# amathislab/myochallenge

Measured on AMD Instinct MI355X. Metric: env-steps/sec (Baoding, 4096 envs), higher is better.
Workload: dtype f64

## Files before the change

include/myobatch.h:

```cpp
#ifndef MYOBATCH_H
#define MYOBATCH_H

#include <stddef.h>
#include <stdint.h>

#ifdef __cplusplus
extern "C" {
#endif

#define MYO_OK 0
#define MYO_E_ARG -1
#define MYO_E_UNSUPPORTED -2
#define MYO_E_DEVICE -3
#define MYO_E_STATE -4

typedef struct myo_model myo_model;
typedef struct myo_batch myo_batch;

enum { MYO_F64 = 0, MYO_MIXED = 1, MYO_F32 = 1 };
enum { MYO_TASK_NONE = 0, MYO_TASK_BAODING_P1 = 1, MYO_TASK_BAODING_P2 = 2, MYO_TASK_REORIENT = 3, MYO_TASK_POSE = 4 };
enum { MYO_POSE_RESET_INIT = 0, MYO_POSE_RESET_RANDOM = 1, MYO_POSE_RESET_SDS = 2 };
enum { MYO_POSE_TARGET_GENERATE = 0, MYO_POSE_TARGET_FIXED = 1 };
enum { MYO_WHICH_HOLD = 0, MYO_WHICH_CW = 1, MYO_WHICH_CCW = 2 };
enum { MYO_CHOICE_FIXED = 0, MYO_CHOICE_CW = 1, MYO_CHOICE_CCW = 2, MYO_CHOICE_RANDOM = 3 };

#define MYO_N_RWD 8
#define MYO_ROT_CHOICE_MAX 4
#define MYO_OBJG_MAX 20
#define MYO_POSE_NQ_MAX 38

typedef struct myo_task_cfg {
  int32_t kind;
  int32_t frame_skip;
  int32_t max_episode_steps;
  int32_t n_hand;
  int32_t obj1_sid, obj2_sid, target1_sid, target2_sid;
  int32_t obj1_bid, obj2_bid, obj1_gid, obj2_gid;
  int32_t task_choice;
  int32_t enable_rsi, balls_overlap, limit_init_angle_on, beta_init_angle_on, beta_ball_size_on,
      beta_ball_mass_on;
  double drop_th, proximity_th;
  double center_pos[2];
  double weights[7];
  double goal_time_period[2], goal_xrange[2], goal_yrange[2];
  double rsi_probability, overlap_probability;
  double noise_palm, noise_fingers, noise_balls;
  double limit_init_angle, beta_init_angle[2], beta_ball_size[2], beta_ball_mass[2];
  double obj_size_range[2], obj_mass_range[2], obj_friction_change[3];
  double init_qpos0;
  double ro_weights[9];
  double ro_goal_pos[2], ro_goal_rot[2];
  int32_t ro_n_rot_choice[3], ro_pad_;
  double ro_rot_choice[3][MYO_ROT_CHOICE_MAX][2];
  double ro_obj_size_change, ro_pos_th, ro_rot_th;
  double ro_goal_init_pos[3], ro_goal_obj_offset[3];
  double ro_rsi_distance_pos, ro_rsi_distance_rot;
  double pose_weights[7];
  double pose_thd, pose_far_th, pose_sds_distance, pose_target_distance;
  int32_t pose_reset_type, pose_target_type;
  double pose_init_qpos[MYO_POSE_NQ_MAX];
  double pose_target_value[MYO_POSE_NQ_MAX];
  double pose_target_range[MYO_POSE_NQ_MAX][2];
  double pose_reset_range[MYO_POSE_NQ_MAX][2];
} myo_task_cfg;

int myo_model_from_blob(const void* blob, size_t nbytes, myo_model** out);
int myo_model_load_mjb(const char* path, int integrator, int unsupported_contacts, myo_model** out);
void myo_model_destroy(myo_model* m);
int myo_model_size(const myo_model* m, const char* name);

int myo_batch_create(const myo_model* m, const myo_task_cfg* cfg, int n_envs, int device,
                     uint64_t seed, int dtype, myo_batch** out);
void myo_batch_destroy(myo_batch* b);
int myo_batch_num_envs(const myo_batch* b);
int myo_batch_obs_dim(const myo_batch* b);
int myo_batch_lds_bytes(const myo_batch* b);

int myo_batch_reset(myo_batch* b, const uint8_t* mask, float* obs, void* stream);

int myo_batch_step(myo_batch* b, const float* act, float* obs, float* rew, uint8_t* done,
                   uint8_t* trunc, float* term_obs, float* comps, float* ep_info, void* stream);

int myo_batch_set_step_generation(myo_batch* b, unsigned int gen);

int myo_batch_health(myo_batch* b, int out[4]);

int myo_debug_wave_slots(int device, int n_workgroups, int lds_bytes, int32_t out[4]);

int myo_batch_step_inner(myo_batch* b, const uint8_t* mask, const float* act, float* obs, uint8_t* done, void* stream);

int myo_batch_step_inner_idx(myo_batch* b, const int* idx, int n_idx, const float* act, float* obs, uint8_t* done, void* stream);

int myo_batch_copy_envs(myo_batch* dst, const int* dst_idx, const myo_batch* src, const int* src_idx, int k, void* stream);

int myo_batch_physics_step(myo_batch* b, const double* ctrl, int nsub, void* stream);

int myo_batch_get_state(myo_batch* b, double* qpos, double* qvel, double* act, double* time,
                        void* stream);
int myo_batch_set_state(myo_batch* b, const double* qpos, const double* qvel, const double* act,
                        const double* time, void* stream);
int myo_batch_set_bad_state_buffer(myo_batch* b, uint8_t* bad_state);

int myo_batch_warmstart(myo_batch* b, double* get_qacc_warmstart, const double* set_qacc_warmstart, void* stream);

int myo_batch_set_task(myo_batch* b, const int32_t* task_i, const double* task_d,
                       const double* ball_d, void* stream);
int myo_batch_get_task(myo_batch* b, int32_t* task_i, double* task_d, double* ball_d, void* stream);

int myo_batch_set_object_group(myo_batch* b, int gid0, int gidn);
int myo_batch_object_friction(myo_batch* b, const double* set_fric, double* get_fric, void* stream);

int myo_batch_bind_constants(myo_batch* b, void* stream);

int myo_batch_tune_wrap_order(myo_batch* b, void* stream);

int myo_batch_forward_dump(myo_batch* b, const double* ctrl, double* out, void* stream);
int myo_batch_dump_size(const myo_batch* b);
int myo_batch_dump_offset(const myo_batch* b, const char* name);

typedef struct myo_render_camera {
  double lookat[3];
  double distance, azimuth, elevation;
  double fovy;
} myo_render_camera;
#define MYO_RENDER_RGB 1
#define MYO_RENDER_DEPTH 2
#define MYO_RENDER_SEG 4
#define MYO_RENDER_SITES 8
#define MYO_RENDER_ITEM_N 24
#define MYO_RENDER_MAX_PIXELS (1 << 24)

int myo_model_default_camera(const myo_model* m, myo_render_camera* out);

int myo_batch_geom_poses(myo_batch* b, const int32_t* env_idx, int k, double* out, void* stream);

int myo_batch_render(myo_batch* b, const int32_t* env_idx, int k, const myo_render_camera* cams, int ncams, int width, int height,
                     int flags, uint8_t* rgb, float* depth, int32_t* segid, void* stream);

double myo_batch_kernel_ms(myo_batch* b);
int myo_batch_enable_timing(myo_batch* b, int on);

int myo_ppo_loss_grad(const float* mean, const float* values, const float* actions, const float* old_logp,
                      const float* adv, const float* returns, const float* log_std, const float* adv_stats,
                      int B, int A, float clip, float vf_coef, float* dmean, float* dvalue, float* acc,
                      uint16_t* dmean_bf16, uint16_t* dvalue_bf16, float* work, int in_bf16, float ent_coef,
                      float* g_log_std, float* g_bias_pi, float* g_bias_vf, void* stream);

int myo_ppo_gather(const float* obs, const float* act, const float* oldlp, const float* adv, const float* ret,
                   const int64_t* idx, int bs, int obs_dim, int act_dim, uint16_t* obs_bf16, int copies,
                   float* act_mb, float* oldlp_mb, float* adv_mb, float* ret_mb, float* adv_stats , float* work,
                   void* stream);

int myo_bias_relu_bf16(uint16_t* h, const uint16_t* bias, int groups, int rows, int cols, void* stream);

int myo_splitk_reduce(const void* part, int part_is_bf16, float* out, int groups, int splits, int n, void* stream);
int myo_splitk_reduce2(const void* part_a, int a_is_bf16, float* out_a, int groups_a, int splits_a, int n_a,
                       const void* part_b, int b_is_bf16, float* out_b, int groups_b, int splits_b, int n_b, void* stream);

int myo_relu_bwd_colsum_bf16(uint16_t* dy, const uint16_t* act, int rows, int cols, float* partial, void* stream);

int myo_rollout_policy_input(const float* obs, int N, int O, float* obs_buf, uint16_t* x_bf16, int copies,
                             const int32_t* t_idx, void* stream);
int myo_rollout_sample(const uint16_t* mean_bf16, const uint16_t* value_bf16, const float* log_std, int N, int A,
                       uint64_t seed, uint64_t* draw_counter, const int32_t* t_idx, float* act_buf, float* val_buf,
                       float* logp_buf, float* clipped, int deterministic, void* stream);
int myo_vecnorm_step(const float* obs, const float* rew, const uint8_t* done, const uint8_t* trunc, const float* term_obs,
                     int N, int O, double* obs_mean, double* obs_var, double* obs_count, double* ret_stats,
                     double* returns, double gamma, double eps, double clip_obs, double clip_rew, int training,
                     int norm_obs, int norm_reward, float* nobs, float* starts, const int32_t* t_idx, float* rew_buf,
                     float* start_buf, float* term_buf, float* trunc_buf, double* work, void* stream);
int myo_rollout_sample_sde(const float* mean, const float* latent, const float* exploration_mat, const float* log_std, int N, int L,
                           int A, float* actions, float* clipped, float* logp, int deterministic, void* stream);

int myo_vecnorm_batch_moments(const float* obs, const float* rew, int N, int O, double* returns, double gamma, int training,
                              double* work, double* batch, void* stream);
int myo_vecnorm_finish(const float* obs, const float* rew, const uint8_t* done, const uint8_t* trunc, const float* term_obs,
                       int N, int O, double* obs_mean, double* obs_var, double* obs_count, double* ret_stats, double* returns,
                       double eps, double clip_obs, double clip_rew, int training, int norm_obs, int norm_reward, float* nobs,
                       float* starts, const int32_t* t_idx, float* rew_buf, float* start_buf, float* term_buf, float* trunc_buf,
                       const double* batch, void* stream);
int myo_rollout_advance(int32_t* t_idx, int T, uint64_t* draw_counter, void* stream);

int myo_lstm_cell_fwd(const void* gx, const void* gh, const void* c_prev, const float* keep_next, int R, int N, int H,
                      int is_bf16, void* out_h, void* hm_next, void* cm_next, void* c_new, void* ws, void* stream);
int myo_lstm_cell_bwd(const void* dout, const void* dhm_next, const void* dcm_next, const float* keep_next,
                      const void* c_prev, const void* c_new, const void* ws, int R, int N, int H, int is_bf16,
                      void* dgates, void* dc_prev, void* stream);

int myo_lstm_step_supported(int H);
int myo_lstm_step_fwd(const void* gx, long long gx_sg, long long gx_sr, const void* h_prev, const void* c_prev, const void* w_hh,
                      const float* keep_next, int G, int N, int H, void* out_h, long long out_sg, void* hm_next, void* cm_next,
                      void* c_new, void* ws, const float* c_prev32, float* cm_next32, void* stream);
int myo_lstm_step_bwd(const void* dout, long long dout_sg, const void* dgates_next, const void* dcm_next, const void* w_hh_t,
                      const float* keep_next, const void* c_prev, const void* c_new, const void* ws, int G, int N, int H,
                      void* dgates, void* dc_prev, void* stream);

int myo_lstm_seq_supported(int H);
int myo_lstm_seq_fwd(const void* gx, long long gx_st, long long gx_sg, long long gx_sr, void* hm, void* cm, const void* w_frag,
                     const float* keep, int G, int N, int H, int T, int row_split, void* out_h, long long out_sg, long long out_st,
                     void* c_new, void* ws, const float* c0_32, void* stream);
int myo_lstm_seq_bwd(const void* dout, long long dout_sg, long long dout_st, const void* wt_frag, const float* keep, const void* cm,
                     const void* c_new, const void* ws, int G, int N, int H, int T, int row_split, void* dgates, void* stream);

int myo_gae(const float* rew, const float* val, const float* starts, const float* last_val,
            const float* last_done, int T, int N, float gamma, float lam, float* adv, float* ret,
            void* stream);

typedef struct myo_ppo_mlp_desc {
  const float *obs, *act, *oldlp, *adv, *ret;
  const int64_t* idx;
  int32_t B, O, A, hidden;
  const float* params;
  float* grads;
  int64_t G;
  int64_t off_W1[2], off_b1[2], off_W2[2], off_b2[2], off_Wh[2], off_bh[2], off_log_std;
  float clip, vf_coef, ent_coef;
  int32_t compute_adv_stats;
  float* adv_stats;
  float* acc;
  void* workspace;
  int64_t workspace_bytes;
  float* sqnorm_part;
  int32_t* adam_step;
} myo_ppo_mlp_desc;
int myo_ppo_mlp_sqnorm_parts(int act_dim);
long long myo_ppo_mlp_workspace_bytes(int B, int obs_dim, int act_dim, int hidden, long long G);
int myo_ppo_mlp_step(const myo_ppo_mlp_desc* d, void* stream);

typedef struct myo_ppo_mlp_rollout_desc {
  const float* obs;
  int32_t N, O, A, hidden;
  const float* params;
  int64_t off_W1[2], off_b1[2], off_W2[2], off_b2[2], off_Wh[2], off_bh[2], off_log_std;
  uint64_t seed;
  uint64_t* draw_counter;
  const int32_t* t_idx;
  float *obs_buf, *act_buf, *val_buf, *logp_buf, *clipped;
  int32_t deterministic;
  void* workspace;
  int64_t workspace_bytes;
} myo_ppo_mlp_rollout_desc;
long long myo_ppo_mlp_rollout_workspace_bytes(int obs_dim, int act_dim, int hidden);
int myo_ppo_mlp_rollout_refresh(const myo_ppo_mlp_rollout_desc* d, void* stream);
int myo_ppo_mlp_rollout(const myo_ppo_mlp_rollout_desc* d, void* stream);

int myo_adam_clip_step(float* p, const float* g, float* m, float* v, int n, float lr, float b1, float b2,
                       float eps, float max_norm, float grad_scale, int* step, float* scratch, uint16_t* p_bf16,
                       void* stream);
int myo_adam_apply(float* p, const float* g, float* m, float* v, int n, float lr, float b1, float b2,
                   float eps, float max_norm, float grad_scale, const int* step, const float* scratch, int nparts,
                   uint16_t* p_bf16, void* stream);

const char* myo_last_error(void);
const char* myo_version(void);

#ifdef __cplusplus
}
#endif
#endif
```

myochallenge_amd/csrc/myo_ppo_mlp.h:

```cpp
#pragma once
#ifndef MYO_EMU

typedef __attribute__((ext_vector_type(8))) __bf16 myo_bf16x8;
typedef __attribute__((ext_vector_type(4))) float myo_f32x4;

#define MLP_H 256
#define MLP_OPMAX 128
#define MLP_APM 48
#define MLP_AKP 64
#define MLP_XS (MLP_OPMAX + 8)
#define MLP_HS (MLP_H + 8)
#define MLP_DS (MLP_AKP + 8)
#define MLP_SOS 49
#define MLP_SPLITK 16

struct MlpArgs {
  const float *obs, *act, *oldlp, *adv, *ret;
  const long long* idx;
  const float *log_std, *adv_stats;
  const unsigned short *W1p, *W2, *W2T, *Whp, *WhT;
  const float* bias;
  unsigned short *XT, *H1T, *H2T, *dH1T, *dH2T, *dOT;
  float* part;
  int B, O, A, OP, NB;
  float clip, vf_coef;
};

__device__ __forceinline__ unsigned short mlp_f2bf(float x) {
  unsigned u = __float_as_uint(x);
  u += 0x7fffu + ((u >> 16) & 1u);
  return (unsigned short)(u >> 16);
}
__device__ __forceinline__ float mlp_bf2f(unsigned short h) { return __uint_as_float((unsigned)h << 16); }

struct MlpPrepArgs {
  const float* p;
  long long off_W1[2], off_b1[2], off_W2[2], off_b2[2], off_Wh[2], off_bh[2];
  int O, OP, Ah[2];
  unsigned short *W1p, *W2, *W2T, *Whp, *WhT;
  float* bias;
  const float* adv_part;
  float* adv_stats;
  int adv_nb, B;
};

#define MLP_ADV_BLOCKS 64
__global__ void __launch_bounds__(256) k_mlp_prep(MlpPrepArgs P) {
  if (P.adv_nb > 0 && blockIdx.x == gridDim.x - 1) {
    __shared__ float sp[3 * MLP_ADV_BLOCKS];
    const int t = threadIdx.x;
    if (t < 3 * P.adv_nb) sp[t] = P.adv_part[t];
    __syncthreads();
    if (t == 0) {
      float cn = 0.f, cm = 0.f, c2 = 0.f;
      for (int b = 0; b < P.adv_nb; ++b) {
        const float bn = sp[3 * b], bm = sp[3 * b + 1], b2 = sp[3 * b + 2];
        if (bn > 0.f) {
          const float tot = cn + bn, dl = bm - cm;
          cm += dl * (bn / tot);
          c2 += b2 + dl * dl * (cn * bn / tot);
          cn = tot;
        }
      }
      P.adv_stats[0] = cm; P.adv_stats[1] = sqrtf(c2 / (P.B > 1 ? P.B - 1 : 1));
    }
  }
  constexpr int H = MLP_H;
  const long long tid = (long long)blockIdx.x * blockDim.x + threadIdx.x, nth = (long long)gridDim.x * blockDim.x;
  for (int net = 0; net < 2; ++net) {
    const float* W1 = P.p + P.off_W1[net]; const float* W2 = P.p + P.off_W2[net]; const float* Wh = P.p + P.off_Wh[net];
    for (long long e = tid; e < (long long)H * P.OP; e += nth) {
      const int o = (int)(e / P.OP), i = (int)(e % P.OP);
      P.W1p[(size_t)net * H * P.OP + e] = i < P.O ? mlp_f2bf(W1[(size_t)o * P.O + i]) : (unsigned short)0;
    }
    for (long long e = tid; e < (long long)H * H; e += nth) {
      const int o = (int)(e / H), i = (int)(e % H);
      const unsigned short v = mlp_f2bf(W2[e]);
      P.W2[(size_t)net * H * H + e] = v;
      P.W2T[(size_t)net * H * H + (size_t)i * H + o] = v;
    }
    for (long long e = tid; e < (long long)MLP_APM * H; e += nth) {
      const int a = (int)(e / H), h = (int)(e % H);
      P.Whp[(size_t)net * MLP_APM * H + e] = a < P.Ah[net] ? mlp_f2bf(Wh[(size_t)a * H + h]) : (unsigned short)0;
    }
    for (long long e = tid; e < (long long)H * MLP_AKP; e += nth) {
      const int h = (int)(e / MLP_AKP), a = (int)(e % MLP_AKP);
      P.WhT[(size_t)net * H * MLP_AKP + e] = a < P.Ah[net] ? mlp_f2bf(Wh[(size_t)a * H + h]) : (unsigned short)0;
    }
    for (long long e = tid; e < H; e += nth) {
      P.bias[net * H + e] = P.p[P.off_b1[net] + e];
      P.bias[2 * H + net * H + e] = P.p[P.off_b2[net] + e];
    }
    for (long long e = tid; e < MLP_APM; e += nth) P.bias[4 * H + net * MLP_APM + e] = e < P.Ah[net] ? P.p[P.off_bh[net] + e] : 0.f;
  }
}

__global__ void __launch_bounds__(256) k_adv_moments(const float* __restrict__ adv, const long long* __restrict__ idx, int B,
                                                     float* __restrict__ part) {
  __shared__ float red[4];
  __shared__ float s_mean;
  const int t = threadIdx.x, nb = gridDim.x;
  const int chunk = (B + nb - 1) / nb, lo = blockIdx.x * chunk, hi = min(B, lo + chunk), n = max(hi - lo, 0);
  constexpr int PER = 4;
  float v[PER];
  float s = 0.f;
#pragma unroll
  for (int k = 0; k < PER; ++k) { const int i = lo + t + 256 * k; v[k] = i < hi ? adv[idx[i]] : 0.f; s += v[k]; }
  for (int i = lo + t + 256 * PER; i < hi; i += 256) s += adv[idx[i]];
  for (int off = 32; off >= 1; off >>= 1) s += __shfl_xor(s, off, 64);
  if ((t & 63) == 0) red[t >> 6] = s;
  __syncthreads();
  if (t == 0) s_mean = n ? ((red[0] + red[1]) + (red[2] + red[3])) / n : 0.f;
  __syncthreads();
  const float mean = s_mean;
  float m2 = 0.f;
#pragma unroll
  for (int k = 0; k < PER; ++k) { const float d = v[k] - mean; m2 += (lo + t + 256 * k) < hi ? d * d : 0.f; }
  for (int i = lo + t + 256 * PER; i < hi; i += 256) { const float d = adv[idx[i]] - mean; m2 += d * d; }
  for (int off = 32; off >= 1; off >>= 1) m2 += __shfl_xor(m2, off, 64);
  __syncthreads();
  if ((t & 63) == 0) red[t >> 6] = m2;
  __syncthreads();
  if (t == 0) { part[3 * blockIdx.x] = (float)n; part[3 * blockIdx.x + 1] = mean; part[3 * blockIdx.x + 2] = (red[0] + red[1]) + (red[2] + red[3]); }
}

template <int KSTEPS>
__device__ __forceinline__ void mlp_load_w(myo_bf16x8 (&bw)[8][4], const unsigned short* Wg, int w_stride, int n0, int lm, int lq) {
#pragma unroll
  for (int ks = 0; ks < KSTEPS; ++ks)
#pragma unroll
    for (int nt = 0; nt < 4; ++nt) bw[ks][nt] = *reinterpret_cast<const myo_bf16x8*>(Wg + (size_t)(n0 + 16 * nt + lm) * w_stride + 32 * ks + 8 * lq);
  __builtin_amdgcn_sched_barrier(0);
}
template <int KSTEPS, int MT>
__device__ __forceinline__ void mlp_mma_slab(myo_f32x4 (&acc)[MT][4], const unsigned short* As, int as_stride, const myo_bf16x8 (&bw)[8][4],
                                             int lm, int lq) {
#pragma unroll
  for (int mt = 0; mt < MT; ++mt)
#pragma unroll
    for (int nt = 0; nt < 4; ++nt) acc[mt][nt] = myo_f32x4{0.f, 0.f, 0.f, 0.f};
#pragma unroll
  for (int ks = 0; ks < KSTEPS; ++ks) {
#pragma unroll
    for (int m2 = 0; m2 < MT; m2 += 2) {
      myo_bf16x8 a[2];
#pragma unroll
      for (int mt = 0; mt < 2; ++mt) a[mt] = *reinterpret_cast<const myo_bf16x8*>(As + (16 * (m2 + mt) + lm) * as_stride + 32 * ks + 8 * lq);
#pragma unroll
      for (int mt = 0; mt < 2; ++mt)
#pragma unroll
        for (int nt = 0; nt < 4; ++nt) acc[m2 + mt][nt] = __builtin_amdgcn_mfma_f32_16x16x32_bf16(a[mt], bw[ks][nt], acc[m2 + mt][nt], 0, 0, 0);
    }
  }
  __builtin_amdgcn_sched_barrier(0);
}

#ifdef MLP_PROF
__device__ unsigned long long g_mlp_prof[16];
#define MLP_STAMP(k) { __syncthreads(); if (threadIdx.x == 0 && blockIdx.x == 3 && blockIdx.y == 0) g_mlp_prof[k] = wall_clock64(); }
extern "C" int myo_debug_mlp_prof(unsigned long long* out) { return (int)hipMemcpyFromSymbol(out, HIP_SYMBOL(g_mlp_prof), sizeof g_mlp_prof); }
#else
#define MLP_STAMP(k)
#endif

#ifndef MLP_BM
#define MLP_BM 32
#endif
#define MLP_FWDBWD_LDS (512 + MLP_BM * MLP_XS * 2 + MLP_BM * MLP_HS * 2 + MLP_BM * MLP_SOS * 4 + MLP_BM * MLP_DS * 2 + 128 * 4 + 192 * 4)

template <int MT>
__device__ __forceinline__ unsigned long long mlp_store_act(const myo_f32x4 (&acc)[MT][4], const float (&bb)[4], unsigned short* Hs, unsigned short* HT,
                                                            size_t B, int r0, int n0, int lm, int lq) {
  static_assert(MT * 16 <= 64, "one mask bit per accumulator element");
  unsigned long long mask = 0;
#pragma unroll
  for (int mt = 0; mt < MT; ++mt)
#pragma unroll
    for (int nt = 0; nt < 4; ++nt) {
      const int n = n0 + 16 * nt + lm, m = 16 * mt + 4 * lq;
      unsigned short h[4];
#pragma unroll
      for (int r = 0; r < 4; ++r) {
        h[r] = mlp_f2bf(fmaxf(acc[mt][nt][r] + bb[nt], 0.f)); Hs[(m + r) * MLP_HS + n] = h[r];
        mask |= (unsigned long long)(h[r] != 0) << (16 * mt + 4 * nt + r);
      }
      *reinterpret_cast<uint2*>(HT + (size_t)n * B + r0 + m) = make_uint2((unsigned)h[0] | ((unsigned)h[1] << 16), (unsigned)h[2] | ((unsigned)h[3] << 16));
    }
  return mask;
}
template <int MT, bool TO_LDS>
__device__ __forceinline__ void mlp_store_grad(const myo_f32x4 (&acc)[MT][4], unsigned long long mask, unsigned short* Hs, unsigned short* HT, size_t B,
                                               int r0, int n0, int lm, int lq) {
#pragma unroll
  for (int mt = 0; mt < MT; ++mt)
#pragma unroll
    for (int nt = 0; nt < 4; ++nt) {
      const int n = n0 + 16 * nt + lm, m = 16 * mt + 4 * lq;
      unsigned short h[4];
#pragma unroll
      for (int r = 0; r < 4; ++r) {
        const unsigned short on = (unsigned short)(-(int)((mask >> (16 * mt + 4 * nt + r)) & 1ull));
        h[r] = mlp_f2bf(acc[mt][nt][r]) & on;
        if (TO_LDS) Hs[(m + r) * MLP_HS + n] = h[r];
      }
      *reinterpret_cast<uint2*>(HT + (size_t)n * B + r0 + m) = make_uint2((unsigned)h[0] | ((unsigned)h[1] << 16), (unsigned)h[2] | ((unsigned)h[3] << 16));
    }
}

__global__ void __launch_bounds__(256, 2) k_mlp_fwdbwd(MlpArgs P) {
  constexpr int H = MLP_H, XS = MLP_XS, HS = MLP_HS, DS = MLP_DS, SOS = MLP_SOS, BM = MLP_BM, MT = BM / 16, RW = BM / 4;
  extern __shared__ __align__(16) unsigned char mlp_smem[];
  long long* s_idx = reinterpret_cast<long long*>(mlp_smem);
  unsigned short* Xs = reinterpret_cast<unsigned short*>(mlp_smem + 512);
  float* So = reinterpret_cast<float*>(mlp_smem + 512);
  unsigned short* Hs = Xs + BM * XS;
  float* Sa = reinterpret_cast<float*>(Hs + BM * HS);
  unsigned short* dOs = reinterpret_cast<unsigned short*>(Sa + BM * SOS);
  float* s_ls = reinterpret_cast<float*>(dOs + BM * DS);
  float* s_row = s_ls + 128;
  static_assert(BM * MLP_SOS * 4 <= BM * MLP_XS * 2, "the head output tile fits where X was");
  static_assert(BM == 32 || BM == 64, "wave / tile mapping below");
  const int t = threadIdx.x, w = t >> 6, lane = t & 63, lm = lane & 15, lq = lane >> 4;
  const int net = blockIdx.y, blk = blockIdx.x, r0 = blk * BM, B = P.B, O = P.O, A = P.A, OP = P.OP;
  const int n0 = 64 * w;
  MLP_STAMP(0)
  if (t < BM) s_idx[t] = P.idx[r0 + t];
  if (t < A) { const float ls = P.log_std[t]; s_ls[t] = ls; s_ls[64 + t] = __expf(-ls); }
  const float* b1 = P.bias + net * H; const float* b2 = P.bias + 2 * H + net * H; const float* bh = P.bias + 4 * H + net * MLP_APM;
  float bb1[4], bb2[4];
#pragma unroll
  for (int nt = 0; nt < 4; ++nt) { bb1[nt] = b1[n0 + 16 * nt + lm]; bb2[nt] = b2[n0 + 16 * nt + lm]; }
  myo_bf16x8 bw[8][4];
  {
    const unsigned short* W1 = P.W1p + (size_t)net * H * OP;
    if (OP == 96) mlp_load_w<3>(bw, W1, OP, n0, lm, lq);
    else if (OP == 128) mlp_load_w<4>(bw, W1, OP, n0, lm, lq);
    else if (OP == 64) mlp_load_w<2>(bw, W1, OP, n0, lm, lq);
    else mlp_load_w<1>(bw, W1, OP, n0, lm, lq);
  }
  __syncthreads();
  if (t < BM) {
    const size_t src = (size_t)s_idx[t];
    s_row[t] = P.adv[src]; s_row[64 + t] = P.oldlp[src]; s_row[128 + t] = P.ret[src];
  }
  {
    float v[RW][2], av[RW];
#pragma unroll
    for (int k = 0; k < RW; ++k) {
      const size_t row = (size_t)s_idx[RW * w + k];
      v[k][0] = lane < O ? P.obs[row * O + lane] : 0.f;
      v[k][1] = lane + 64 < O ? P.obs[row * O + lane + 64] : 0.f;
      av[k] = (net == 0 && lane < A) ? P.act[row * A + lane] : 0.f;
    }
#pragma unroll
    for (int k = 0; k < RW; ++k) {
      Xs[(RW * w + k) * XS + lane] = mlp_f2bf(v[k][0]);
      if (lane + 64 < OP) Xs[(RW * w + k) * XS + lane + 64] = mlp_f2bf(v[k][1]);
      if (lane < A) Sa[(RW * w + k) * SOS + lane] = av[k];
    }
    if (net == 0) {
#pragma unroll
      for (int h = 0; h < 2; ++h) {
        const int c = lane + 64 * h;
        if (c < OP) {
          unsigned u[RW / 2];
#pragma unroll
          for (int k = 0; k < RW / 2; ++k) u[k] = (unsigned)mlp_f2bf(v[2 * k][h]) | ((unsigned)mlp_f2bf(v[2 * k + 1][h]) << 16);
          uint4* dst = reinterpret_cast<uint4*>(P.XT + (size_t)c * B + r0 + RW * w);
#pragma unroll
          for (int q = 0; q < RW / 8; ++q) dst[q] = make_uint4(u[4 * q], u[4 * q + 1], u[4 * q + 2], u[4 * q + 3]);
        }
      }
    }
  }
  __syncthreads();
  MLP_STAMP(1)
  myo_f32x4 acc[MT][4];
  if (OP == 96) mlp_mma_slab<3, MT>(acc, Xs, XS, bw, lm, lq);
  else if (OP == 128) mlp_mma_slab<4, MT>(acc, Xs, XS, bw, lm, lq);
  else if (OP == 64) mlp_mma_slab<2, MT>(acc, Xs, XS, bw, lm, lq);
  else mlp_mma_slab<1, MT>(acc, Xs, XS, bw, lm, lq);
  mlp_load_w<H / 32>(bw, P.W2 + (size_t)net * H * H, H, n0, lm, lq);
  const unsigned long long mask1 = mlp_store_act<MT>(acc, bb1, Hs, P.H1T + (size_t)net * H * B, B, r0, n0, lm, lq);
  __syncthreads();
  MLP_STAMP(2)
  mlp_mma_slab<H / 32, MT>(acc, Hs, HS, bw, lm, lq);
  const unsigned short* Wh = P.Whp + (size_t)net * MLP_APM * H;
  myo_bf16x8 bh2[H / 32];
  if (w < 3) {
#pragma unroll
    for (int ks = 0; ks < H / 32; ++ks) bh2[ks] = *reinterpret_cast<const myo_bf16x8*>(Wh + (size_t)(16 * w + lm) * H + 32 * ks + 8 * lq);
  }
  __builtin_amdgcn_sched_barrier(0);
  __syncthreads();
  const unsigned long long mask2 = mlp_store_act<MT>(acc, bb2, Hs, P.H2T + (size_t)net * H * B, B, r0, n0, lm, lq);
  __syncthreads();
  MLP_STAMP(3)
  if (w < 3) {
    const float bv = bh[16 * w + lm];
#pragma unroll
    for (int mt = 0; mt < MT; ++mt) {
      myo_f32x4 ah = myo_f32x4{0.f, 0.f, 0.f, 0.f};
#pragma unroll
      for (int ks = 0; ks < H / 32; ++ks) {
        const myo_bf16x8 a = *reinterpret_cast<const myo_bf16x8*>(Hs + (16 * mt + lm) * HS + 32 * ks + 8 * lq);
        ah = __builtin_amdgcn_mfma_f32_16x16x32_bf16(a, bh2[ks], ah, 0, 0, 0);
      }
#pragma unroll
      for (int r = 0; r < 4; ++r) So[(16 * mt + 4 * lq + r) * SOS + 16 * w + lm] = ah[r] + bv;
    }
  }
  mlp_load_w<MLP_AKP / 32>(bw, P.WhT + (size_t)net * H * MLP_AKP, MLP_AKP, n0, lm, lq);
  __syncthreads();
  MLP_STAMP(4)
  const int NB = P.NB;
  if (w == 0) {
    const int r = lane < BM ? lane : 0;
    const bool on = lane < BM;
    if (net == 0) {
      float logp = 0.f;
      for (int a = 0; a < A; ++a) {
        const float z = (Sa[r * SOS + a] - So[r * SOS + a]) * s_ls[64 + a];
        logp += -0.5f * z * z - s_ls[a] - 0.9189385332046727f;
      }
      const float an = (s_row[r] - P.adv_stats[0]) / (P.adv_stats[1] + 1e-8f);
      const float ratio = __expf(logp - s_row[64 + r]);
      const float s1 = an * ratio;
      const float rc = fminf(fmaxf(ratio, 1.f - P.clip), 1.f + P.clip);
      const float s2 = an * rc;
      float pl_i = on ? -fminf(s1, s2) / B : 0.f;
      const bool inside = (ratio > 1.f - P.clip) && (ratio < 1.f + P.clip);
      const float dlogp = -(an * ratio) * ((s1 <= s2) ? 1.f : (inside ? 1.f : 0.f)) / B;
      if (on) {
        for (int a = 0; a < A; ++a) {
          const float inv = s_ls[64 + a];
          const float z = (Sa[r * SOS + a] - So[r * SOS + a]) * inv;
          const float dm = dlogp * z * inv;
          So[r * SOS + a] = dm;
          Sa[r * SOS + a] = dlogp * (z * z - 1.f);
          dOs[r * DS + a] = mlp_f2bf(dm);
        }
        for (int a = A; a < MLP_AKP; ++a) dOs[r * DS + a] = 0;
      }
      for (int off = 32; off >= 1; off >>= 1) pl_i += __shfl_xor(pl_i, off, 64);
      if (lane == 0) P.part[(size_t)A * NB + blk] = pl_i;
    } else {
      const float dv = So[r * SOS] - s_row[128 + r];
      float vl_i = on ? dv * dv / B : 0.f, dv_i = on ? P.vf_coef * 2.f / B * dv : 0.f;
      if (on) {
        dOs[r * DS] = mlp_f2bf(dv_i);
        for (int a = 1; a < MLP_AKP; ++a) dOs[r * DS + a] = 0;
      }
      for (int off = 32; off >= 1; off >>= 1) { vl_i += __shfl_xor(vl_i, off, 64); dv_i += __shfl_xor(dv_i, off, 64); }
      if (lane == 0) { P.part[(size_t)(A + 1) * NB + blk] = vl_i; P.part[(size_t)(2 * A + 2) * NB + blk] = dv_i; }
    }
  }
  __syncthreads();
  MLP_STAMP(5)
  if (net == 0 && t < A) {
    float my_ls = 0.f, my_db = 0.f;
    for (int r = 0; r < BM; ++r) { my_ls += Sa[r * SOS + t]; my_db += So[r * SOS + t]; }
    P.part[(size_t)t * NB + blk] = my_ls; P.part[(size_t)(A + 2 + t) * NB + blk] = my_db;
  }
  {
    const int Ah = net == 0 ? A : 1;
    for (int e = t; e < Ah * (BM / 8); e += 256) {
      const int c = e / (BM / 8), ch = e % (BM / 8);
      unsigned v[4];
#pragma unroll
      for (int k = 0; k < 4; ++k) v[k] = (unsigned)dOs[(8 * ch + 2 * k) * DS + c] | ((unsigned)dOs[(8 * ch + 2 * k + 1) * DS + c] << 16);
      *reinterpret_cast<uint4*>(P.dOT + ((size_t)net * 128 + c) * B + r0 + 8 * ch) = make_uint4(v[0], v[1], v[2], v[3]);
    }
  }
  MLP_STAMP(6)
  mlp_mma_slab<MLP_AKP / 32, MT>(acc, dOs, DS, bw, lm, lq);
  mlp_load_w<H / 32>(bw, P.W2T + (size_t)net * H * H, H, n0, lm, lq);
  mlp_store_grad<MT, true>(acc, mask2, Hs, P.dH2T + (size_t)net * H * B, B, r0, n0, lm, lq);
  __syncthreads();
  MLP_STAMP(7)
  mlp_mma_slab<H / 32, MT>(acc, Hs, HS, bw, lm, lq);
  mlp_store_grad<MT, false>(acc, mask1, Hs, P.dH1T + (size_t)net * H * B, B, r0, n0, lm, lq);
  MLP_STAMP(8)
}

struct MlpPolicyArgs {
  const float* obs;
  const float* log_std;
  const unsigned short *W1p, *W2, *Whp;
  const float* bias;
  float* obs_buf;
  float *act_buf, *val_buf, *logp_buf, *clipped;
  const int* t_idx;
  unsigned long long* draw_counter;
  unsigned long long seed;
  int N, O, A, OP, deterministic;
};
#define MLP_POLICY_LDS (MLP_BM * MLP_XS * 2 + MLP_BM * MLP_HS * 2 + 128 * 4)

template <int MT>
__device__ __forceinline__ void mlp_store_act_lds(const myo_f32x4 (&acc)[MT][4], const float (&bb)[4], unsigned short* Hs, int n0, int lm, int lq) {
#pragma unroll
  for (int mt = 0; mt < MT; ++mt)
#pragma unroll
    for (int nt = 0; nt < 4; ++nt) {
// ... 250 lines not shown
```

myochallenge_amd/csrc/myobatch.hip:

```cpp
#include <hip/hip_runtime.h>
#include <utility>
#include <vector>
#define MYO_BACKEND_NAME "gfx950"
#define MYO_BACKEND_DENSE_NEWTON 0
#define MYO_BACKEND_BATCH_FIELDS hipEvent_t ev0, ev1; std::vector<std::pair<hipEvent_t, hipEvent_t>> pending;
#include "myo_host.h"

typedef hipStream_t be_stream;
static int be_malloc(void** p, size_t n) { return (int)hipMalloc(p, n ? n : 1); }
static void be_free(void* p) { (void)hipFree(p); }
static int be_h2d(void* d, const void* h, size_t n) { return (int)hipMemcpy(d, h, n, hipMemcpyHostToDevice); }
static int be_set_device(int dev) { return (int)hipSetDevice(dev); }
static const char* be_errstr(int e) { return hipGetErrorString((hipError_t)e); }

#define MYO_MAX_DEVICES 64
struct BoundDev { const myo_batch* b = nullptr; hipStream_t last = nullptr; bool have_last = false; hipEvent_t ev = nullptr; };
static BoundDev g_bound[MYO_MAX_DEVICES];
static std::mutex g_bound_mu;
struct SlotWs { double* p = nullptr; int* map = nullptr; int users = 0; char* big = nullptr; int big_users = 0; };
static SlotWs g_slot_ws[MYO_MAX_DEVICES];
static bool slot_workspace_acquire(int device, double** ws, int** map) {
  if (device < 0 || device >= MYO_MAX_DEVICES) return false;
  std::lock_guard<std::mutex> lk(g_bound_mu);
  SlotWs& w = g_slot_ws[device];
// ... 1258 lines not shown
      const double m = part[((size_t)b * (O + 1) + c) * 2];
      s1 += n_b * m;
      s2 += part[((size_t)b * (O + 1) + c) * 2 + 1] + n_b * m * m;
    }
    batch[1 + c] = s1; batch[2 + O + c] = s2;
  }
  if (t == 0) batch[0] = (double)N;
}
__global__ void __launch_bounds__(128) k_vecnorm_merge_batch(const double* __restrict__ batch, int O, double* __restrict__ obs_mean,
                                                             double* __restrict__ obs_var, double* __restrict__ obs_count,
                                                             double* __restrict__ ret_stats, int upd_obs, int upd_ret) {
  const int t = threadIdx.x;
  const double oc = *obs_count, rc = ret_stats[2], n = batch[0];
  __syncthreads();
  for (int c = t; c <= O; c += 128) {
    if ((c < O && !upd_obs) || (c == O && !upd_ret)) continue;
    const double bmean = batch[1 + c] / n;
    double bvar = batch[2 + O + c] / n - bmean * bmean;
    bvar = bvar < 0 ? 0 : bvar;
    double* mean = c < O ? obs_mean + c : ret_stats;
    double* var = c < O ? obs_var + c : ret_stats + 1;
    const double cnt = c < O ? oc : rc;
    const double delta = bmean - *mean, tot = cnt + n;
    const double new_mean = *mean + delta * n / tot;
    const double M2 = *var * cnt + bvar * n + delta * delta * cnt * n / tot;
    *mean = new_mean; *var = M2 / tot;
  }
  if (t == 0) { if (upd_obs) *obs_count = oc + n; if (upd_ret) ret_stats[2] = rc + n; }
}
__global__ void __launch_bounds__(256) k_vecnorm_apply(const float* __restrict__ obs, const float* __restrict__ rew,
                                                       const unsigned char* __restrict__ done, const unsigned char* __restrict__ trunc,
                                                       const float* __restrict__ term, int N, int O, const double* __restrict__ obs_mean,
                                                       const double* __restrict__ obs_var, const double* __restrict__ ret_stats,
                                                       double* __restrict__ returns, double eps, double clip_obs, double clip_rew,
                                                       int norm_obs, int norm_rew, float* __restrict__ nobs, float* __restrict__ starts,
                                                       const int* __restrict__ t_idx, float* __restrict__ rew_buf,
                                                       float* __restrict__ start_buf, float* __restrict__ term_buf,
                                                       float* __restrict__ trunc_buf) {
  const size_t i = (size_t)blockIdx.x * blockDim.x + threadIdx.x;
  const size_t n = (size_t)N * O, tt = (size_t)(*t_idx);
  if (i < n) {
    const int c = (int)(i % O);
    double o = obs[i], q = term[i];
    if (norm_obs) {
      const double sd = sqrt(obs_var[c] + eps), mu = obs_mean[c];
      o = fmin(fmax((o - mu) / sd, -clip_obs), clip_obs);
      q = fmin(fmax((q - mu) / sd, -clip_obs), clip_obs);
    }
    nobs[i] = (float)o;
    if (term_buf) term_buf[tt * n + i] = (float)q;
  }
  if (i < (size_t)N) {
    double r = rew[i];
    if (norm_rew) r = fmin(fmax(r / sqrt(ret_stats[1] + eps), -clip_rew), clip_rew);
    rew_buf[tt * N + i] = (float)r;
    start_buf[tt * N + i] = starts[i];
    const unsigned char dn = done[i];
    starts[i] = dn ? 1.f : 0.f;
    if (trunc_buf) trunc_buf[tt * N + i] = trunc[i] ? 1.f : 0.f;
    if (dn) returns[i] = 0.0;
  }
}
__global__ void __launch_bounds__(64) k_sample_sde(const float* __restrict__ mean, const float* __restrict__ latent,
                                                   const float* __restrict__ W, const float* __restrict__ log_std, int N, int L, int A,
                                                   float* __restrict__ actions, float* __restrict__ clipped, float* __restrict__ logp,
                                                   int deterministic) {
  const int n = blockIdx.x, t = threadIdx.x;
  float lp_part = 0.f;
  for (int j = t; j < A; j += 64) {
    const float* w = W + (size_t)n * L * A + j;
    const float* lat = latent + (size_t)n * L;
    float noise = 0.f, var = 0.f;
    for (int l = 0; l < L; ++l) {
      const float x = lat[l], sd = __expf(log_std[(size_t)l * A + j]);
      noise = fmaf(x, w[(size_t)l * A], noise);
      var = fmaf(x * x, sd * sd, var);
    }
    const float mu = mean[(size_t)n * A + j], sg = sqrtf(var + 1e-6f);
    const float a = deterministic ? mu : mu + noise;
    actions[(size_t)n * A + j] = a;
    clipped[(size_t)n * A + j] = fminf(fmaxf(a, -1.f), 1.f);
    const float z = (a - mu) / sg;
    lp_part += -0.5f * z * z - logf(sg) - 0.9189385332046727f;
  }
  for (int off = 32; off >= 1; off >>= 1) lp_part += __shfl_xor(lp_part, off, 64);
  if (t == 0) logp[n] = lp_part;
}
__global__ void k_rollout_advance(int* t_idx, int T, unsigned long long* draw_counter) {
  *t_idx = (*t_idx + 1) % T;
  draw_counter[0] = draw_counter[1];
}
extern "C" int myo_rollout_policy_input(const float* obs, int N, int O, float* obs_buf, uint16_t* x_bf16, int copies,
                                        const int32_t* t_idx, void* stream) {
  if (!obs || !x_bf16 || !t_idx || N <= 0 || O <= 0 || copies <= 0) return fail(MYO_E_ARG, "myo_rollout_policy_input: bad arguments");
  const size_t n = (size_t)N * O;
  hipLaunchKernelGGL(k_obs_prepare, dim3((unsigned)((n + 255) / 256)), dim3(256), 0, (hipStream_t)stream, obs, n, obs_buf, x_bf16, copies, t_idx);
  LAUNCH_CHECK(0)
  return MYO_OK;
}
extern "C" int myo_rollout_sample(const uint16_t* mean_bf16, const uint16_t* value_bf16, const float* log_std, int N, int A,
                                  uint64_t seed, uint64_t* draw_counter, const int32_t* t_idx, float* act_buf, float* val_buf,
                                  float* logp_buf, float* clipped, int deterministic, void* stream) {
  if (!mean_bf16 || !value_bf16 || !log_std || !draw_counter || !t_idx || !act_buf || !val_buf || !logp_buf || !clipped || N <= 0 || A <= 0)
    return fail(MYO_E_ARG, "myo_rollout_sample: bad arguments");
  hipLaunchKernelGGL(k_sample_actions, dim3((N + MYO_SAMPLE_ROWS - 1) / MYO_SAMPLE_ROWS), dim3(16 * MYO_SAMPLE_ROWS), 0, (hipStream_t)stream, mean_bf16, value_bf16, log_std, N, A,
                     (unsigned long long)seed, (unsigned long long*)draw_counter, t_idx, act_buf, val_buf, logp_buf, clipped, deterministic);
  LAUNCH_CHECK(0)
  return MYO_OK;
}
extern "C" int myo_vecnorm_step(const float* obs, const float* rew, const uint8_t* done, const uint8_t* trunc, const float* term_obs,
                                int N, int O, double* obs_mean, double* obs_var, double* obs_count, double* ret_stats,
                                double* returns, double gamma, double eps, double clip_obs, double clip_rew, int training,
                                int norm_obs, int norm_reward, float* nobs, float* starts, const int32_t* t_idx, float* rew_buf,
                                float* start_buf, float* term_buf, float* trunc_buf, double* work, void* stream) {
  if (!obs || !rew || !done || !trunc || !term_obs || !obs_mean || !obs_var || !obs_count || !ret_stats || !returns || !nobs ||
      !starts || !t_idx || !rew_buf || !start_buf || !work || N <= 0 || O <= 0)
    return fail(MYO_E_ARG, "myo_vecnorm_step: bad arguments");
  hipStream_t st = (hipStream_t)stream;
  const int nb = (N + MYO_VN_ROWS - 1) / MYO_VN_ROWS;
  hipLaunchKernelGGL(k_vecnorm_moments, dim3(nb), dim3(128), 0, st, obs, rew, N, O, returns, gamma, training, work);
  if (training)
    hipLaunchKernelGGL(k_vecnorm_merge, dim3(1), dim3(128), 0, st, work, nb, N, O, obs_mean, obs_var, obs_count, ret_stats,
                       (int)(training && norm_obs), (int)(training != 0));
  const size_t n = (size_t)N * O;
  hipLaunchKernelGGL(k_vecnorm_apply, dim3((unsigned)((n + 255) / 256)), dim3(256), 0, st, obs, rew, done, trunc, term_obs, N, O,
                     obs_mean, obs_var, ret_stats, returns, eps, clip_obs, clip_rew, norm_obs, norm_reward, nobs, starts, t_idx,
                     rew_buf, start_buf, term_buf, trunc_buf);
  LAUNCH_CHECK(0)
  return MYO_OK;
}
extern "C" int myo_rollout_sample_sde(const float* mean, const float* latent, const float* exploration_mat, const float* log_std,
                                      int N, int L, int A, float* actions, float* clipped, float* logp, int deterministic, void* stream) {
  if (!mean || !latent || !exploration_mat || !log_std || !actions || !clipped || !logp || N <= 0 || L <= 0 || A <= 0)
    return fail(MYO_E_ARG, "myo_rollout_sample_sde: bad arguments");
  hipLaunchKernelGGL(k_sample_sde, dim3(N), dim3(64), 0, (hipStream_t)stream, mean, latent, exploration_mat, log_std, N, L, A, actions,
                     clipped, logp, deterministic);
  LAUNCH_CHECK(0)
  return MYO_OK;
}
extern "C" int myo_vecnorm_batch_moments(const float* obs, const float* rew, int N, int O, double* returns, double gamma, int training,
                                         double* work, double* batch, void* stream) {
  if (!obs || !rew || !returns || !work || !batch || N <= 0 || O <= 0) return fail(MYO_E_ARG, "myo_vecnorm_batch_moments: bad arguments");
  hipStream_t st = (hipStream_t)stream;
  const int nb = (N + MYO_VN_ROWS - 1) / MYO_VN_ROWS;
  hipLaunchKernelGGL(k_vecnorm_moments, dim3(nb), dim3(128), 0, st, obs, rew, N, O, returns, gamma, training, work);
  hipLaunchKernelGGL(k_vecnorm_batch, dim3(1), dim3(128), 0, st, work, nb, N, O, batch);
  LAUNCH_CHECK(0)
  return MYO_OK;
}
extern "C" int myo_vecnorm_finish(const float* obs, const float* rew, const uint8_t* done, const uint8_t* trunc, const float* term_obs,
                                  int N, int O, double* obs_mean, double* obs_var, double* obs_count, double* ret_stats,
                                  double* returns, double eps, double clip_obs, double clip_rew, int training, int norm_obs,
                                  int norm_reward, float* nobs, float* starts, const int32_t* t_idx, float* rew_buf, float* start_buf,
                                  float* term_buf, float* trunc_buf, const double* batch, void* stream) {
  if (!obs || !rew || !done || !trunc || !term_obs || !obs_mean || !obs_var || !obs_count || !ret_stats || !returns || !nobs ||
      !starts || !t_idx || !rew_buf || !start_buf || !batch || N <= 0 || O <= 0)
    return fail(MYO_E_ARG, "myo_vecnorm_finish: bad arguments");
  hipStream_t st = (hipStream_t)stream;
  if (training)
    hipLaunchKernelGGL(k_vecnorm_merge_batch, dim3(1), dim3(128), 0, st, batch, O, obs_mean, obs_var, obs_count, ret_stats,
                       (int)(training && norm_obs), (int)(training != 0));
  const size_t n = (size_t)N * O;
  hipLaunchKernelGGL(k_vecnorm_apply, dim3((unsigned)((n + 255) / 256)), dim3(256), 0, st, obs, rew, done, trunc, term_obs, N, O,
                     obs_mean, obs_var, ret_stats, returns, eps, clip_obs, clip_rew, norm_obs, norm_reward, nobs, starts, t_idx,
                     rew_buf, start_buf, term_buf, trunc_buf);
  LAUNCH_CHECK(0)
  return MYO_OK;
}
extern "C" int myo_rollout_advance(int32_t* t_idx, int T, uint64_t* draw_counter, void* stream) {
  if (!t_idx || !draw_counter || T <= 0) return fail(MYO_E_ARG, "myo_rollout_advance: bad arguments");
  hipLaunchKernelGGL(k_rollout_advance, dim3(1), dim3(1), 0, (hipStream_t)stream, t_idx, T, (unsigned long long*)draw_counter);
  LAUNCH_CHECK(0)
  return MYO_OK;
}

template <typename E> __device__ __forceinline__ float myo_ld(const E* p, size_t i);
template <> __device__ __forceinline__ float myo_ld<float>(const float* p, size_t i) { return p[i]; }
template <> __device__ __forceinline__ float myo_ld<unsigned short>(const unsigned short* p, size_t i) { return __uint_as_float((unsigned)p[i] << 16); }
template <typename E> __device__ __forceinline__ void myo_st(E* p, size_t i, float v);
template <> __device__ __forceinline__ void myo_st<float>(float* p, size_t i, float v) { p[i] = v; }
template <> __device__ __forceinline__ void myo_st<unsigned short>(unsigned short* p, size_t i, float v) { p[i] = myo_f2bf(v); }
__device__ __forceinline__ float myo_sigmoid(float x) { return 1.f / (1.f + __expf(-x)); }
template <typename E>
__global__ void __launch_bounds__(256) k_lstm_cell_fwd(const E* __restrict__ gx, const E* __restrict__ gh, const E* __restrict__ c_prev,
                                                       const float* __restrict__ keep_next, int R, int N, int H, E* __restrict__ out_h,
                                                       E* __restrict__ hm_next, E* __restrict__ cm_next, E* __restrict__ c_new,
                                                       E* __restrict__ ws) {
  const size_t idx = (size_t)blockIdx.x * blockDim.x + threadIdx.x;
  if (idx >= (size_t)R * H) return;
  const int r = (int)(idx / H), j = (int)(idx % H);
  const size_t g0 = (size_t)r * 4 * H + j;
  const float i = myo_sigmoid(myo_ld(gx, g0) + myo_ld(gh, g0));
  const float f = myo_sigmoid(myo_ld(gx, g0 + H) + myo_ld(gh, g0 + H));
  const float g = tanhf(myo_ld(gx, g0 + 2 * H) + myo_ld(gh, g0 + 2 * H));
  const float o = myo_sigmoid(myo_ld(gx, g0 + 3 * H) + myo_ld(gh, g0 + 3 * H));
  const float c = f * myo_ld(c_prev, idx) + i * g;
  const float h = o * tanhf(c);
  const float k = keep_next ? keep_next[r % N] : 1.f;
  myo_st(out_h, idx, h);
  myo_st(c_new, idx, c);
  myo_st(hm_next, idx, h * k);
  myo_st(cm_next, idx, c * k);
  myo_st(ws, g0, i); myo_st(ws, g0 + H, f); myo_st(ws, g0 + 2 * H, g); myo_st(ws, g0 + 3 * H, o);
}
template <typename E>
__global__ void __launch_bounds__(256) k_lstm_cell_bwd(const E* __restrict__ dout, const E* __restrict__ dhm_next, const E* __restrict__ dcm_next,
                                                       const float* __restrict__ keep_next, const E* __restrict__ c_prev,
                                                       const E* __restrict__ c_new, const E* __restrict__ ws, int R, int N, int H,
                                                       E* __restrict__ dgates, E* __restrict__ dc_prev) {
  const size_t idx = (size_t)blockIdx.x * blockDim.x + threadIdx.x;
  if (idx >= (size_t)R * H) return;
  const int r = (int)(idx / H), j = (int)(idx % H);
  const size_t g0 = (size_t)r * 4 * H + j;
  const float k = keep_next ? keep_next[r % N] : 1.f;
  const float dh = (dout ? myo_ld(dout, idx) : 0.f) + (dhm_next ? k * myo_ld(dhm_next, idx) : 0.f);
  const float dc_in = dcm_next ? k * myo_ld(dcm_next, idx) : 0.f;
  const float i = myo_ld(ws, g0), f = myo_ld(ws, g0 + H), g = myo_ld(ws, g0 + 2 * H), o = myo_ld(ws, g0 + 3 * H);
  const float tc = tanhf(myo_ld(c_new, idx));
  const float dct = dc_in + dh * o * (1.f - tc * tc);
  myo_st(dgates, g0, dct * g * i * (1.f - i));
  myo_st(dgates, g0 + H, dct * myo_ld(c_prev, idx) * f * (1.f - f));
  myo_st(dgates, g0 + 2 * H, dct * i * (1.f - g * g));
  myo_st(dgates, g0 + 3 * H, dh * tc * o * (1.f - o));
  myo_st(dc_prev, idx, dct * f);
}
extern "C" int myo_lstm_cell_fwd(const void* gx, const void* gh, const void* c_prev, const float* keep_next, int R, int N, int H,
                                 int is_bf16, void* out_h, void* hm_next, void* cm_next, void* c_new, void* ws, void* stream) {
  if (!gx || !gh || !c_prev || !out_h || !hm_next || !cm_next || !c_new || !ws || R <= 0 || N <= 0 || H <= 0 || R % N)
    return fail(MYO_E_ARG, "myo_lstm_cell_fwd: bad arguments");
  const unsigned nb = (unsigned)(((size_t)R * H + 255) / 256);
  if (is_bf16)
    hipLaunchKernelGGL(k_lstm_cell_fwd<unsigned short>, dim3(nb), dim3(256), 0, (hipStream_t)stream, (const unsigned short*)gx,
                       (const unsigned short*)gh, (const unsigned short*)c_prev, keep_next, R, N, H, (unsigned short*)out_h,
                       (unsigned short*)hm_next, (unsigned short*)cm_next, (unsigned short*)c_new, (unsigned short*)ws);
  else
    hipLaunchKernelGGL(k_lstm_cell_fwd<float>, dim3(nb), dim3(256), 0, (hipStream_t)stream, (const float*)gx, (const float*)gh,
                       (const float*)c_prev, keep_next, R, N, H, (float*)out_h, (float*)hm_next, (float*)cm_next, (float*)c_new,
                       (float*)ws);
  LAUNCH_CHECK(0)
  return MYO_OK;
}
extern "C" int myo_lstm_cell_bwd(const void* dout, const void* dhm_next, const void* dcm_next, const float* keep_next,
                                 const void* c_prev, const void* c_new, const void* ws, int R, int N, int H, int is_bf16,
                                 void* dgates, void* dc_prev, void* stream) {
  if (!c_prev || !c_new || !ws || !dgates || !dc_prev || R <= 0 || N <= 0 || H <= 0 || R % N)
    return fail(MYO_E_ARG, "myo_lstm_cell_bwd: bad arguments");
  const unsigned nb = (unsigned)(((size_t)R * H + 255) / 256);
  if (is_bf16)
    hipLaunchKernelGGL(k_lstm_cell_bwd<unsigned short>, dim3(nb), dim3(256), 0, (hipStream_t)stream, (const unsigned short*)dout,
                       (const unsigned short*)dhm_next, (const unsigned short*)dcm_next, keep_next, (const unsigned short*)c_prev,
                       (const unsigned short*)c_new, (const unsigned short*)ws, R, N, H, (unsigned short*)dgates,
                       (unsigned short*)dc_prev);
  else
    hipLaunchKernelGGL(k_lstm_cell_bwd<float>, dim3(nb), dim3(256), 0, (hipStream_t)stream, (const float*)dout, (const float*)dhm_next,
                       (const float*)dcm_next, keep_next, (const float*)c_prev, (const float*)c_new, (const float*)ws, R, N, H,
                       (float*)dgates, (float*)dc_prev);
  LAUNCH_CHECK(0)
  return MYO_OK;
}

__global__ void k_gae(const float* __restrict__ rew, const float* __restrict__ val, const float* __restrict__ starts,
                      const float* __restrict__ last_val, const float* __restrict__ last_done, int T, int N, float gamma,
                      float lam, float* __restrict__ adv, float* __restrict__ ret) {
  const int e = blockIdx.x * blockDim.x + threadIdx.x;
  if (e >= N) return;
  float last = 0.f, nextv = last_val[e], nonterm = 1.f - last_done[e];
  for (int t = T - 1; t >= 0; --t) {
    const size_t i = (size_t)t * N + e;
    const float v = val[i];
    const float delta = rew[i] + gamma * nextv * nonterm - v;
    last = delta + gamma * lam * nonterm * last;
    adv[i] = last;
    ret[i] = last + v;
    nextv = v;
    nonterm = 1.f - starts[i];
  }
}
extern "C" int myo_gae(const float* rew, const float* val, const float* starts, const float* last_val, const float* last_done,
                       int T, int N, float gamma, float lam, float* adv, float* ret, void* stream) {
  if (!rew || !val || !starts || !last_val || !last_done || !adv || !ret || T <= 0 || N <= 0) return fail(MYO_E_ARG, "myo_gae: bad arguments");
  hipLaunchKernelGGL(k_gae, dim3((N + 255) / 256), dim3(256), 0, (hipStream_t)stream, rew, val, starts, last_val, last_done, T, N,
                     gamma, lam, adv, ret);
  LAUNCH_CHECK(0)
  return MYO_OK;
}

#define MYO_SQN_BLOCKS 64
__global__ void __launch_bounds__(256) k_grad_sqnorm(const float* __restrict__ g, int n, float gs, float* __restrict__ part,
                                                     int* __restrict__ step) {
  float acc = 0.f;
  for (int i = blockIdx.x * 256 + threadIdx.x; i < n; i += MYO_SQN_BLOCKS * 256) { const float x = g[i] * gs; acc += x * x; }
  for (int off = 32; off >= 1; off >>= 1) acc += __shfl_xor(acc, off, 64);
  __shared__ float red[4];
  if ((threadIdx.x & 63) == 0) red[threadIdx.x >> 6] = acc;
  __syncthreads();
  if (threadIdx.x == 0) {
    part[blockIdx.x] = (red[0] + red[1]) + (red[2] + red[3]);
    if (blockIdx.x == 0) { const int done = step[1]; step[0] = done; step[1] = done + 1; }
  }
}
__global__ void __launch_bounds__(256) k_adam(float* __restrict__ p, const float* __restrict__ g, float* __restrict__ m,
                                              float* __restrict__ v, int n, float lr, float b1, float b2, float eps,
                                              float max_norm, float gs, const int* __restrict__ step,
                                              const float* __restrict__ part, unsigned short* __restrict__ p_bf16, int nparts) {
  __shared__ float sq_red[256];
  {
    float a = 0.f;
    for (int k = threadIdx.x; k < nparts; k += 256) a += part[k];
    sq_red[threadIdx.x] = a;
    __syncthreads();
    for (int w = 128; w >= 1; w >>= 1) { if ((int)threadIdx.x < w) sq_red[threadIdx.x] += sq_red[threadIdx.x + w]; __syncthreads(); }
  }
  const float sq = sq_red[0];
  const int t = step[1];
  const float norm = sqrtf(sq);
  const float clip = (max_norm > 0.f) ? fminf(1.f, max_norm / (norm + 1e-6f)) : 1.f;
  const float bc1 = 1.f - powf(b1, (float)t), bc2 = 1.f - powf(b2, (float)t);
  const float step_size = lr / bc1, inv_sqrt_bc2 = rsqrtf(bc2);
  for (int i = blockIdx.x * blockDim.x + threadIdx.x; i < n; i += gridDim.x * blockDim.x) {
    const float gi = g[i] * gs * clip;
    const float mi = b1 * m[i] + (1.f - b1) * gi;
    const float vi = b2 * v[i] + (1.f - b2) * gi * gi;
    m[i] = mi; v[i] = vi;
    const float pn = p[i] - step_size * mi / (sqrtf(vi) * inv_sqrt_bc2 + eps);
    p[i] = pn;
    if (p_bf16) p_bf16[i] = myo_f2bf(pn);
  }
}
extern "C" int myo_adam_clip_step(float* p, const float* g, float* m, float* v, int n, float lr, float b1, float b2,
                                  float eps, float max_norm, float grad_scale, int* step, float* scratch, uint16_t* p_bf16,
                                  void* stream) {
  if (!p || !g || !m || !v || !step || !scratch || n <= 0) return fail(MYO_E_ARG, "myo_adam_clip_step: bad arguments");
  hipStream_t st = (hipStream_t)stream;
  const int blocks = (n + 255) / 256 < 1024 ? (n + 255) / 256 : 1024;
  hipLaunchKernelGGL(k_grad_sqnorm, dim3(MYO_SQN_BLOCKS), dim3(256), 0, st, g, n, grad_scale, scratch, step);
  hipLaunchKernelGGL(k_adam, dim3(blocks), dim3(256), 0, st, p, g, m, v, n, lr, b1, b2, eps, max_norm, grad_scale, step, scratch,
                     (unsigned short*)p_bf16, MYO_SQN_BLOCKS);
  LAUNCH_CHECK(0)
  return MYO_OK;
}
extern "C" int myo_adam_apply(float* p, const float* g, float* m, float* v, int n, float lr, float b1, float b2,
                              float eps, float max_norm, float grad_scale, const int* step, const float* scratch, int nparts,
                              uint16_t* p_bf16, void* stream) {
  if (!p || !g || !m || !v || !step || !scratch || n <= 0 || nparts <= 0) return fail(MYO_E_ARG, "myo_adam_apply: bad arguments");
  const int blocks = (n + 255) / 256 < 1024 ? (n + 255) / 256 : 1024;
  hipLaunchKernelGGL(k_adam, dim3(blocks), dim3(256), 0, (hipStream_t)stream, p, g, m, v, n, lr, b1, b2, eps, max_norm, grad_scale, step, scratch,
                     (unsigned short*)p_bf16, nparts);
  LAUNCH_CHECK(0)
  return MYO_OK;
}

#include "myo_ppo_mlp.h"
struct MlpWs { unsigned short *W1p, *W2, *W2T, *Whp, *WhT; float* bias; unsigned short *XT, *H1T, *H2T, *dH1T, *dH2T, *dOT; float *part, *slab, *advpart; size_t bytes; };
static MlpWs mlp_carve(unsigned char* base, int B, int OP, int A, long long G) {
  MlpWs w;
  size_t o = 0;
  auto take = [&](size_t n) { unsigned char* p = base ? base + o : nullptr; o += (n + 255) / 256 * 256; return p; };
  const size_t H = MLP_H;
  w.W1p = (unsigned short*)take(2 * H * OP * 2); w.W2 = (unsigned short*)take(2 * H * H * 2); w.W2T = (unsigned short*)take(2 * H * H * 2);
  w.Whp = (unsigned short*)take(2 * MLP_APM * H * 2); w.WhT = (unsigned short*)take(2 * H * MLP_AKP * 2);
  w.bias = (float*)take((4 * H + 2 * MLP_APM) * 4);
  w.XT = (unsigned short*)take((size_t)128 * B * 2);
  w.H1T = (unsigned short*)take(2 * H * (size_t)B * 2); w.H2T = (unsigned short*)take(2 * H * (size_t)B * 2);
  w.dH1T = (unsigned short*)take(2 * H * (size_t)B * 2); w.dH2T = (unsigned short*)take(2 * H * (size_t)B * 2);
  w.dOT = (unsigned short*)take((size_t)256 * B * 2);
  w.part = (float*)take((size_t)(2 * A + 3) * (B / MLP_BM) * 4);
  w.slab = (float*)take((size_t)MLP_SPLITK * G * 4);
  w.advpart = (float*)take(3 * MLP_ADV_BLOCKS * 4);
  w.bytes = o;
  return w;
}
static int mlp_shape_ok(int B, int O, int A, int hidden) {
  return hidden == MLP_H && O >= 1 && O <= MLP_OPMAX && A >= 1 && A <= MLP_APM && B >= 64 * MLP_SPLITK && B % (64 * MLP_SPLITK) == 0;
}
extern "C" long long myo_ppo_mlp_workspace_bytes(int B, int obs_dim, int act_dim, int hidden, long long G) {
  if (!mlp_shape_ok(B, obs_dim, act_dim, hidden) || G <= 0) return -1;
  return (long long)mlp_carve(nullptr, B, (obs_dim + 31) / 32 * 32, act_dim, G).bytes;
}
extern "C" int myo_ppo_mlp_sqnorm_parts(int act_dim) {
  return MLP_RF_BLOCKS + 2 * act_dim + 3;
}
extern "C" int myo_ppo_mlp_step(const myo_ppo_mlp_desc* d, void* stream) {
  if (!d || !d->obs || !d->act || !d->oldlp || !d->adv || !d->ret || !d->idx || !d->params || !d->grads || !d->adv_stats || !d->acc ||
      !d->workspace)
    return fail(MYO_E_ARG, "myo_ppo_mlp_step: null argument");
  const int B = d->B, O = d->O, A = d->A, OP = (O + 31) / 32 * 32;
  if (!mlp_shape_ok(B, O, A, d->hidden)) return fail(MYO_E_UNSUPPORTED, "myo_ppo_mlp_step: needs hidden = %d, obs <= %d, act <= %d, batch a multiple of %d", MLP_H, MLP_OPMAX, MLP_APM, 64 * MLP_SPLITK);
  const MlpWs w = mlp_carve((unsigned char*)d->workspace, B, OP, A, d->G);
  if ((long long)w.bytes > d->workspace_bytes) return fail(MYO_E_ARG, "myo_ppo_mlp_step: workspace too small (%zu bytes needed)", w.bytes);
  hipStream_t st = (hipStream_t)stream;
  static bool lds_set = false;
  if (!lds_set) {
    if (hipFuncSetAttribute((const void*)k_mlp_fwdbwd, hipFuncAttributeMaxDynamicSharedMemorySize, MLP_FWDBWD_LDS) != hipSuccess)
      return fail(MYO_E_DEVICE, "myo_ppo_mlp_step: cannot reserve %d bytes of LDS", (int)MLP_FWDBWD_LDS);
    lds_set = true;
  }
  if (d->compute_adv_stats) hipLaunchKernelGGL(k_adv_moments, dim3(MLP_ADV_BLOCKS), dim3(256), 0, st, d->adv, (const long long*)d->idx, B, w.advpart);
  MlpPrepArgs pp;
  pp.p = d->params; pp.O = O; pp.OP = OP; pp.Ah[0] = A; pp.Ah[1] = 1;
  for (int k = 0; k < 2; ++k) {
    pp.off_W1[k] = d->off_W1[k]; pp.off_b1[k] = d->off_b1[k]; pp.off_W2[k] = d->off_W2[k]; pp.off_b2[k] = d->off_b2[k];
    pp.off_Wh[k] = d->off_Wh[k]; pp.off_bh[k] = d->off_bh[k];
  }
  pp.adv_part = w.advpart; pp.adv_stats = d->adv_stats; pp.adv_nb = d->compute_adv_stats ? MLP_ADV_BLOCKS : 0; pp.B = B;
  pp.W1p = w.W1p; pp.W2 = w.W2; pp.W2T = w.W2T; pp.Whp = w.Whp; pp.WhT = w.WhT; pp.bias = w.bias;
  hipLaunchKernelGGL(k_mlp_prep, dim3(256), dim3(256), 0, st, pp);
  MlpArgs a;
  a.obs = d->obs; a.act = d->act; a.oldlp = d->oldlp; a.adv = d->adv; a.ret = d->ret; a.idx = (const long long*)d->idx;
  a.log_std = d->params + d->off_log_std; a.adv_stats = d->adv_stats;
  a.W1p = w.W1p; a.W2 = w.W2; a.W2T = w.W2T; a.Whp = w.Whp; a.WhT = w.WhT; a.bias = w.bias;
  a.XT = w.XT; a.H1T = w.H1T; a.H2T = w.H2T; a.dH1T = w.dH1T; a.dH2T = w.dH2T; a.dOT = w.dOT; a.part = w.part;
  a.B = B; a.O = O; a.A = A; a.OP = OP; a.NB = B / MLP_BM; a.clip = d->clip; a.vf_coef = d->vf_coef;
  hipLaunchKernelGGL(k_mlp_fwdbwd, dim3(B / MLP_BM, 2), dim3(256), MLP_FWDBWD_LDS, st, a);
  MlpWgradArgs g;
  g.njobs = 0; g.B = B; g.rows_per_split = B / MLP_SPLITK; g.G = d->G; g.slab = w.slab;
  const size_t HB = (size_t)MLP_H * B;
  for (int net = 0; net < 2; ++net) {
    for (int m0 = 0; m0 < MLP_H; m0 += 128) {
      for (int n0 = 0; n0 < MLP_H; n0 += 128)
        g.job[g.njobs++] = MlpWgradJob{w.dH2T + net * HB, w.H1T + net * HB, MLP_H, MLP_H, MLP_H, m0, n0, d->off_W2[net], n0 == 0 ? d->off_b2[net] : -1};
      g.job[g.njobs++] = MlpWgradJob{w.dH1T + net * HB, w.XT, MLP_H, O, O, m0, 0, d->off_W1[net], d->off_b1[net]};
    }
    for (int n0 = 0; n0 < MLP_H; n0 += 128)
      g.job[g.njobs++] = MlpWgradJob{w.dOT + (size_t)net * 128 * B, w.H2T + net * HB, net == 0 ? A : 1, MLP_H, MLP_H, 0, n0, d->off_Wh[net], -1};
  }
  hipLaunchKernelGGL(k_mlp_wgrad, dim3(g.njobs * MLP_SPLITK), dim3(256), 0, st, g);
  if (d->sqnorm_part && d->adam_step) {
    MlpRfArgs rf;
    rf.slab = w.slab; rf.g = d->grads; rf.G = d->G; rf.splits = MLP_SPLITK; rf.part = w.part; rf.acc = d->acc; rf.NB = B / MLP_BM; rf.A = A;
    rf.ent_coef = d->ent_coef; rf.off_log_std = d->off_log_std; rf.off_bh0 = d->off_bh[0]; rf.off_bh1 = d->off_bh[1];
    rf.sq_part = d->sqnorm_part; rf.adam_step = d->adam_step;
    hipLaunchKernelGGL(k_mlp_reduce_finish, dim3(MLP_RF_BLOCKS + 2 * A + 3), dim3(256), 0, st, rf);
  } else {
    hipLaunchKernelGGL(k_mlp_reduce, dim3((unsigned)((d->G + 255) / 256)), dim3(256), 0, st, (const float*)w.slab, d->grads, d->G, MLP_SPLITK);
    hipLaunchKernelGGL(k_colmajor_finish, dim3(2 * A + 3), dim3(64), 0, st, (const float*)w.part, d->acc, B / MLP_BM, A, d->ent_coef,
                       d->grads + d->off_log_std, d->grads + d->off_bh[0], d->grads + d->off_bh[1]);
  }
  LAUNCH_CHECK(0)
  return MYO_OK;
}

struct MlpImg { unsigned short *W1p, *W2, *W2T, *Whp, *WhT; float* bias; size_t bytes; };
static MlpImg mlp_carve_images(unsigned char* base, int OP) {
  MlpImg w;
  size_t o = 0;
  auto take = [&](size_t n) { unsigned char* p = base ? base + o : nullptr; o += (n + 255) / 256 * 256; return p; };
  const size_t H = MLP_H;
  w.W1p = (unsigned short*)take(2 * H * OP * 2); w.W2 = (unsigned short*)take(2 * H * H * 2); w.W2T = (unsigned short*)take(2 * H * H * 2);
  w.Whp = (unsigned short*)take(2 * MLP_APM * H * 2); w.WhT = (unsigned short*)take(2 * H * MLP_AKP * 2);
  w.bias = (float*)take((4 * H + 2 * MLP_APM) * 4);
  w.bytes = o;
  return w;
}
static int mlp_rollout_ok(const myo_ppo_mlp_rollout_desc* d) {
  return d->hidden == MLP_H && d->O >= 1 && d->O <= MLP_OPMAX && d->A >= 1 && d->A <= MLP_APM && d->N >= MLP_BM && d->N % MLP_BM == 0;
}
extern "C" long long myo_ppo_mlp_rollout_workspace_bytes(int obs_dim, int act_dim, int hidden) {
  if (hidden != MLP_H || obs_dim < 1 || obs_dim > MLP_OPMAX || act_dim < 1 || act_dim > MLP_APM) return -1;
  return (long long)mlp_carve_images(nullptr, (obs_dim + 31) / 32 * 32).bytes;
}
extern "C" int myo_ppo_mlp_rollout_refresh(const myo_ppo_mlp_rollout_desc* d, void* stream) {
  if (!d || !d->params || !d->workspace) return fail(MYO_E_ARG, "myo_ppo_mlp_rollout_refresh: null argument");
  if (!mlp_rollout_ok(d)) return fail(MYO_E_UNSUPPORTED, "myo_ppo_mlp_rollout: needs hidden = %d, obs <= %d, act <= %d, envs a multiple of %d", MLP_H, MLP_OPMAX, MLP_APM, MLP_BM);
  const int OP = (d->O + 31) / 32 * 32;
  const MlpImg w = mlp_carve_images((unsigned char*)d->workspace, OP);
  if ((long long)w.bytes > d->workspace_bytes) return fail(MYO_E_ARG, "myo_ppo_mlp_rollout_refresh: workspace too small (%zu bytes needed)", w.bytes);
  MlpPrepArgs pp;
  pp.p = d->params; pp.O = d->O; pp.OP = OP; pp.Ah[0] = d->A; pp.Ah[1] = 1;
  for (int k = 0; k < 2; ++k) {
    pp.off_W1[k] = d->off_W1[k]; pp.off_b1[k] = d->off_b1[k]; pp.off_W2[k] = d->off_W2[k]; pp.off_b2[k] = d->off_b2[k];
    pp.off_Wh[k] = d->off_Wh[k]; pp.off_bh[k] = d->off_bh[k];
  }
  pp.adv_part = nullptr; pp.adv_stats = nullptr; pp.adv_nb = 0; pp.B = 0;
  pp.W1p = w.W1p; pp.W2 = w.W2; pp.W2T = w.W2T; pp.Whp = w.Whp; pp.WhT = w.WhT; pp.bias = w.bias;
  hipLaunchKernelGGL(k_mlp_prep, dim3(256), dim3(256), 0, (hipStream_t)stream, pp);
  LAUNCH_CHECK(0)
  return MYO_OK;
}
extern "C" int myo_ppo_mlp_rollout(const myo_ppo_mlp_rollout_desc* d, void* stream) {
  if (!d || !d->obs || !d->params || !d->draw_counter || !d->t_idx || !d->act_buf || !d->val_buf || !d->logp_buf || !d->clipped || !d->workspace)
    return fail(MYO_E_ARG, "myo_ppo_mlp_rollout: null argument");
  if (!mlp_rollout_ok(d)) return fail(MYO_E_UNSUPPORTED, "myo_ppo_mlp_rollout: needs hidden = %d, obs <= %d, act <= %d, envs a multiple of %d", MLP_H, MLP_OPMAX, MLP_APM, MLP_BM);
  const int OP = (d->O + 31) / 32 * 32;
  const MlpImg w = mlp_carve_images((unsigned char*)d->workspace, OP);
  if ((long long)w.bytes > d->workspace_bytes) return fail(MYO_E_ARG, "myo_ppo_mlp_rollout: workspace too small (%zu bytes needed)", w.bytes);
  MlpPolicyArgs a;
  a.obs = d->obs; a.log_std = d->params + d->off_log_std; a.W1p = w.W1p; a.W2 = w.W2; a.Whp = w.Whp; a.bias = w.bias;
  a.obs_buf = d->obs_buf; a.act_buf = d->act_buf; a.val_buf = d->val_buf; a.logp_buf = d->logp_buf; a.clipped = d->clipped;
  a.t_idx = d->t_idx; a.draw_counter = (unsigned long long*)d->draw_counter; a.seed = d->seed;
  a.N = d->N; a.O = d->O; a.A = d->A; a.OP = OP; a.deterministic = d->deterministic;
  hipLaunchKernelGGL(k_mlp_policy, dim3(d->N / MLP_BM, 2), dim3(256), MLP_POLICY_LDS, (hipStream_t)stream, a);
  LAUNCH_CHECK(0)
  return MYO_OK;
}

#include "myo_lstm_step.h"
extern "C" int myo_lstm_step_supported(int H) { return (H == 32 || H == 64 || H == 128 || H == 256) ? 1 : 0; }
extern "C" int myo_lstm_step_fwd(const void* gx, long long gx_sg, long long gx_sr, const void* h_prev, const void* c_prev, const void* w_hh,
                                 const float* keep_next, int G, int N, int H, void* out_h, long long out_sg, void* hm_next, void* cm_next,
                                 void* c_new, void* ws, const float* c_prev32, float* cm_next32, void* stream) {
  if (!gx || !h_prev || (!c_prev && !c_prev32) || !w_hh || !out_h || !hm_next || (!cm_next && !cm_next32) || G <= 0 || N <= 0 || H <= 0 || (gx_sg & 3) || (gx_sr & 3) || (out_sg & 3))
    return fail(MYO_E_ARG, "myo_lstm_step_fwd: bad arguments");
  if (!myo_lstm_step_supported(H)) return fail(MYO_E_UNSUPPORTED, "myo_lstm_step_fwd: hidden size %d (32, 64, 128 or 256)", H);
  typedef const unsigned short* cu;
  typedef unsigned short* mu;
#define MYO_LSTM_FWD(HH)                                                                                                              \
  lstm_step_fwd_launch<HH>((cu)gx, gx_sg, gx_sr, (cu)h_prev, (cu)c_prev, (cu)w_hh, keep_next, G, N, (mu)out_h, out_sg, (mu)hm_next,   \
                           (mu)cm_next, (mu)c_new, (mu)ws, c_prev32, cm_next32, (hipStream_t)stream)
  switch (H) {
    case 32: MYO_LSTM_FWD(32); break;
    case 64: MYO_LSTM_FWD(64); break;
    case 128: MYO_LSTM_FWD(128); break;
    default: MYO_LSTM_FWD(256); break;
  }
#undef MYO_LSTM_FWD
  LAUNCH_CHECK(0)
  return MYO_OK;
}
extern "C" int myo_lstm_step_bwd(const void* dout, long long dout_sg, const void* dgates_next, const void* dcm_next, const void* w_hh_t,
                                 const float* keep_next, const void* c_prev, const void* c_new, const void* ws, int G, int N, int H,
                                 void* dgates, void* dc_prev, void* stream) {
  if (!c_prev || !c_new || !ws || !dgates || !dc_prev || (dgates_next && !w_hh_t) || G <= 0 || N <= 0 || H <= 0 || (dout_sg & 3))
    return fail(MYO_E_ARG, "myo_lstm_step_bwd: bad arguments");
  if (!myo_lstm_step_supported(H)) return fail(MYO_E_UNSUPPORTED, "myo_lstm_step_bwd: hidden size %d (32, 64, 128 or 256)", H);
  typedef const unsigned short* cu;
  typedef unsigned short* mu;
#define MYO_LSTM_BWD(HH)                                                                                                               \
  lstm_step_bwd_launch<HH>((cu)dout, dout_sg, (cu)dgates_next, (cu)dcm_next, (cu)w_hh_t, keep_next, (cu)c_prev, (cu)c_new, (cu)ws, G, N, \
                           (mu)dgates, (mu)dc_prev, (hipStream_t)stream)
  switch (H) {
    case 32: MYO_LSTM_BWD(32); break;
    case 64: MYO_LSTM_BWD(64); break;
    case 128: MYO_LSTM_BWD(128); break;
    default: MYO_LSTM_BWD(256); break;
  }
#undef MYO_LSTM_BWD
  LAUNCH_CHECK(0)
  return MYO_OK;
}

#include "myo_lstm_seq.h"
extern "C" int myo_lstm_seq_supported(int H) { return (H == 128 || H == 256) ? 1 : 0; }
static int lstm_seq_rs_ok(int H, int rs) { return rs == 1 || rs == 2 || (rs == 4 && H == 256); }
extern "C" int myo_lstm_seq_fwd(const void* gx, long long gx_st, long long gx_sg, long long gx_sr, void* hm, void* cm, const void* w_frag,
                                const float* keep, int G, int N, int H, int T, int row_split, void* out_h, long long out_sg, long long out_st,
                                void* c_new, void* ws, const float* c0_32, void* stream) {
  if (!gx || !hm || !cm || !w_frag || !keep || !out_h || !c_new || !ws || G <= 0 || N <= 0 || H <= 0 || T <= 0 || (gx_st & 7) || (gx_sg & 7) ||
      (gx_sr & 7) || (out_sg & 7) || (out_st & 7) || (N & 15))
    return fail(MYO_E_ARG, "myo_lstm_seq_fwd: bad arguments (N must be a multiple of 16, strides of 8)");
  if (!myo_lstm_seq_supported(H) || !lstm_seq_rs_ok(H, row_split))
    return fail(MYO_E_UNSUPPORTED, "myo_lstm_seq_fwd: hidden size %d (128 or 256) with row split %d (1, 2; 4 at 256)", H, row_split);
  typedef const unsigned short* cu;
  typedef unsigned short* mu;
#define MYO_SEQ_FWD(HH, RR) lstm_seq_fwd_launch<HH, RR>((cu)gx, gx_st, gx_sg, gx_sr, (mu)hm, (mu)cm, (cu)w_frag, keep, G, N, T, (mu)out_h, out_sg, out_st, \
                                                        (mu)c_new, (mu)ws, c0_32, (hipStream_t)stream)
  const int rc = H == 128 ? (row_split == 1 ? MYO_SEQ_FWD(128, 1) : MYO_SEQ_FWD(128, 2))
                          : (row_split == 1 ? MYO_SEQ_FWD(256, 1) : row_split == 2 ? MYO_SEQ_FWD(256, 2) : MYO_SEQ_FWD(256, 4));
#undef MYO_SEQ_FWD
  return rc ? fail(MYO_E_DEVICE, "myo_lstm_seq_fwd: launch failed") : MYO_OK;
}
extern "C" int myo_lstm_seq_bwd(const void* dout, long long dout_sg, long long dout_st, const void* wt_frag, const float* keep, const void* cm,
                                const void* c_new, const void* ws, int G, int N, int H, int T, int row_split, void* dgates, void* stream) {
  if (!dout || !wt_frag || !keep || !cm || !c_new || !ws || !dgates || G <= 0 || N <= 0 || H <= 0 || T <= 0 || (dout_sg & 7) || (dout_st & 7) || (N & 15))
    return fail(MYO_E_ARG, "myo_lstm_seq_bwd: bad arguments (N must be a multiple of 16, strides of 8)");
  if (!myo_lstm_seq_supported(H) || !lstm_seq_rs_ok(H, row_split))
    return fail(MYO_E_UNSUPPORTED, "myo_lstm_seq_bwd: hidden size %d (128 or 256) with row split %d (1, 2; 4 at 256)", H, row_split);
  typedef const unsigned short* cu;
#define MYO_SEQ_BWD(HH, RR) lstm_seq_bwd_launch<HH, RR>((cu)dout, dout_sg, dout_st, (cu)wt_frag, keep, (cu)cm, (cu)c_new, (cu)ws, G, N, T, \
                                                        (unsigned short*)dgates, (hipStream_t)stream)
  const int rc = H == 128 ? (row_split == 1 ? MYO_SEQ_BWD(128, 1) : MYO_SEQ_BWD(128, 2))
                          : (row_split == 1 ? MYO_SEQ_BWD(256, 1) : row_split == 2 ? MYO_SEQ_BWD(256, 2) : MYO_SEQ_BWD(256, 4));
#undef MYO_SEQ_BWD
  return rc ? fail(MYO_E_DEVICE, "myo_lstm_seq_bwd: launch failed") : MYO_OK;
}
```

myochallenge_amd/native.py:

```python
from __future__ import annotations

import ctypes as C
import os
from typing import Optional

import numpy as np

_HERE = os.path.dirname(os.path.abspath(__file__))
LIB_PATH = os.path.join(_HERE, "libmyobatch.so")

MYO_F64, MYO_MIXED = 0, 1
MYO_F32 = MYO_MIXED
TASK_NONE, TASK_BAODING_P1, TASK_BAODING_P2, TASK_REORIENT, TASK_POSE = 0, 1, 2, 3, 4
POSE_RESET_INIT, POSE_RESET_RANDOM, POSE_RESET_SDS = 0, 1, 2
POSE_TARGET_GENERATE, POSE_TARGET_FIXED = 0, 1
CHOICE_FIXED, CHOICE_CW, CHOICE_CCW, CHOICE_RANDOM = 0, 1, 2, 3
N_RWD = 8
RWD_KEYS = ("pos_dist_1", "pos_dist_2", "act_reg", "alive", "sparse", "solved", "done", "dense")


ROT_CHOICE_MAX, OBJG_MAX, POSE_NQ_MAX = 4, 20, 38


class TaskCfg(C.Structure):
    _fields_ = [
        ("kind", C.c_int32), ("frame_skip", C.c_int32), ("max_episode_steps", C.c_int32),
        ("n_hand", C.c_int32),
        ("obj1_sid", C.c_int32), ("obj2_sid", C.c_int32), ("target1_sid", C.c_int32),
        ("target2_sid", C.c_int32), ("obj1_bid", C.c_int32), ("obj2_bid", C.c_int32),
        ("obj1_gid", C.c_int32), ("obj2_gid", C.c_int32),
        ("task_choice", C.c_int32), ("enable_rsi", C.c_int32), ("balls_overlap", C.c_int32),
        ("limit_init_angle_on", C.c_int32), ("beta_init_angle_on", C.c_int32),
        ("beta_ball_size_on", C.c_int32), ("beta_ball_mass_on", C.c_int32),
        ("drop_th", C.c_double), ("proximity_th", C.c_double), ("center_pos", C.c_double * 2),
        ("weights", C.c_double * 7),
        ("goal_time_period", C.c_double * 2), ("goal_xrange", C.c_double * 2),
        ("goal_yrange", C.c_double * 2),
        ("rsi_probability", C.c_double), ("overlap_probability", C.c_double),
        ("noise_palm", C.c_double), ("noise_fingers", C.c_double), ("noise_balls", C.c_double),
        ("limit_init_angle", C.c_double), ("beta_init_angle", C.c_double * 2),
        ("beta_ball_size", C.c_double * 2), ("beta_ball_mass", C.c_double * 2),
        ("obj_size_range", C.c_double * 2), ("obj_mass_range", C.c_double * 2),
        ("obj_friction_change", C.c_double * 3), ("init_qpos0", C.c_double),
        ("ro_weights", C.c_double * 9), ("ro_goal_pos", C.c_double * 2), ("ro_goal_rot", C.c_double * 2),
        ("ro_n_rot_choice", C.c_int32 * 3), ("ro_pad_", C.c_int32),
        ("ro_rot_choice", C.c_double * 2 * ROT_CHOICE_MAX * 3),
        ("ro_obj_size_change", C.c_double), ("ro_pos_th", C.c_double), ("ro_rot_th", C.c_double),
        ("ro_goal_init_pos", C.c_double * 3), ("ro_goal_obj_offset", C.c_double * 3),
        ("ro_rsi_distance_pos", C.c_double), ("ro_rsi_distance_rot", C.c_double),
        ("pose_weights", C.c_double * 7),
        ("pose_thd", C.c_double), ("pose_far_th", C.c_double), ("pose_sds_distance", C.c_double),
        ("pose_target_distance", C.c_double),
        ("pose_reset_type", C.c_int32), ("pose_target_type", C.c_int32),
        ("pose_init_qpos", C.c_double * POSE_NQ_MAX), ("pose_target_value", C.c_double * POSE_NQ_MAX),
        ("pose_target_range", C.c_double * 2 * POSE_NQ_MAX), ("pose_reset_range", C.c_double * 2 * POSE_NQ_MAX),
    ]


class PpoMlpDesc(C.Structure):
    _fields_ = [
        ("obs", C.c_void_p), ("act", C.c_void_p), ("oldlp", C.c_void_p), ("adv", C.c_void_p), ("ret", C.c_void_p), ("idx", C.c_void_p),
        ("B", C.c_int32), ("O", C.c_int32), ("A", C.c_int32), ("hidden", C.c_int32),
        ("params", C.c_void_p), ("grads", C.c_void_p), ("G", C.c_int64),
        ("off_W1", C.c_int64 * 2), ("off_b1", C.c_int64 * 2), ("off_W2", C.c_int64 * 2), ("off_b2", C.c_int64 * 2),
        ("off_Wh", C.c_int64 * 2), ("off_bh", C.c_int64 * 2), ("off_log_std", C.c_int64),
        ("clip", C.c_float), ("vf_coef", C.c_float), ("ent_coef", C.c_float), ("compute_adv_stats", C.c_int32),
        ("adv_stats", C.c_void_p), ("acc", C.c_void_p), ("workspace", C.c_void_p), ("workspace_bytes", C.c_int64),
        ("sqnorm_part", C.c_void_p), ("adam_step", C.c_void_p),
    ]


class PpoMlpRolloutDesc(C.Structure):
    _fields_ = [
        ("obs", C.c_void_p), ("N", C.c_int32), ("O", C.c_int32), ("A", C.c_int32), ("hidden", C.c_int32), ("params", C.c_void_p),
        ("off_W1", C.c_int64 * 2), ("off_b1", C.c_int64 * 2), ("off_W2", C.c_int64 * 2), ("off_b2", C.c_int64 * 2),
        ("off_Wh", C.c_int64 * 2), ("off_bh", C.c_int64 * 2), ("off_log_std", C.c_int64),
        ("seed", C.c_uint64), ("draw_counter", C.c_void_p), ("t_idx", C.c_void_p),
        ("obs_buf", C.c_void_p), ("act_buf", C.c_void_p), ("val_buf", C.c_void_p), ("logp_buf", C.c_void_p), ("clipped", C.c_void_p),
        ("deterministic", C.c_int32), ("workspace", C.c_void_p), ("workspace_bytes", C.c_int64),
    ]


class RenderCamera(C.Structure):
    _fields_ = [("lookat", C.c_double * 3), ("distance", C.c_double), ("azimuth", C.c_double), ("elevation", C.c_double),
                ("fovy", C.c_double)]


RENDER_RGB, RENDER_DEPTH, RENDER_SEG, RENDER_SITES = 1, 2, 4, 8
RENDER_ITEM_N = 24


class MyoError(RuntimeError):
    pass


class NativeLib:
    def __init__(self, path: str):
        if not os.path.exists(path):
            raise MyoError(
                f"{path} not found: build the HIP extension first (python -c 'import __graft_entry__ as g; "
                "g.build()').  libmyobatch has no CPU fallback.")
        L = C.CDLL(path)
        self.path = path
        self.L = L
        vp, i32, u64, dbl = C.c_void_p, C.c_int, C.c_uint64, C.c_double
        L.myo_last_error.restype = C.c_char_p
        L.myo_version.restype = C.c_char_p
        L.myo_model_from_blob.argtypes = [vp, C.c_size_t, C.POINTER(vp)]
        L.myo_model_load_mjb.argtypes = [C.c_char_p, i32, i32, C.POINTER(vp)]
        L.myo_model_destroy.argtypes = [vp]
        L.myo_model_size.argtypes = [vp, C.c_char_p]
        L.myo_batch_create.argtypes = [vp, C.POINTER(TaskCfg), i32, i32, u64, i32, C.POINTER(vp)]
        L.myo_batch_destroy.argtypes = [vp]
        L.myo_batch_num_envs.argtypes = [vp]
        L.myo_batch_set_step_generation.argtypes = [vp, C.c_uint32]
        L.myo_batch_health.argtypes = [vp, C.POINTER(i32)]
        L.myo_debug_wave_slots.argtypes = [C.c_int, C.c_int, C.c_int, C.POINTER(i32)]
        L.myo_batch_obs_dim.argtypes = [vp]
        L.myo_batch_lds_bytes.argtypes = [vp]
        L.myo_batch_reset.argtypes = [vp, vp, vp, vp]
        L.myo_batch_step.argtypes = [vp] * 10
        L.myo_batch_step_inner.argtypes = [vp] * 6
        L.myo_batch_step_inner_idx.argtypes = [vp, vp, i32, vp, vp, vp, vp]
        L.myo_batch_copy_envs.argtypes = [vp, vp, vp, vp, i32, vp]
        L.myo_batch_physics_step.argtypes = [vp, vp, i32, vp]
        L.myo_batch_get_state.argtypes = [vp] * 6
        L.myo_batch_set_state.argtypes = [vp] * 6
        L.myo_batch_set_task.argtypes = [vp] * 5
        L.myo_batch_warmstart.argtypes = [vp] * 4
        L.myo_batch_set_bad_state_buffer.argtypes = [vp, vp]
        L.myo_batch_get_task.argtypes = [vp] * 5
        L.myo_batch_bind_constants.argtypes = [vp, vp]
        L.myo_batch_tune_wrap_order.argtypes = [vp, vp]
        L.myo_batch_set_object_group.argtypes = [vp, i32, i32]
        L.myo_batch_object_friction.argtypes = [vp, vp, vp, vp]
        L.myo_batch_forward_dump.argtypes = [vp, vp, vp, vp]
        L.myo_batch_dump_size.argtypes = [vp]
        L.myo_batch_dump_offset.argtypes = [vp, C.c_char_p]
        L.myo_batch_kernel_ms.argtypes = [vp]
        L.myo_batch_kernel_ms.restype = dbl
        L.myo_batch_enable_timing.argtypes = [vp, i32]
        L.myo_model_default_camera.argtypes = [vp, C.POINTER(RenderCamera)]
        L.myo_batch_geom_poses.argtypes = [vp, vp, i32, vp, vp]
        L.myo_batch_render.argtypes = [vp, vp, i32, C.POINTER(RenderCamera), i32, i32, i32, i32, vp, vp, vp, vp]
        if b"MYO_EMU" in L.myo_version():
            return
        L.myo_ppo_loss_grad.argtypes = [vp] * 8 + [i32, i32, C.c_float, C.c_float, vp, vp, vp, vp, vp, vp, i32, C.c_float, vp, vp, vp, vp]
        L.myo_ppo_gather.argtypes = [vp] * 6 + [i32, i32, i32, vp, i32] + [vp] * 7
        L.myo_bias_relu_bf16.argtypes = [vp, vp, i32, i32, i32, vp]
        L.myo_splitk_reduce.argtypes = [vp, i32, vp, i32, i32, i32, vp]
        L.myo_splitk_reduce2.argtypes = [vp, i32, vp, i32, i32, i32, vp, i32, vp, i32, i32, i32, vp]
        L.myo_relu_bwd_colsum_bf16.argtypes = [vp, vp, i32, i32, vp, vp]
        L.myo_rollout_policy_input.argtypes = [vp, i32, i32, vp, vp, i32, vp, vp]
        L.myo_rollout_sample.argtypes = [vp, vp, vp, i32, i32, u64, vp, vp, vp, vp, vp, vp, i32, vp]
        L.myo_vecnorm_step.argtypes = [vp] * 5 + [i32, i32] + [vp] * 5 + [dbl] * 4 + [i32] * 3 + [vp] * 9
        L.myo_rollout_advance.argtypes = [vp, i32, vp, vp]
        L.myo_rollout_sample_sde.argtypes = [vp] * 4 + [i32] * 3 + [vp] * 3 + [i32, vp]
        L.myo_vecnorm_batch_moments.argtypes = [vp, vp, i32, i32, vp, dbl, i32, vp, vp, vp]
        L.myo_vecnorm_finish.argtypes = [vp] * 5 + [i32, i32] + [vp] * 5 + [dbl] * 3 + [i32] * 3 + [vp] * 9
        L.myo_gae.argtypes = [vp] * 5 + [i32, i32, C.c_float, C.c_float, vp, vp, vp]
        L.myo_lstm_cell_fwd.argtypes = [vp] * 4 + [i32] * 4 + [vp] * 6
        L.myo_lstm_cell_bwd.argtypes = [vp] * 7 + [i32] * 4 + [vp] * 3
        L.myo_lstm_step_supported.argtypes = [i32]
        L.myo_lstm_step_fwd.argtypes = [vp, C.c_longlong, C.c_longlong] + [vp] * 4 + [i32] * 3 + [vp, C.c_longlong] + [vp] * 7
        L.myo_lstm_step_bwd.argtypes = [vp, C.c_longlong] + [vp] * 7 + [i32] * 3 + [vp] * 3
        L.myo_lstm_seq_supported.argtypes = [i32]
        L.myo_lstm_seq_fwd.argtypes = [vp] + [C.c_longlong] * 3 + [vp] * 4 + [i32] * 5 + [vp, C.c_longlong, C.c_longlong] + [vp] * 4
        L.myo_lstm_seq_bwd.argtypes = [vp, C.c_longlong, C.c_longlong] + [vp] * 5 + [i32] * 5 + [vp] * 2
        L.myo_adam_clip_step.argtypes = [vp] * 4 + [i32] + [C.c_float] * 6 + [vp, vp, vp, vp]
        L.myo_adam_apply.argtypes = [vp] * 4 + [i32] + [C.c_float] * 6 + [vp, vp, i32, vp, vp]
        L.myo_ppo_mlp_workspace_bytes.restype = C.c_longlong
        L.myo_ppo_mlp_workspace_bytes.argtypes = [i32, i32, i32, i32, C.c_longlong]
        L.myo_ppo_mlp_step.argtypes = [C.POINTER(PpoMlpDesc), vp]
        L.myo_ppo_mlp_sqnorm_parts.argtypes = [i32]
        L.myo_ppo_mlp_rollout_workspace_bytes.restype = C.c_longlong
        L.myo_ppo_mlp_rollout_workspace_bytes.argtypes = [i32, i32, i32]
        L.myo_ppo_mlp_rollout_refresh.argtypes = [C.POINTER(PpoMlpRolloutDesc), vp]
        L.myo_ppo_mlp_rollout.argtypes = [C.POINTER(PpoMlpRolloutDesc), vp]

    def check(self, rc: int):
        if rc != 0:
            raise MyoError(f"libmyobatch error {rc}: {self.L.myo_last_error().decode()}")

    @property
    def version(self) -> str:
        return self.L.myo_version().decode()

    @property
    def build_id(self) -> str:
        v = self.version
        return v.rsplit(" build ", 1)[1] if " build " in v else "unknown"

    @property
    def is_emulation(self) -> bool:
        return "MYO_EMU" in self.version


_LIB: Optional[NativeLib] = None


def load(path: Optional[str] = None) -> NativeLib:
    global _LIB
    if path is not None:
        return NativeLib(path)
    if _LIB is None:
        _LIB = NativeLib(LIB_PATH)
    return _LIB


EXPORTED_SYMBOLS = [
    "myo_model_from_blob", "myo_model_load_mjb", "myo_model_destroy", "myo_model_size", "myo_batch_create",
    "myo_batch_destroy", "myo_batch_set_step_generation", "myo_batch_health", "myo_debug_wave_slots", "myo_batch_num_envs", "myo_batch_obs_dim", "myo_batch_lds_bytes",
    "myo_batch_reset", "myo_batch_step", "myo_batch_step_inner", "myo_batch_step_inner_idx", "myo_batch_copy_envs", "myo_batch_physics_step", "myo_batch_get_state",
    "myo_batch_set_state", "myo_batch_warmstart", "myo_batch_set_bad_state_buffer", "myo_batch_set_task", "myo_batch_get_task", "myo_batch_set_object_group", "myo_batch_object_friction", "myo_batch_bind_constants", "myo_batch_tune_wrap_order", "myo_batch_forward_dump",
    "myo_batch_dump_size", "myo_batch_dump_offset", "myo_batch_kernel_ms",
    "myo_batch_enable_timing", "myo_ppo_loss_grad", "myo_ppo_gather", "myo_bias_relu_bf16", "myo_rollout_policy_input", "myo_rollout_sample",
    "myo_vecnorm_step", "myo_rollout_sample_sde", "myo_vecnorm_batch_moments", "myo_vecnorm_finish", "myo_rollout_advance", "myo_gae", "myo_lstm_cell_fwd", "myo_lstm_cell_bwd", "myo_lstm_step_supported", "myo_lstm_step_fwd", "myo_lstm_step_bwd", "myo_lstm_seq_supported", "myo_lstm_seq_fwd", "myo_lstm_seq_bwd", "myo_splitk_reduce", "myo_splitk_reduce2", "myo_relu_bwd_colsum_bf16", "myo_adam_clip_step", "myo_ppo_mlp_workspace_bytes", "myo_ppo_mlp_step", "myo_ppo_mlp_sqnorm_parts", "myo_adam_apply", "myo_ppo_mlp_rollout_workspace_bytes", "myo_ppo_mlp_rollout_refresh", "myo_ppo_mlp_rollout", "myo_last_error", "myo_version",
    "myo_model_default_camera", "myo_batch_geom_poses", "myo_batch_render",
]

ENV_PATH_SYMBOLS = [
    "myo_batch_bind_constants", "myo_batch_copy_envs", "myo_batch_create", "myo_batch_destroy", "myo_batch_dump_offset", "myo_batch_dump_size",
    "myo_batch_enable_timing", "myo_batch_forward_dump", "myo_batch_get_state", "myo_batch_get_task", "myo_batch_health", "myo_batch_kernel_ms",
    "myo_batch_lds_bytes", "myo_batch_num_envs", "myo_batch_object_friction", "myo_batch_obs_dim", "myo_batch_physics_step", "myo_batch_reset",
    "myo_batch_set_bad_state_buffer", "myo_batch_set_object_group", "myo_batch_set_state", "myo_batch_set_step_generation", "myo_batch_set_task",
    "myo_batch_step", "myo_batch_step_inner", "myo_batch_step_inner_idx", "myo_batch_tune_wrap_order", "myo_batch_warmstart", "myo_debug_wave_slots",
    "myo_last_error", "myo_model_destroy", "myo_model_from_blob", "myo_model_load_mjb", "myo_model_size", "myo_version",
    "myo_model_default_camera", "myo_batch_geom_poses", "myo_batch_render",
]


class Model:

    def __init__(self, compiled, lib: Optional[NativeLib] = None):
        self.lib = lib or load()
        self.compiled = compiled
        blob = compiled.to_blob()
        self._buf = C.create_string_buffer(blob, len(blob))
        h = C.c_void_p()
        self.lib.check(self.lib.L.myo_model_from_blob(self._buf, len(blob), C.byref(h)))
        self.h = h

    @classmethod
    def from_mjb(cls, path: str, lib: Optional[NativeLib] = None, integrator: Optional[int] = None, unsupported_contacts: str = "error",
                 allow_other_solver: bool = False):
        self = cls.__new__(cls)
        self.lib, self.compiled, self._buf = lib or load(), None, None
        h = C.c_void_p()
        self.lib.check(self.lib.L.myo_model_load_mjb(os.fsencode(path), -1 if integrator is None else int(integrator),
                                                     {"error": 0, "drop": 1}[unsupported_contacts] | (2 if allow_other_solver else 0), C.byref(h)))
        self.h = h
        return self

    def size(self, name: str) -> int:
        return self.lib.L.myo_model_size(self.h, name.encode())

    def default_camera(self) -> dict:
        c = RenderCamera()
        self.lib.check(self.lib.L.myo_model_default_camera(self.h, C.byref(c)))
        return {"lookat": tuple(c.lookat), "distance": c.distance, "azimuth": c.azimuth, "elevation": c.elevation, "fovy": c.fovy}

    def __del__(self):
        if getattr(self, "h", None):
            self.lib.L.myo_model_destroy(self.h)
            self.h = None


def _ptr(x):
    if x is None:
        return None
    if isinstance(x, int):
        return x
    if isinstance(x, np.ndarray):
        assert x.flags["C_CONTIGUOUS"]
        return x.ctypes.data
    return x.data_ptr()


class Batch:

    def __init__(self, model: Model, cfg: Optional[TaskCfg], n_envs: int, device: int = 0, seed: int = 0,
                 dtype: int = MYO_F32):
        self.lib, self.model = model.lib, model
        h = C.c_void_p()
        self.lib.check(self.lib.L.myo_batch_create(model.h, C.byref(cfg) if cfg is not None else None,
                                                   n_envs, device, seed, dtype, C.byref(h)))
        self.h = h
        self.n = n_envs
        self.dtype = dtype
        self.obs_dim = self.lib.L.myo_batch_obs_dim(h)

    def reset(self, mask=None, obs=None, stream=None):
        self.lib.check(self.lib.L.myo_batch_reset(self.h, _ptr(mask), _ptr(obs), stream))

    def step(self, act, obs, rew, done, trunc=None, term_obs=None, comps=None, ep_info=None, stream=None):
        self.lib.check(self.lib.L.myo_batch_step(self.h, _ptr(act), _ptr(obs), _ptr(rew), _ptr(done), _ptr(trunc),
                                                 _ptr(term_obs), _ptr(comps), _ptr(ep_info), stream))

    def step_inner(self, mask, act, obs, done=None, stream=None):
        self.lib.check(self.lib.L.myo_batch_step_inner(self.h, _ptr(mask), _ptr(act), _ptr(obs), _ptr(done), stream))

    def step_inner_idx(self, idx, act, obs, done=None, stream=None):
        self.lib.check(self.lib.L.myo_batch_step_inner_idx(self.h, _ptr(idx), int(idx.shape[0]), _ptr(act), _ptr(obs), _ptr(done), stream))

    def copy_envs_from(self, src: "Batch", dst_idx, src_idx, stream=None):
        self.lib.check(self.lib.L.myo_batch_copy_envs(self.h, _ptr(dst_idx), src.h, _ptr(src_idx), int(dst_idx.shape[0]), stream))

    def physics_step(self, ctrl, nsub, stream=None):
        self.lib.check(self.lib.L.myo_batch_physics_step(self.h, _ptr(ctrl), nsub, stream))

    def get_state(self, qpos=None, qvel=None, act=None, time=None, stream=None):
        self.lib.check(self.lib.L.myo_batch_get_state(self.h, _ptr(qpos), _ptr(qvel), _ptr(act), _ptr(time), stream))

    def set_state(self, qpos=None, qvel=None, act=None, time=None, stream=None):
        self.lib.check(self.lib.L.myo_batch_set_state(self.h, _ptr(qpos), _ptr(qvel), _ptr(act), _ptr(time), stream))

    def health(self) -> dict:
        out = (C.c_int32 * 4)()
        self.lib.check(self.lib.L.myo_batch_health(self.h, out))
        return {"protocol_errors": int(out[0]), "contact_overflows": int(out[1]), "limit_row_overflows": int(out[2]), "contact_slots_wanted": int(out[3])}

    def set_bad_state_buffer(self, buf):
        self._bad_buf = buf
        self.lib.check(self.lib.L.myo_batch_set_bad_state_buffer(self.h, _ptr(buf)))

    def warmstart(self, get=None, set=None, stream=None):
        self.lib.check(self.lib.L.myo_batch_warmstart(self.h, _ptr(get), _ptr(set), stream))

    def set_task(self, task_i=None, task_d=None, ball_d=None, stream=None):
        self.lib.check(self.lib.L.myo_batch_set_task(self.h, _ptr(task_i), _ptr(task_d), _ptr(ball_d), stream))

    def set_object_group(self, gid0: int, gidn: int):
        self.lib.check(self.lib.L.myo_batch_set_object_group(self.h, gid0, gidn))

    def object_friction(self, set_fric=None, get_fric=None, stream=None):
        self.lib.check(self.lib.L.myo_batch_object_friction(self.h, _ptr(set_fric), _ptr(get_fric), stream))

    def bind_constants(self, stream=None):
        self.lib.check(self.lib.L.myo_batch_bind_constants(self.h, stream))

    def tune_wrap_order(self, stream=None):
        self.lib.check(self.lib.L.myo_batch_tune_wrap_order(self.h, stream))

    def get_task(self, task_i=None, task_d=None, ball_d=None, stream=None):
        self.lib.check(self.lib.L.myo_batch_get_task(self.h, _ptr(task_i), _ptr(task_d), _ptr(ball_d), stream))

    def forward_dump(self, ctrl, out, stream=None):
        self.lib.check(self.lib.L.myo_batch_forward_dump(self.h, _ptr(ctrl), _ptr(out), stream))

    def geom_poses(self, env_idx, out, stream=None):
        self.lib.check(self.lib.L.myo_batch_geom_poses(self.h, _ptr(env_idx), int(env_idx.shape[0]), _ptr(out), stream))

    def render(self, env_idx, cams, width, height, flags, rgb=None, depth=None, segid=None, stream=None):
        arr = (RenderCamera * len(cams))()
        for c, d in zip(arr, cams):
            c.lookat[:] = [float(x) for x in d["lookat"]]
            c.distance, c.azimuth, c.elevation, c.fovy = (float(d[k]) for k in ("distance", "azimuth", "elevation", "fovy"))
        self.lib.check(self.lib.L.myo_batch_render(self.h, _ptr(env_idx), int(env_idx.shape[0]), arr, len(cams), int(width), int(height),
                                                   int(flags), _ptr(rgb), _ptr(depth), _ptr(segid), stream))

    @property
    def dump_size(self) -> int:
        return self.lib.L.myo_batch_dump_size(self.h)

    def dump_offset(self, name: str) -> int:
        return self.lib.L.myo_batch_dump_offset(self.h, name.encode())

    @property
    def lds_bytes(self) -> int:
        return self.lib.L.myo_batch_lds_bytes(self.h)

    def enable_timing(self, on=True):
        self.lib.check(self.lib.L.myo_batch_enable_timing(self.h, int(on)))

    def kernel_ms(self) -> float:
        return self.lib.L.myo_batch_kernel_ms(self.h)

    def close(self):
        if getattr(self, "h", None):
            self.lib.L.myo_batch_destroy(self.h)
            self.h = None

    def __del__(self):
        self.close()
```

myochallenge_amd/rl/fused_mlp.py:

```python
from __future__ import annotations

import ctypes as C
import math
from typing import List, Tuple

import torch


def _layers(seq) -> List[torch.nn.Linear]:
    return [m for m in seq if isinstance(m, torch.nn.Linear)]


def _nets(policy):
    return {"pi": _layers(policy.mlp_extractor.policy_net) + [policy.action_net],
            "vf": _layers(policy.mlp_extractor.value_net) + [policy.value_net]}


def _splitk_wgrad(dy: torch.Tensor, x: torch.Tensor, split: int) -> Tuple[torch.Tensor, torch.Tensor]:
    B = x.shape[0]
    if split > 1 and B % split == 0:
        gw = torch.bmm(dy.view(split, B // split, -1).transpose(1, 2), x.view(split, B // split, -1)).sum(0, dtype=torch.float32)
    else:
        gw = (dy.t() @ x).float()
    return gw, dy.sum(0, dtype=torch.float32)


@torch.no_grad()
def ppo_mlp_step_grads(policy, obs, actions, old_logp, adv, returns, clip_range, ent_coef, vf_coef,
                       normalize_advantage=True, bf16=True, split_k=32):
    assert not policy.recurrent
    cd = torch.bfloat16 if (bf16 and obs.is_cuda) else torch.float32
    B = obs.shape[0]
    x0 = obs.to(cd)
    nets = _nets(policy)
    acts, outs = {}, {}
    for name, layers in nets.items():
        h = x0
        saved = [h]
        for li, lin in enumerate(layers):
            h = torch.addmm(lin.bias.to(cd), h, lin.weight.to(cd).t())
            if li < len(layers) - 1:
                h = torch.relu_(h)
                saved.append(h)
        acts[name], outs[name] = saved, h.float()
    mean, values = outs["pi"], outs["vf"].squeeze(-1)
    log_std = policy.log_std.float()
    inv_std = torch.exp(-log_std)
    z = (actions - mean) * inv_std
    logp = (-0.5 * z * z - log_std - 0.5 * math.log(2 * math.pi)).sum(-1)
    if normalize_advantage and B > 1:
        adv = (adv - adv.mean()) / (adv.std() + 1e-8)
    ratio = torch.exp(logp - old_logp)
    s1 = adv * ratio
    s2 = adv * torch.clamp(ratio, 1 - clip_range, 1 + clip_range)
    pl = -torch.min(s1, s2).mean()
    vl = torch.mean((values - returns) ** 2)
    inside = (ratio > 1 - clip_range) & (ratio < 1 + clip_range)
    dlogp = -(adv * ratio) * torch.where(s1 <= s2, torch.ones_like(ratio), inside.to(ratio.dtype)) / B
    dmean = dlogp.unsqueeze(-1) * z * inv_std
    dlogstd = (dlogp.unsqueeze(-1) * (z * z - 1)).sum(0) - ent_coef
    dvalue = (vf_coef * 2.0 / B) * (values - returns)

    def put(p, g):
        if p.grad is None:
            p.grad = g.clone()
        else:
            p.grad.copy_(g)
    put(policy.log_std, dlogstd)
    for name, dout in (("pi", dmean), ("vf", dvalue.unsqueeze(-1))):
        layers, saved = nets[name], acts[name]
        dy = dout.to(cd)
        for li in reversed(range(len(layers))):
            lin = layers[li]
            gw, gb = _splitk_wgrad(dy, saved[li], split_k)
            put(lin.weight, gw)
            put(lin.bias, gb)
            if li > 0:
                dy = (dy @ lin.weight.to(cd)) * (saved[li] > 0).to(cd)
    return pl, vl


def _colsum(x):
    xf = x.float()
    ones = torch.ones((*xf.shape[:-2], 1, xf.shape[-2]), device=x.device)
    return torch.matmul(ones, xf).squeeze(-2)


def flatten_parameters(policy, pad: int = 64):
    if getattr(policy, "_flat", None) is not None:
        return policy._flat
    params = list(policy.parameters())
    pi, vf = _layers(policy.mlp_extractor.policy_net), _layers(policy.mlp_extractor.value_net)
    lead = []
    if len(pi) == len(vf) and all(a.weight.shape == b.weight.shape for a, b in zip(pi, vf)):
        for a, b in zip(pi, vf):
            lead += [a.weight, b.weight, a.bias, b.bias]
    la, lc = getattr(policy, "lstm_actor", None), getattr(policy, "lstm_critic", None)
    if policy.recurrent and lc is not None and la.hidden_size == lc.hidden_size:
        for key in ("weight_ih_l0", "weight_hh_l0", "bias_ih_l0", "bias_hh_l0"):
            lead += [getattr(la, key), getattr(lc, key)]
    ids = {id(p) for p in lead}
    params = lead + [p for p in params if id(p) not in ids]
    dev = params[0].device
    slots, n = [], 0
    for p in params:
        slots.append((n, p.numel()))
        n += (p.numel() + pad - 1) // pad * pad
    pflat, gflat = torch.zeros(n, device=dev), torch.zeros(n, device=dev)
    for p, (off, k) in zip(params, slots):
        pflat[off:off + k].copy_(p.data.reshape(-1))
        p.data = pflat[off:off + k].view(p.shape)
        p.grad = gflat[off:off + k].view(p.shape)
    policy._flat = {"p": pflat, "g": gflat, "slots": slots, "params": params}
    return policy._flat


class FlatAdam:

    def __init__(self, flat, lib, lr, max_norm, betas=(0.9, 0.999), eps=1e-5):
        self.flat, self.lib = flat, lib
        self.lr, self.max_norm, self.betas, self.eps = float(lr), float(max_norm), betas, float(eps)
        dev = flat["p"].device
        self.m, self.v = torch.zeros_like(flat["p"]), torch.zeros_like(flat["p"])
        self._step = torch.zeros(2, dtype=torch.int32, device=dev)
        self.sq = torch.zeros(512, device=dev)
        self.presummed = 0
        self.shadow = None

    @property
    def step_count(self):
        return self._step[1]

    def set_step_count(self, step: float) -> None:
        self._step.fill_(int(step))

    def step(self, grad_scale: float = 1.0):
        f = self.flat
        stream = torch.cuda.current_stream(f["p"].device).cuda_stream
        p = lambda t: C.c_void_p(t.data_ptr())
        if self.presummed > 0:
            self.lib.check(self.lib.L.myo_adam_apply(
                p(f["p"]), p(f["g"]), p(self.m), p(self.v), f["p"].numel(), self.lr, self.betas[0], self.betas[1],
                self.eps, self.max_norm, float(grad_scale), p(self._step), p(self.sq), int(self.presummed),
                p(self.shadow) if self.shadow is not None else None, C.c_void_p(stream)))
            return
        self.lib.check(self.lib.L.myo_adam_clip_step(
            p(f["p"]), p(f["g"]), p(self.m), p(self.v), f["p"].numel(), self.lr, self.betas[0], self.betas[1],
            self.eps, self.max_norm, float(grad_scale), p(self._step), p(self.sq),
            p(self.shadow) if self.shadow is not None else None, C.c_void_p(stream)))

    def snapshot(self):
        return [t.clone() for t in (self.flat["p"], self.m, self.v, self._step)]

    def restore(self, snap):
        for t, s in zip((self.flat["p"], self.m, self.v, self._step), snap):
            t.copy_(s)
        if self.shadow is not None:
            self.shadow.copy_(self.flat["p"])


class FusedPPOStep:

    def __init__(self, policy, lib, clip_range, ent_coef, vf_coef, split_k=64):
        self.policy, self.lib = policy, lib
        self.clip, self.ent, self.vf, self.split = float(clip_range), float(ent_coef), float(vf_coef), split_k
        self.adam_syncs_shadow = False
        self.nets = _nets(policy)
        dev = policy.log_std.device
        self.master, self.half = [], []
        self.wb = {}
        flat = getattr(policy, "_flat", None)
        if flat is not None:
            hflat = torch.empty_like(flat["p"], dtype=torch.bfloat16)
            self.master, self.half = [flat["p"]], [hflat]
            for p, (off, k) in zip(flat["params"], flat["slots"]):
                self.wb[id(p)] = hflat[off:off + k].view(p.shape)
        else:
            for name, layers in self.nets.items():
                for lin in layers:
                    for p in (lin.weight, lin.bias):
                        if p.grad is None:
                            p.grad = torch.zeros_like(p)
                        h = torch.empty_like(p, dtype=torch.bfloat16)
                        self.master.append(p.data)
                        self.half.append(h)
                        self.wb[id(p)] = h
        if policy.log_std.grad is None:
            policy.log_std.grad = torch.zeros_like(policy.log_std)
        A = policy.act_dim
        self.merged = None
        if flat is not None:
            self.merged = self._stacked_views(flat, hflat)
        self.acc = torch.zeros(2 * A + 4, device=dev)
        self.stats = torch.zeros(2, device=dev)
        self.external_adv_stats = False
        self.A = A
        self._work = {}
        self._mfma = {}
        self.use_mfma_step = True
        self.adam = None

    def _mfma_desc(self, B, obs_all, act_all, oldlp_all, adv_all, ret_all, idx):
        from .. import native
        flat = getattr(self.policy, "_flat", None)
        if not self.use_mfma_step or flat is None or self.merged is None or len(self.merged) != 2 or self.policy.recurrent:
            return None
        pi, vf = self.nets["pi"], self.nets["vf"]
        O = obs_all.shape[1]
        hid = pi[0].weight.shape[0]
        shapes_ok = all(tuple(l.weight.shape) == s for l, s in ((pi[0], (hid, O)), (vf[0], (hid, O)), (pi[1], (hid, hid)), (vf[1], (hid, hid)),
                                                               (pi[2], (self.A, hid)), (vf[2], (1, hid))))
        if not shapes_ok or self.policy.log_std.dim() != 1 or obs_all.dtype != torch.float32:
            return None
        G = flat["p"].numel()
        key = (B, O, self.A, hid, G)
        hit = self._mfma.get(key)
        if hit is not None:
            d = hit[0]
            if d is not None:
                d.obs, d.act, d.oldlp, d.adv, d.ret, d.idx = (t.data_ptr() for t in (obs_all, act_all, oldlp_all, adv_all, ret_all, idx))
            return d
        nbytes = self.lib.L.myo_ppo_mlp_workspace_bytes(B, O, self.A, hid, G)
        if nbytes <= 0:
            self._mfma[key] = (None, None)
            return None
        ws = torch.zeros(nbytes, dtype=torch.uint8, device=obs_all.device)
        slot = {id(p): sl[0] for p, sl in zip(flat["params"], flat["slots"])}
        d = native.PpoMlpDesc()
        d.obs, d.act, d.oldlp, d.adv, d.ret, d.idx = (t.data_ptr() for t in (obs_all, act_all, oldlp_all, adv_all, ret_all, idx))
        d.B, d.O, d.A, d.hidden = B, O, self.A, hid
        d.params, d.grads, d.G = flat["p"].data_ptr(), flat["g"].data_ptr(), G
        for k, (a, b) in enumerate(zip(pi, vf)):
            for net, lin in enumerate((a, b)):
                wname, bname = (("off_W1", "off_b1"), ("off_W2", "off_b2"), ("off_Wh", "off_bh"))[k]
                getattr(d, wname)[net] = slot[id(lin.weight)]
                getattr(d, bname)[net] = slot[id(lin.bias)]
        d.off_log_std = slot[id(self.policy.log_std)]
        d.clip, d.vf_coef, d.ent_coef = self.clip, self.vf, self.ent
        d.adv_stats, d.acc = self.stats.data_ptr(), self.acc.data_ptr()
        d.workspace, d.workspace_bytes = ws.data_ptr(), nbytes
        if self.adam is not None and self.lib.L.myo_ppo_mlp_sqnorm_parts(self.A) <= self.adam.sq.numel():
            d.sqnorm_part, d.adam_step = self.adam.sq.data_ptr(), self.adam._step.data_ptr()
        self._mfma[key] = (d, ws)
        return d

    def rollout_desc(self, obs, seed, draw, t_idx, obs_buf, act_buf, val_buf, logp_buf, clipped):
        from .. import native
        flat = getattr(self.policy, "_flat", None)
        if not self.use_mfma_step or flat is None or self.merged is None or len(self.merged) != 2 or self.policy.recurrent:
            return None
        pi, vf = self.nets["pi"], self.nets["vf"]
        N, O = obs.shape
        hid = pi[0].weight.shape[0]
        shapes_ok = all(tuple(l.weight.shape) == s for l, s in ((pi[0], (hid, O)), (vf[0], (hid, O)), (pi[1], (hid, hid)), (vf[1], (hid, hid)),
                                                               (pi[2], (self.A, hid)), (vf[2], (1, hid))))
        if not shapes_ok or self.policy.log_std.dim() != 1 or obs.dtype != torch.float32 or N % 32:
            return None
        nbytes = self.lib.L.myo_ppo_mlp_rollout_workspace_bytes(O, self.A, hid)
        if nbytes <= 0:
            return None
        ws = torch.zeros(nbytes, dtype=torch.uint8, device=obs.device)
        slot = {id(p): sl[0] for p, sl in zip(flat["params"], flat["slots"])}
        d = native.PpoMlpRolloutDesc()
        d.obs, d.N, d.O, d.A, d.hidden, d.params = obs.data_ptr(), N, O, self.A, hid, flat["p"].data_ptr()
        for k, (a, b) in enumerate(zip(pi, vf)):
            for net, lin in enumerate((a, b)):
                wname, bname = (("off_W1", "off_b1"), ("off_W2", "off_b2"), ("off_Wh", "off_bh"))[k]
                getattr(d, wname)[net] = slot[id(lin.weight)]
                getattr(d, bname)[net] = slot[id(lin.bias)]
        d.off_log_std = slot[id(self.policy.log_std)]
        d.seed, d.draw_counter, d.t_idx = seed, draw.data_ptr(), t_idx.data_ptr()
        d.obs_buf, d.act_buf, d.val_buf, d.logp_buf, d.clipped = (t.data_ptr() for t in (obs_buf, act_buf, val_buf, logp_buf, clipped))
        d.deterministic, d.workspace, d.workspace_bytes = 0, ws.data_ptr(), nbytes
        self._rollout = (d, ws)
        self.refresh_rollout_images()
        return d

    def refresh_rollout_images(self):
        r = getattr(self, "_rollout", None)
        if r is not None:
            stream = torch.cuda.current_stream(self.acc.device).cuda_stream
            self.lib.check(self.lib.L.myo_ppo_mlp_rollout_refresh(C.byref(r[0]), C.c_void_p(stream)))

    def rollout_policy(self, d):
        stream = torch.cuda.current_stream(self.acc.device).cuda_stream
        self.lib.check(self.lib.L.myo_ppo_mlp_rollout(C.byref(d), C.c_void_p(stream)))

    def _mfma_step(self, d):
        d.compute_adv_stats = 0 if self.external_adv_stats else 1
        stream = torch.cuda.current_stream(self.acc.device).cuda_stream
        self.lib.check(self.lib.L.myo_ppo_mlp_step(C.byref(d), C.c_void_p(stream)))
        if self.adam is not None:
            self.adam.presummed = self.lib.L.myo_ppo_mlp_sqnorm_parts(self.A) if d.sqnorm_part else 0
        return self.acc[self.A], self.acc[self.A + 1]

    def _workbuf(self, key, n):
        w = self._work.get((key, n))
        if w is None:
            w = self._work[(key, n)] = torch.zeros(n, device=self.acc.device)
        return w

    def _stacked_views(self, flat, hflat):
        pi, vf = self.nets["pi"][:-1], self.nets["vf"][:-1]
        if len(pi) != len(vf) or (not pi and not self.policy.recurrent):
            return None
        slot = {id(p): sl for p, sl in zip(flat["params"], flat["slots"])}
        out = []
        for a, b in zip(pi, vf):
            lay = {}
            for key, pa, pb in (("w", a.weight, b.weight), ("b", a.bias, b.bias)):
                (oa, k), (ob, kb) = slot[id(pa)], slot[id(pb)]
                if pa.shape != pb.shape or ob != oa + k:
                    return None
                shape = (2,) + tuple(pa.shape)
                lay[key + "h"] = hflat[oa:oa + 2 * k].view(shape)
                lay[key + "g"] = flat["g"][oa:oa + 2 * k].view(shape)
            out.append(lay)
        return out

    def _reduce(self, part, out, groups, splits):
        n = out.numel() // groups
        stream = torch.cuda.current_stream(out.device).cuda_stream
        self.lib.check(self.lib.L.myo_splitk_reduce(C.c_void_p(part.data_ptr()), int(part.dtype == torch.bfloat16),
                                                    C.c_void_p(out.data_ptr()), groups, splits, n, C.c_void_p(stream)))

    def _reduce2(self, part_a, out_a, groups_a, splits_a, part_b, out_b, groups_b, splits_b):
        stream = torch.cuda.current_stream(out_a.device).cuda_stream
        self.lib.check(self.lib.L.myo_splitk_reduce2(
            C.c_void_p(part_a.data_ptr()), int(part_a.dtype == torch.bfloat16), C.c_void_p(out_a.data_ptr()), groups_a, splits_a,
            out_a.numel() // groups_a, C.c_void_p(part_b.data_ptr()), int(part_b.dtype == torch.bfloat16),
            C.c_void_p(out_b.data_ptr()), groups_b, splits_b, out_b.numel() // groups_b, C.c_void_p(stream)))

    def _relu_bwd_partial(self, dh, act):
        G, B, H = dh.shape
        if not (B % 32 == 0 and H % 16 == 0 and 256 % (H // 2) == 0):
            return None
        partial = torch.empty((G * B // 32, H), device=dh.device)
        stream = torch.cuda.current_stream(dh.device).cuda_stream
        self.lib.check(self.lib.L.myo_relu_bwd_colsum_bf16(C.c_void_p(dh.data_ptr()), C.c_void_p(act.data_ptr()), G * B, H,
                                                           C.c_void_p(partial.data_ptr()), C.c_void_p(stream)))
        return partial

    def _relu_bwd_bias(self, dh, act, bias_grad):
        G, B, H = dh.shape
        if B % 32 == 0 and H % 16 == 0 and 256 % (H // 2) == 0:
            partial = torch.empty((G * B // 32, H), device=dh.device)
            stream = torch.cuda.current_stream(dh.device).cuda_stream
            self.lib.check(self.lib.L.myo_relu_bwd_colsum_bf16(C.c_void_p(dh.data_ptr()), C.c_void_p(act.data_ptr()), G * B, H,
                                                               C.c_void_p(partial.data_ptr()), C.c_void_p(stream)))
            self._reduce(partial, bias_grad, G, B // 32)
            return dh
        dh = torch.ops.aten.threshold_backward(dh, act, 0)
        bias_grad.copy_(_colsum(dh))
        return dh

    def _loss_kernel(self, mean, values, actions, old_logp, adv, returns, dmean_h=None, dvalue_h=None, direct=None):
        pol = self.policy
        B, A = mean.shape[0], self.A
        in_bf16 = int(mean.dtype == torch.bfloat16)
        assert values.dtype == mean.dtype
        d = direct or (None, None, None)
        dev = mean.device
        dmean, dvalue = torch.empty((B, A), device=dev), torch.empty(B, device=dev)
        work = self._workbuf("loss", ((B + 63) // 64) * (2 * A + 3))
        stream = torch.cuda.current_stream(dev).cuda_stream
        p = lambda t: C.c_void_p(t.data_ptr()) if t is not None else None
        self.lib.check(self.lib.L.myo_ppo_loss_grad(
            p(mean), p(values), p(actions), p(old_logp), p(adv), p(returns), p(pol.log_std.data), p(self.stats),
            B, A, self.clip, self.vf, p(dmean), p(dvalue), p(self.acc), p(dmean_h), p(dvalue_h), p(work), in_bf16, self.ent,
            p(d[0]), p(d[1]), p(d[2]), C.c_void_p(stream)))
        return dmean, dvalue

    def _sde_loss(self, mean_h, value_h, lat_h, actions, old_logp, adv, returns):
        pol, A, B = self.policy, self.A, mean_h.shape[0]
        pi_head, vf_head = self.nets["pi"][-1], self.nets["vf"][-1]
        lat2 = lat_h.float() ** 2
        e2 = torch.exp(2.0 * pol.log_std.data.float())
        var = lat2 @ e2 + pol.SDE_EPS
        diff = actions - mean_h.float()
        z2 = diff * diff
        logp = (-0.5 * z2 / var - 0.5 * torch.log(var)).sum(-1) - 0.5 * A * math.log(2 * math.pi)
        advn = (adv - self.stats[0]) / (self.stats[1] + 1e-8)
        ratio = torch.exp(logp - old_logp)
        s1, s2 = advn * ratio, advn * torch.clamp(ratio, 1 - self.clip, 1 + self.clip)
        inside = (ratio > 1 - self.clip) & (ratio < 1 + self.clip)
        dlogp = -(advn * ratio) * torch.where(s1 <= s2, torch.ones_like(ratio), inside.to(ratio.dtype)) / B
        dmean = dlogp.unsqueeze(-1) * diff / var
        dvar = dlogp.unsqueeze(-1) * (0.5 * z2 / (var * var) - 0.5 / var) - (self.ent / B) * 0.5 / var
        pol.log_std.grad.copy_(2.0 * e2 * (lat2.t() @ dvar))
        v = value_h.float().reshape(B)
        err = v - returns
        dvalue = (self.vf * 2.0 / B) * err
        sums = _colsum(torch.stack([torch.min(s1, s2), err * err], -1))
        self.acc[A].copy_(-sums[0] / B)
        self.acc[A + 1].copy_(sums[1] / B)
        pi_head.bias.grad.copy_(_colsum(dmean))
        vf_head.bias.grad.copy_(_colsum(dvalue.unsqueeze(-1)))
        return dmean.to(torch.bfloat16), dvalue.to(torch.bfloat16).unsqueeze(-1)

    @torch.no_grad()
    def run_indexed(self, obs_all, act_all, oldlp_all, adv_all, ret_all, idx):
        if self.merged is None:
            return self.run(obs_all[idx], act_all[idx], oldlp_all[idx], adv_all[idx], ret_all[idx])
        d = self._mfma_desc(idx.shape[0], obs_all, act_all, oldlp_all, adv_all, ret_all, idx)
        if d is not None:
            return self._mfma_step(d)
        if self.adam is not None:
            self.adam.presummed = 0
        B, O, A = idx.shape[0], obs_all.shape[1], self.A
        dev = obs_all.device
        x2 = torch.empty((2, B, O), device=dev, dtype=torch.bfloat16)
        act, oldlp = torch.empty((B, A), device=dev), torch.empty(B, device=dev)
        adv, ret = torch.empty(B, device=dev), torch.empty(B, device=dev)
        work = self._workbuf("gather", 2 * ((B + 15) // 16))
        stream = torch.cuda.current_stream(dev).cuda_stream
        p = lambda t: C.c_void_p(t.data_ptr())
        self.lib.check(self.lib.L.myo_ppo_gather(p(obs_all), p(act_all), p(oldlp_all), p(adv_all), p(ret_all), p(idx), B, O, A,
                                                 p(x2), 2, p(act), p(oldlp), p(adv), p(ret), None if self.external_adv_stats else p(self.stats), p(work),
                                                 C.c_void_p(stream)))
        return self._merged_core(x2, act, oldlp, adv, ret)

    @torch.no_grad()
    def _run_merged(self, obs, actions, old_logp, adv, returns):
        if self.use_mfma_step:
            B = obs.shape[0]
            ar = self._work.get(("arange", B))
            if ar is None:
                ar = self._work[("arange", B)] = torch.arange(B, device=obs.device)
            d = self._mfma_desc(B, obs.contiguous(), actions.contiguous(), old_logp.contiguous(), adv.contiguous(), returns.contiguous(), ar)
            if d is not None:
                return self._mfma_step(d)
        if self.adam is not None:
            self.adam.presummed = 0
        var, mu = torch.var_mean(adv)
        self.stats[0].copy_(mu)
        self.stats[1].copy_(var.sqrt())
        x2 = obs.to(torch.bfloat16).unsqueeze(0).expand(2, obs.shape[0], obs.shape[1]).contiguous()
        return self._merged_core(x2, actions, old_logp, adv, returns)

    def refresh_shadow(self):
        if len(self.half) == 1:
            self.half[0].copy_(self.master[0])
        else:
            torch._foreach_copy_(self.half, self.master)
        self.refresh_rollout_images()

    def trunk_heads(self, x2):
        B = x2.shape[1]
        stream = torch.cuda.current_stream(x2.device).cuda_stream
        h, saved = x2, [x2]
        for lay in self.merged:
            h = torch.bmm(h, lay["wh"].transpose(1, 2))
            self.lib.check(self.lib.L.myo_bias_relu_bf16(C.c_void_p(h.data_ptr()), C.c_void_p(lay["bh"].data_ptr()), 2, B,
                                                         h.shape[2], C.c_void_p(stream)))
            saved.append(h)
        pi_head, vf_head = self.nets["pi"][-1], self.nets["vf"][-1]
        mean_h = torch.addmm(self.wb[id(pi_head.bias)], h[0], self.wb[id(pi_head.weight)].t())
        value_h = torch.addmm(self.wb[id(vf_head.bias)], h[1], self.wb[id(vf_head.weight)].t())
        return saved, mean_h, value_h

    def _merged_core(self, x2, actions, old_logp, adv, returns, want_dx=False):
        pol, L = self.policy, self.merged
        B, A = x2.shape[1], self.A
        s = self.split if (B % self.split == 0) else 1
        dev = x2.device
        stream = torch.cuda.current_stream(dev).cuda_stream
        if not self.adam_syncs_shadow:
            self.refresh_shadow()
        saved, mean_h, value_h = self.trunk_heads(x2)
        h = saved[-1]
        pi_head, vf_head = self.nets["pi"][-1], self.nets["vf"][-1]
        wpi, wvf = self.wb[id(pi_head.weight)], self.wb[id(vf_head.weight)]
        acc = self.acc
        if getattr(pol, "use_sde", False):
            dmean_h, dvalue_h = self._sde_loss(mean_h, value_h, h[0], actions, old_logp, adv, returns)
        else:
            dmean_h = torch.empty((B, A), device=dev, dtype=torch.bfloat16)
            dvalue_h = torch.empty((B, 1), device=dev, dtype=torch.bfloat16)
            self._loss_kernel(mean_h, value_h, actions, old_logp, adv, returns, dmean_h, dvalue_h,
                              direct=(pol.log_std.grad, pi_head.bias.grad, vf_head.bias.grad))
        parts = [torch.bmm(dy.view(s, B // s, -1).transpose(1, 2), x.view(s, B // s, -1))
                 for dy, x in ((dmean_h, h[0]), (dvalue_h, h[1]))]
        if pi_head.weight.grad.numel() % 2 == 0 and vf_head.weight.grad.numel() % 2 == 0:
            self._reduce2(parts[0], pi_head.weight.grad, 1, s, parts[1], vf_head.weight.grad, 1, s)
        else:
            self._reduce(parts[0], pi_head.weight.grad, 1, s)
            self._reduce(parts[1], vf_head.weight.grad, 1, s)
        dh = torch.empty_like(h)
        torch.mm(dmean_h, wpi, out=dh[0])
        torch.mm(dvalue_h, wvf, out=dh[1])
        for li in reversed(range(len(L))):
            lay, x = L[li], saved[li]
            bias_part = self._relu_bwd_partial(dh, saved[li + 1])
            if bias_part is None:
                dh = self._relu_bwd_bias(dh, saved[li + 1], lay["bg"])
            H, I = lay["wh"].shape[1], lay["wh"].shape[2]
            part = torch.bmm(dh.view(2 * s, B // s, H).transpose(1, 2), x.reshape(2 * s, B // s, I))
            if bias_part is not None and (H * I) % 2 == 0:
                self._reduce2(part, lay["wg"], 2, s, bias_part, lay["bg"], 2, B // 32)
            else:
                if bias_part is not None:
                    self._reduce(bias_part, lay["bg"], 2, B // 32)
                self._reduce(part, lay["wg"], 2, s)
            if li > 0 or want_dx:
                dh = torch.bmm(dh, lay["wh"])
        if want_dx:
            return acc[A], acc[A + 1], dh
        return acc[A], acc[A + 1]

    @torch.no_grad()
    def run(self, obs, actions, old_logp, adv, returns):
        if self.merged is not None:
            return self._run_merged(obs, actions, old_logp, adv, returns)
        pol = self.policy
        if self.adam is not None:
            self.adam.presummed = 0
        B, A = obs.shape[0], self.A
        torch._foreach_copy_(self.half, self.master)
        x0 = obs.to(torch.bfloat16)
        acts, outs = {}, {}
        for name, layers in self.nets.items():
            h = x0
            saved = [h]
            for li, lin in enumerate(layers):
                h = torch.addmm(self.wb[id(lin.bias)], h, self.wb[id(lin.weight)].t())
                if li < len(layers) - 1:
                    h = torch.relu_(h)
                    saved.append(h)
            acts[name], outs[name] = saved, h.float()
        mean, values = outs["pi"].contiguous(), outs["vf"].reshape(B).contiguous()
        var, mu = torch.var_mean(adv)
        self.stats[0].copy_(mu)
        self.stats[1].copy_(var.sqrt())
        dmean, dvalue = self._loss_kernel(mean, values, actions, old_logp, adv, returns)
        torch.sub(self.acc[:A], self.ent, out=pol.log_std.grad)
        for name, dout in (("pi", dmean), ("vf", dvalue.unsqueeze(-1))):
            layers, saved = self.nets[name], acts[name]
            dy = dout.to(torch.bfloat16)
            for li in reversed(range(len(layers))):
                lin = layers[li]
                x = saved[li]
                s = self.split if (B % self.split == 0) else 1
                part = torch.bmm(dy.view(s, B // s, -1).transpose(1, 2), x.view(s, B // s, -1))
                torch.sum(part, 0, dtype=torch.float32, out=lin.weight.grad)
                lin.bias.grad.copy_(_colsum(dy))
                if li > 0:
                    dy = torch.ops.aten.threshold_backward(dy @ self.wb[id(lin.weight)], saved[li], 0)
        return self.acc[A], self.acc[A + 1]
```

myochallenge_amd/rl/ppo.py:

```python
from __future__ import annotations

import os
import time
from dataclasses import dataclass, field
from typing import Callable, Dict, Optional

import torch
import torch.distributed as dist

from .policy import ActorCriticPolicy


@dataclass
class PPOConfig:
    n_steps: int = 128
    batch_size: int = 4096
    n_epochs: int = 10
    learning_rate: float = 3e-4
    clip_range: float = 0.2
    ent_coef: float = 0.0
    vf_coef: float = 0.5
    gamma: float = 0.99
    gae_lambda: float = 0.95
    max_grad_norm: float = 0.5
    normalize_advantage: bool = True
    bf16: bool = True
    sync_adv_moments: bool = False
    use_graphs: bool = True
    graph_allreduce: bool = False


def compute_gae(rewards, values, episode_starts, last_values, last_dones, gamma, lam):
    T = rewards.shape[0]
    if rewards.is_cuda and rewards.dtype == torch.float32:
        import ctypes as C
        from .. import native
        lib = native.load()
        adv, ret = torch.empty_like(rewards), torch.empty_like(rewards)
        p = lambda t: C.c_void_p(t.contiguous().data_ptr())
        lv, ld = last_values.float().contiguous(), last_dones.float().contiguous()
        lib.check(lib.L.myo_gae(p(rewards), p(values), p(episode_starts), p(lv), p(ld), T, rewards.shape[1],
                                float(gamma), float(lam), p(adv), p(ret),
                                C.c_void_p(torch.cuda.current_stream(rewards.device).cuda_stream)))
        return adv, ret
    adv = torch.zeros_like(rewards)
    last = torch.zeros_like(last_values)
    for t in reversed(range(T)):
        if t == T - 1:
            nonterm, nextv = 1.0 - last_dones, last_values
        else:
            nonterm, nextv = 1.0 - episode_starts[t + 1], values[t + 1]
        delta = rewards[t] + gamma * nextv * nonterm - values[t]
        last = delta + gamma * lam * nonterm * last
        adv[t] = last
    return adv, adv + values


class PPO:
    def __init__(self, env, policy: ActorCriticPolicy, cfg: PPOConfig = PPOConfig(), seed: int = 0):
        self.env, self.policy, self.cfg = env, policy, cfg
        self.device = env.device
        self.policy.to(self.device)
        on_gpu = self.device.type == "cuda"
        if not policy.recurrent and (cfg.n_steps * env.num_envs) % min(cfg.batch_size, cfg.n_steps * env.num_envs):
            import warnings
            warnings.warn(f"rollout of {cfg.n_steps * env.num_envs} samples is not a multiple of batch_size={cfg.batch_size}: the last "
                          f"{(cfg.n_steps * env.num_envs) % cfg.batch_size} samples of every epoch's permutation are not trained on "
                          "(stable-baselines3 would train on them as a truncated minibatch)")
        self.optimizer = torch.optim.Adam(self.policy.parameters(), lr=cfg.learning_rate, eps=1e-5,
                                          capturable=on_gpu, foreach=True if on_gpu else None)
        self._graph = None
        self._t_host = 0
        self._fused = None
        self._fused_rec = None
        self._flat_adam = None
        sde = getattr(policy, "use_sde", False)
        if cfg.use_graphs and on_gpu and not policy.recurrent:
            from .. import native
            from .fused_mlp import FlatAdam, flatten_parameters
            self._flat_adam = FlatAdam(flatten_parameters(self.policy), native.load(), cfg.learning_rate,
                                       cfg.max_grad_norm)
            from .fused_mlp import FusedPPOStep
            self._fused = FusedPPOStep(self.policy, native.load(), cfg.clip_range, cfg.ent_coef, cfg.vf_coef)
            if sde and self._fused.merged is None:
                self._fused = self._flat_adam = None
                self.optimizer = torch.optim.Adam(self.policy.parameters(), lr=cfg.learning_rate, eps=1e-5, capturable=on_gpu,
                                                  foreach=True if on_gpu else None)
            if self._fused is not None and len(self._fused.half) == 1:
                self._flat_adam.shadow = self._fused.half[0]
                self._fused.adam_syncs_shadow = True
                self._fused.refresh_shadow()
        elif cfg.use_graphs and on_gpu and policy.recurrent:
            from .. import native
            from .fused_mlp import FlatAdam, flatten_parameters
            self._flat_adam = FlatAdam(flatten_parameters(self.policy), native.load(), cfg.learning_rate,
                                       cfg.max_grad_norm)
            if cfg.bf16 and os.environ.get("MYO_RECURRENT_AUTOGRAD") != "1":
                from .fused_lstm import FusedRecurrentPPOStep
                self._fused_rec = FusedRecurrentPPOStep.create(self.policy, native.load(), cfg.clip_range, cfg.ent_coef, cfg.vf_coef)
                if self._fused_rec is not None:
                    self._flat_adam.shadow = self._fused_rec.half[0]
                    self._fused_rec.adam_syncs_shadow = True
                    self._fused_rec.refresh_shadow()
        self.world = dist.get_world_size() if dist.is_available() and dist.is_initialized() else 1
        if self._fused is not None and self._flat_adam is not None and self.world == 1 and os.environ.get("MYO_ADAM_SEPARATE") != "1":
            self._fused.adam = self._flat_adam
        self.rank = dist.get_rank() if self.world > 1 else 0
        N, T, O, A = env.num_envs, cfg.n_steps, env.obs_dim, env.act_dim
        d = self.device
        self.obs_buf = torch.zeros((T, N, O), device=d)
        self.act_buf = torch.zeros((T, N, A), device=d)
        self.rew_buf = torch.zeros((T, N), device=d)
        self.val_buf = torch.zeros((T, N), device=d)
        self.logp_buf = torch.zeros((T, N), device=d)
        self.start_buf = torch.zeros((T, N), device=d)
        self._last_obs = None
        self._last_starts = torch.ones(N, device=d)
        self._state = policy.initial_state(N, d)
        self._rollout_state0 = None
        self.num_timesteps = 0
        self.n_updates = 0
        self.ep_returns: list = []
        self.ep_lengths: list = []
        self.gen = torch.Generator(device=self.device if on_gpu else "cpu")
        self.gen.manual_seed(seed + 1000 * self.rank)
        nparam = sum(p.numel() for p in self.policy.parameters())
        self._flat_grad = self.policy._flat["g"] if self._flat_adam is not None else torch.zeros(nparam, device=d)
        self.timers: Dict[str, float] = {"rollout": 0.0, "gae": 0.0, "update": 0.0}

    def _autocast(self):
        on = self.cfg.bf16 and self.device.type == "cuda"
        return torch.autocast(device_type=self.device.type, dtype=torch.bfloat16, enabled=on)

    def _graphed_rollout(self) -> bool:
        return self.cfg.use_graphs and self.device.type == "cuda" and hasattr(self.env, "step_tensor")

    @torch.no_grad()
    def _rollout_policy_part(self):
        with self._autocast():
            if self.policy.recurrent:
                actions, values, logp, new_state = self.policy.act(self._obs_s, self._state_s, self._starts_s)
                for dst, src in zip(self._state_new, new_state):
                    dst.copy_(src)
            else:
                actions, values, logp, _ = self.policy.act(self._obs_s, None, None)
        self._act_s.copy_(actions); self._val_s.copy_(values); self._logp_s.copy_(logp)
        self._clip_s.copy_(torch.clamp(actions, -1.0, 1.0))

    @torch.no_grad()
    def _rollout_post_part(self, raw):
        cfg = self.cfg
        outs = self._vec.process_step(*raw) if self._vec is not None else raw
        nobs, rew, done, trunc, term, comps, ep = outs
        with self._autocast():
            if self.policy.recurrent:
                tv = self.policy.predict_values(term, self._state_new, None)
            else:
                tv = self.policy.predict_values(term)
        rew = rew + cfg.gamma * tv * trunc.to(rew.dtype)
        idx = self._t_idx
        self.obs_buf.index_copy_(0, idx, self._obs_s.unsqueeze(0))
        self.act_buf.index_copy_(0, idx, self._act_s.unsqueeze(0))
        self.rew_buf.index_copy_(0, idx, rew.unsqueeze(0))
        self.val_buf.index_copy_(0, idx, self._val_s.unsqueeze(0))
        self.logp_buf.index_copy_(0, idx, self._logp_s.unsqueeze(0))
        self.start_buf.index_copy_(0, idx, self._starts_s.unsqueeze(0))
        self._obs_s.copy_(nobs)
        self._starts_s.copy_(done.to(torch.float32))
        if self.policy.recurrent:
            for dst, src in zip(self._state_s, self._state_new):
                dst.copy_(src)
        self._t_idx.add_(1).remainder_(cfg.n_steps)

    def _native_rollout(self) -> bool:
        fused = self._fused if self._fused is not None else self._fused_rec
        return (self._graphed_rollout() and fused is not None and fused.merged is not None
                and hasattr(self.env, "process_step") and hasattr(self.env, "obs_rms"))

    def _init_native_rollout(self):
        import ctypes as C
        vec, raw, d, cfg = self.env, self.env.venv, self.device, self.cfg
        N, A, O, T = vec.num_envs, vec.act_dim, vec.obs_dim, cfg.n_steps
        recurrent = self.policy.recurrent
        fused = self._fused_rec if recurrent else self._fused
        lib = fused.lib
        first = vec.reset_tensor() if self._last_obs is None else self._last_obs
        self._obs_s = first.clone().contiguous()
        self._starts_s = self._last_starts.clone()
        self._clip_s = torch.zeros((N, A), device=d)
        self._t_idx = torch.zeros(1, dtype=torch.int32, device=d)
        self._draw = torch.zeros(2, dtype=torch.int64, device=d)
        self._x2 = torch.empty((2, N, O), device=d, dtype=torch.bfloat16)
        self.term_buf = torch.zeros((T, N, O), device=d)
        self.trunc_buf = torch.zeros((T, N), device=d)
        self._vn_work = torch.zeros(((N + 127) // 128) * 2 * (O + 1), dtype=torch.float64, device=d)
        seed = int(self.gen.initial_seed()) & 0xFFFFFFFFFFFFFFFF
        p = lambda t: C.c_void_p(t.data_ptr())

        rdesc = fused.rollout_desc(self._obs_s, seed, self._draw, self._t_idx, self.obs_buf, self.act_buf, self.val_buf,
                                   self.logp_buf, self._clip_s) if os.environ.get("MYO_ROLLOUT_GEMM") != "1" else None
        if recurrent:
            H, bf = self.policy.hidden, torch.bfloat16
            self._hs, self._cs = torch.zeros((2, N, H), device=d, dtype=bf), torch.zeros((2, N, H), device=d, dtype=bf)
            self._cs32 = torch.zeros((2, N, H), device=d, dtype=torch.float32)
            self._hs[0].copy_(self._state[0][0]); self._hs[1].copy_(self._state[2][0])
            self._cs32[0].copy_(self._state[1][0]); self._cs32[1].copy_(self._state[3][0])
            self._cs.copy_(self._cs32)
            self._hm, self._cm = torch.empty_like(self._hs), torch.empty_like(self._cs)
            self._cm32 = torch.empty_like(self._cs32)
            self._lat, self._cn = torch.empty_like(self._hs), torch.empty_like(self._hs)
            self._ws = torch.empty((2, N, 4 * H), device=d, dtype=bf)
            self._bsum = torch.zeros((2, 1, 4 * H), device=d, dtype=bf)
            self.crit_h_buf, self.crit_c_buf = torch.zeros((T, N, H), device=d, dtype=bf), torch.zeros((T, N, H), device=d, dtype=bf)
            Lw = fused.lstm

        sde = getattr(self.policy, "use_sde", False)
        if sde:
            self._act_s, self._logp_s = torch.zeros((N, A), device=d), torch.zeros(N, device=d)
            self._sde_W = torch.zeros((N,) + tuple(self.policy.log_std.shape), device=d)
            self._reset_sde_noise()

        def sample(saved, mean_h, value_h, st):
            if not sde:
                lib.check(lib.L.myo_rollout_sample(p(mean_h), p(value_h), p(self.policy.log_std.data), N, A, seed, p(self._draw),
                                                   p(self._t_idx), p(self.act_buf), p(self.val_buf), p(self.logp_buf),
                                                   p(self._clip_s), 0, st))
                return
            mu, lat = mean_h.float(), saved[-1][0].float().contiguous()
            lib.check(lib.L.myo_rollout_sample_sde(p(mu), p(lat), p(self._sde_W), p(self.policy.log_std.data), N, lat.shape[1], A,
                                                   p(self._act_s), p(self._clip_s), p(self._logp_s), 0, st))
            t64 = self._t_idx.long()
            self.act_buf.index_copy_(0, t64, self._act_s.unsqueeze(0))
            self.logp_buf.index_copy_(0, t64, self._logp_s.unsqueeze(0))
            self.val_buf.index_copy_(0, t64, value_h.float().view(1, N))

        def part_a_recurrent():
            st = C.c_void_p(torch.cuda.current_stream(d).cuda_stream)
            lib.check(lib.L.myo_rollout_policy_input(p(self._obs_s), N, O, p(self.obs_buf), p(self._x2), 2, p(self._t_idx), st))
            keep = torch.rsub(self._starts_s, 1.0).view(1, N, 1)
            torch.mul(self._hs, keep, out=self._hm)
            torch.mul(self._cs32, keep, out=self._cm32)
            if fused.step_kernels:
                gx = torch.addmm(self._bsum.view(8 * H), self._x2[0], Lw["wihh"].view(8 * H, O).t())
                lib.check(lib.L.myo_lstm_step_fwd(p(gx), 4 * H, 8 * H, p(self._hm), None, p(Lw["whhh"]), None, 2, N, H,
                                                  p(self._lat), N * H, p(self._hs), p(self._cs), None, None, p(self._cm32), p(self._cs32), st))
            else:
                self._cm.copy_(self._cm32)
                gx = torch.baddbmm(self._bsum, self._x2, Lw["wihh"].transpose(1, 2))
                gh = torch.bmm(self._hm, Lw["whhh"].transpose(1, 2))
                lib.check(lib.L.myo_lstm_cell_fwd(p(gx), p(gh), p(self._cm), None, 2 * N, N, H, 1, p(self._lat), p(self._hs), p(self._cs),
                                                  p(self._cn), p(self._ws), st))
                self._cs32.copy_(self._cs)
            t64 = self._t_idx.long()
            self.crit_h_buf.index_copy_(0, t64, self._hs[1:2])
            self.crit_c_buf.index_copy_(0, t64, self._cs[1:2])
            saved, mean_h, value_h = fused.trunk_heads(self._lat)
            sample(saved, mean_h, value_h, st)

        def part_a():
            if recurrent:
                part_a_recurrent()
                return
            if rdesc is not None:
                fused.rollout_policy(rdesc)
                return
            st = C.c_void_p(torch.cuda.current_stream(d).cuda_stream)
            lib.check(lib.L.myo_rollout_policy_input(p(self._obs_s), N, O, p(self.obs_buf), p(self._x2), 2, p(self._t_idx), st))
            saved, mean_h, value_h = fused.trunk_heads(self._x2)
            sample(saved, mean_h, value_h, st)

        self._vn_sync = self.world > 1 and getattr(vec, "sync_ranks", False) and vec.training
        self._vn_batch = torch.zeros(2 * O + 3, dtype=torch.float64, device=d)

        def part_b1(rawout):
            obs, rew = rawout[:2]
            st = C.c_void_p(torch.cuda.current_stream(d).cuda_stream)
            lib.check(lib.L.myo_vecnorm_batch_moments(p(obs), p(rew), N, O, p(vec.returns), float(vec.gamma), int(vec.training),
                                                      p(self._vn_work), p(self._vn_batch), st))

        def part_b2(rawout):
            obs, rew, done, trunc, term = rawout[:5]
            st = C.c_void_p(torch.cuda.current_stream(d).cuda_stream)
            lib.check(lib.L.myo_vecnorm_finish(
                p(obs), p(rew), p(done), p(trunc), p(term), N, O, p(vec.obs_rms.mean), p(vec.obs_rms.var), p(vec.obs_rms.count),
                p(vec.ret_rms.buf), p(vec.returns), float(vec.epsilon), float(vec.clip_obs), float(vec.clip_reward),
                int(vec.training), int(vec.norm_obs), int(vec.norm_reward), p(self._obs_s), p(self._starts_s), p(self._t_idx),
                p(self.rew_buf), p(self.start_buf), p(self.term_buf), p(self.trunc_buf), p(self._vn_batch), st))
            lib.check(lib.L.myo_rollout_advance(p(self._t_idx), T, p(self._draw), st))

        def part_b(rawout):
            if self._vn_sync:
                part_b1(rawout)
                dist.all_reduce(self._vn_batch)
                part_b2(rawout)
                return
            obs, rew, done, trunc, term = rawout[:5]
            st = C.c_void_p(torch.cuda.current_stream(d).cuda_stream)
            lib.check(lib.L.myo_vecnorm_step(
                p(obs), p(rew), p(done), p(trunc), p(term), N, O, p(vec.obs_rms.mean), p(vec.obs_rms.var), p(vec.obs_rms.count),
                p(vec.ret_rms.buf), p(vec.returns), float(vec.gamma), float(vec.epsilon), float(vec.clip_obs),
                float(vec.clip_reward), int(vec.training), int(vec.norm_obs), int(vec.norm_reward), p(self._obs_s),
                p(self._starts_s), p(self._t_idx), p(self.rew_buf), p(self.start_buf), p(self.term_buf), p(self.trunc_buf),
                p(self._vn_work), st))
            lib.check(lib.L.myo_rollout_advance(p(self._t_idx), T, p(self._draw), st))

        self._raw = raw
        fused.refresh_shadow()
        rawout = (raw._obs, raw._rew, raw._done, raw._trunc, raw._term, raw._comps, raw._ep)
        restore = (self._obs_s, self._starts_s, vec.obs_rms.buf, vec.ret_rms.buf, vec.returns) + ((self._hs, self._cs, self._cs32) if recurrent else ())
        keep = [t.clone() for t in restore]
        if recurrent:
            self._refresh_rollout_lstm()
        side = torch.cuda.Stream(device=d)
        side.wait_stream(torch.cuda.current_stream(d))
        with torch.cuda.stream(side):
            part_a()
            part_b(rawout)
        torch.cuda.current_stream(d).wait_stream(side)
        torch.cuda.synchronize(d)
        for t, k in zip(restore, keep):
            t.copy_(k)
        vec.old_obs, vec.old_reward = rawout[0], rawout[1]
        self._t_idx.zero_()
        self._draw.zero_()
        self._gA, self._gB, self._gB2 = torch.cuda.CUDAGraph(), torch.cuda.CUDAGraph(), None
        with torch.cuda.graph(self._gA, capture_error_mode="thread_local"):
            part_a()
        if self._vn_sync:
            self._gB2 = torch.cuda.CUDAGraph()
            with torch.cuda.graph(self._gB, capture_error_mode="thread_local"):
                part_b1(rawout)
            with torch.cuda.graph(self._gB2, capture_error_mode="thread_local"):
                part_b2(rawout)
        else:
            with torch.cuda.graph(self._gB, capture_error_mode="thread_local"):
                part_b(rawout)
        self._rollout_ready = True
        self._native = True

    def _refresh_rollout_lstm(self):
        Lw = self._fused_rec.lstm
        torch.add(Lw["bihh"], Lw["bhhh"], out=self._bsum.view(2, -1))

    def _native_state(self):
        f = lambda z, k: z[k:k + 1].float()
        return (f(self._hs, 0), f(self._cs32, 0).clone(), f(self._hs, 1), f(self._cs32, 1).clone())

    def _init_rollout_graphs(self):
        env, d = self.env, self.device
        self._vec = env if hasattr(env, "process_step") else None
        self._raw = env.venv if self._vec is not None else env
        N, A = env.num_envs, env.act_dim
        first = env.reset_tensor() if self._last_obs is None else self._last_obs
        self._obs_s = first.clone()
        self._starts_s = self._last_starts.clone()
        self._act_s, self._clip_s = torch.zeros((N, A), device=d), torch.zeros((N, A), device=d)
        self._val_s, self._logp_s = torch.zeros(N, device=d), torch.zeros(N, device=d)
        self._t_idx = torch.zeros(1, dtype=torch.long, device=d)
        if self.policy.recurrent:
            self._state_s = tuple(x.clone() for x in self._state)
            self._state_new = tuple(torch.zeros_like(x) for x in self._state)
        side = torch.cuda.Stream(device=d)
        side.wait_stream(torch.cuda.current_stream(d))
        with torch.cuda.stream(side):
            for _ in range(2):
                self._rollout_policy_part()
                raw = self._raw.step_tensor(self._clip_s)
                self._rollout_post_part(raw)
        torch.cuda.current_stream(d).wait_stream(side)
        torch.cuda.synchronize(d)
        self._t_idx.zero_()
        self._raw_static = raw
        self._gA, self._gB = torch.cuda.CUDAGraph(), torch.cuda.CUDAGraph()
        with torch.cuda.graph(self._gA, capture_error_mode="thread_local"):
            self._rollout_policy_part()
        with torch.cuda.graph(self._gB, capture_error_mode="thread_local"):
            self._rollout_post_part(self._raw_static)
        self._rollout_ready = True

    def rollout_step(self) -> None:
        if not getattr(self, "_rollout_ready", False):
            if self._native_rollout():
                self._init_native_rollout()
            else:
                self._init_rollout_graphs()
        if hasattr(self.env, "begin_rollout"):
            self.env.begin_rollout()
        if self.policy.recurrent:
            if self._t_host == 0:
                self._rollout_state0 = self._native_state() if getattr(self, "_native", False) else tuple(s.clone() for s in self._state_s)
            self._t_host = (self._t_host + 1) % self.cfg.n_steps
        self._gA.replay()
        raw = self._raw.step_tensor(self._clip_s)
        self._log_episodes(raw[2], raw[6])
        self._gB.replay()
        if getattr(self, "_gB2", None) is not None:
            t0 = time.perf_counter()
            dist.all_reduce(self._vn_batch)
            self.vn_allreduce_seconds = getattr(self, "vn_allreduce_seconds", 0.0) + (time.perf_counter() - t0)
            self.vn_allreduce_calls = getattr(self, "vn_allreduce_calls", 0) + 1
            self._gB2.replay()

    def _log_episodes(self, done, ep) -> None:
        T, N = self.cfg.n_steps, self.env.num_envs
        if getattr(self, "_ep_log", None) is None or self._ep_log.shape[:2] != (T, N):
            self._ep_log = torch.full((T, N, 2), float("nan"), device=self.device)
            self._ep_t = 0
            from collections import deque
            self.ep_info_buffer = deque(maxlen=100)
        if ep is None:
            return
        torch.where(done.view(torch.bool).unsqueeze(1), ep, self._ep_nan, out=self._ep_log[self._ep_t % T])
        self._ep_t += 1

    @property
    def _ep_nan(self):
        if getattr(self, "_ep_nan_t", None) is None:
            self._ep_nan_t = torch.full((1, 1), float("nan"), device=self.device)
        return self._ep_nan_t

    def episode_stats(self) -> Dict[str, float]:
        log = getattr(self, "_ep_log", None)
        if log is not None and self._ep_t > 0:
            T = log.shape[0]
            rows = min(self._ep_t, T)
            order = [(self._ep_t - rows + k) % T for k in range(rows)]
            x = log[order].reshape(-1, 2)
            fin = x[~torch.isnan(x[:, 0])]
            if fin.shape[0] > 100:
                fin = fin[-100:]
            for r, l in fin.cpu().tolist():
                self.ep_info_buffer.append((r, l))
            log.fill_(float("nan"))
            self._ep_t = 0
        buf = getattr(self, "ep_info_buffer", None)
        if not buf:
            return {}
        return {"rollout/ep_rew_mean": float(sum(r for r, _ in buf) / len(buf)), "rollout/ep_len_mean": float(sum(l for _, l in buf) / len(buf))}

    def finish_rollout(self) -> None:
        if hasattr(self.env, "end_rollout"):
            self.env.end_rollout()
        with torch.no_grad(), self._autocast():
            if getattr(self, "_native", False) and not self.policy.recurrent:
                T, N = self.trunc_buf.shape
                tv = self.policy.predict_values(self.term_buf.view(T * N, -1)).view(T, N)
                self.rew_buf.add_(self.cfg.gamma * tv * self.trunc_buf)
            elif getattr(self, "_native", False):
                self._state_s = self._native_state()
                if bool(self.trunc_buf.any()):
                    T, N = self.trunc_buf.shape
                    H = self.policy.hidden
                    st = (None, None, self.crit_h_buf.view(1, T * N, H).float(), self.crit_c_buf.view(1, T * N, H).float())
                    tv = self.policy.predict_values(self.term_buf.view(T * N, -1), st, None).view(T, N)
                    self.rew_buf.add_(self.cfg.gamma * tv * self.trunc_buf)
            if self.policy.recurrent:
                self._last_values = self.policy.predict_values(self._obs_s, self._state_s, self._starts_s)
                self._state = self._state_s
            else:
                self._last_values = self.policy.predict_values(self._obs_s)
        self._last_obs, self._last_starts = self._obs_s, self._starts_s

    def _reset_sde_noise(self) -> None:
        pol = self.policy
        gen = self.gen if self.gen.device == pol.log_std.device else None
        W = getattr(self, "_sde_W", None)
        if W is not None and W.shape[1:] == tuple(pol.log_std.shape):
            pol.reset_noise(W.shape[0], gen, out=W)
        else:
            pol.reset_noise(self.env.num_envs, gen)

    @torch.no_grad()
    def collect_rollouts(self) -> None:
        cfg, env, pol = self.cfg, self.env, self.policy
        if getattr(pol, "use_sde", False):
            self._reset_sde_noise()
        if self._graphed_rollout():
            if self._fused is not None:
                self._fused.refresh_shadow()
            if self._fused_rec is not None:
                self._fused_rec.refresh_shadow()
                if getattr(self, "_native", False):
                    self._refresh_rollout_lstm()
            for _ in range(cfg.n_steps):
                self.rollout_step()
            self.finish_rollout()
            self.num_timesteps += cfg.n_steps * env.num_envs * self.world
            return
        if self._last_obs is None:
            self._last_obs = env.reset_tensor().clone()
        if pol.recurrent:
            self._rollout_state0 = tuple(s.clone() for s in self._state)
        if hasattr(env, "begin_rollout"):
            env.begin_rollout()
        for t in range(cfg.n_steps):
            obs, starts = self._last_obs, self._last_starts
            with self._autocast():
                actions, values, logp, new_state = pol.act(obs, self._state, starts)
            clipped = torch.clamp(actions, -1.0, 1.0)
            nobs, rew, done, trunc, term, comps, ep = env.step_tensor(clipped)
            self._log_episodes(done, ep)
            rew = rew.clone()
            if bool(trunc.any()):
                with self._autocast():
                    tv = pol.predict_values(term, new_state, None)
                rew = rew + cfg.gamma * tv * trunc.to(rew.dtype)
            self.obs_buf[t], self.act_buf[t], self.rew_buf[t] = obs, actions, rew
            self.val_buf[t], self.logp_buf[t], self.start_buf[t] = values, logp, starts
            self._state = new_state
            self._last_obs = nobs.clone()
            self._last_starts = done.to(torch.float32)
        self.num_timesteps += cfg.n_steps * env.num_envs * self.world
        if hasattr(env, "end_rollout"):
            env.end_rollout()
        with self._autocast():
            self._last_values = pol.predict_values(self._last_obs, self._state, self._last_starts)

    def _allreduce_grads(self) -> None:
        if self.world == 1:
            return
        off = 0
        for p in self.policy.parameters():
            n = p.numel()
            self._flat_grad[off:off + n] = p.grad.reshape(-1) if p.grad is not None else 0
            off += n
        dist.all_reduce(self._flat_grad, op=dist.ReduceOp.SUM)
        self._flat_grad /= self.world
        off = 0
        for p in self.policy.parameters():
            n = p.numel()
            p.grad = self._flat_grad[off:off + n].view_as(p).clone()
            off += n

    def _loss(self, values, logp, entropy, old_logp, adv, returns):
        cfg = self.cfg
        if cfg.normalize_advantage and adv.numel() > 1:
            if cfg.sync_adv_moments and self.world > 1:
                m = torch.stack([adv.sum(), (adv * adv).sum(), torch.tensor(float(adv.numel()), device=adv.device)])
                dist.all_reduce(m)
                mean = m[0] / m[2]
                std = torch.sqrt(torch.clamp(m[1] / m[2] - mean * mean, min=0.0) * m[2] / (m[2] - 1))
            else:
                mean, std = adv.mean(), adv.std()
            adv = (adv - mean) / (std + 1e-8)
        ratio = torch.exp(logp - old_logp)
        pl = -torch.min(adv * ratio, adv * torch.clamp(ratio, 1 - cfg.clip_range, 1 + cfg.clip_range)).mean()
        vl = torch.nn.functional.mse_loss(values, returns)
        ent = entropy.mean() if torch.is_tensor(entropy) and entropy.dim() > 0 else entropy
        return pl + cfg.ent_coef * (-ent) + cfg.vf_coef * vl, pl.detach(), vl.detach()

    def train(self) -> Dict[str, float]:
        cfg, pol = self.cfg, self.policy
        T, N = cfg.n_steps, self.env.num_envs
        adv, ret = compute_gae(self.rew_buf, self.val_buf, self.start_buf, self._last_values,
                               self._last_starts, cfg.gamma, cfg.gae_lambda)
        stats = {}
        if self._fused is not None:
            pl, vl = self._train_graphed(adv, ret)
        elif not pol.recurrent:
            B = T * N
            obs, act = self.obs_buf.view(B, -1), self.act_buf.view(B, -1)
            oldlp, advf, retf = self.logp_buf.view(B), adv.view(B), ret.view(B)
            bs = min(cfg.batch_size, B)
            for _ in range(cfg.n_epochs):
                perm = torch.randperm(B, generator=self.gen, device=self.device)
                for s in range(0, B - bs + 1, bs):
                    idx = perm[s:s + bs]
                    with self._autocast():
                        v, lp, ent = pol.evaluate_actions(obs[idx], act[idx])
                    loss, pl, vl = self._loss(v, lp, ent, oldlp[idx], advf[idx], retf[idx])
                    self.optimizer.zero_grad(set_to_none=True)
                    loss.backward()
                    self._allreduce_grads()
                    torch.nn.utils.clip_grad_norm_(pol.parameters(), cfg.max_grad_norm)
                    self.optimizer.step()
                    self.n_updates += 1
        elif self._flat_adam is not None:
            pl, vl = self._train_recurrent_graphed(adv, ret)
        else:
            envs_per_mb = max(1, min(N, cfg.batch_size // T))
            for _ in range(cfg.n_epochs):
                perm = torch.randperm(N, generator=self.gen, device=self.device)
                for s in range(0, N - envs_per_mb + 1, envs_per_mb):
                    idx = perm[s:s + envs_per_mb]
                    st0 = tuple(x[:, idx] for x in self._rollout_state0)
                    with self._autocast():
                        v, lp, ent = pol.evaluate_actions(self.obs_buf[:, idx], self.act_buf[:, idx], st0,
                                                          self.start_buf[:, idx])
                    loss, pl, vl = self._loss(v.reshape(-1), lp.reshape(-1), ent, self.logp_buf[:, idx].reshape(-1),
                                              adv[:, idx].reshape(-1), ret[:, idx].reshape(-1))
                    self.optimizer.zero_grad(set_to_none=True)
                    loss.backward()
                    self._allreduce_grads()
                    torch.nn.utils.clip_grad_norm_(pol.parameters(), cfg.max_grad_norm)
                    self.optimizer.step()
                    self.n_updates += 1
        stats.update(policy_loss=float(pl), value_loss=float(vl), n_updates=self.n_updates)
        return stats

    def _mb_forward_backward(self):
        g, cfg = self._gs, self.cfg
        idx = g["idx"]
        pl, vl = self._fused.run_indexed(g["obs"], g["act"], g["oldlp"], g["adv"], g["ret"], idx)
        g["pl"], g["vl"] = pl, vl

    def _mb_apply(self):
        self._flat_adam.step(1.0 / self.world)

    def _build_graphs(self, B, bs):
        d = self.device
        self._gs = {"idx": torch.zeros(bs, dtype=torch.long, device=d),
                    "obs": self.obs_buf.view(B, -1), "act": self.act_buf.view(B, -1), "oldlp": self.logp_buf.view(B),
                    "adv": torch.zeros(B, device=d), "ret": torch.zeros(B, device=d),
                    "pl": torch.zeros((), device=d), "vl": torch.zeros((), device=d)}
        self._gs["idx"].copy_(torch.arange(bs, device=d))
        side = torch.cuda.Stream(device=d)
        snap = self._flat_adam.snapshot()
        side.wait_stream(torch.cuda.current_stream(d))
        with torch.cuda.stream(side):
            for _ in range(2):
                self._mb_forward_backward()
                if self.world > 1:
                    dist.all_reduce(self._flat_grad)
                self._mb_apply()
        torch.cuda.current_stream(d).wait_stream(side)
        torch.cuda.synchronize(d)
        self._graph_fb, self._graph_ap = torch.cuda.CUDAGraph(), None
        import os
        asked = self.world > 1 and (self.cfg.graph_allreduce or os.environ.get("MYO_GRAPH_ALLREDUCE") == "1")
        want_inside = asked and dist.get_backend() == "nccl"
        if asked and not want_inside:
            import warnings
            warnings.warn(f"graph_allreduce needs the nccl (RCCL) backend, this process group is {dist.get_backend()!r}: "
                          "using the eager all-reduce between the two optimizer graphs")
        self._allreduce_in_graph = False
        if want_inside:
            g_all = torch.cuda.CUDAGraph()
            try:
                with torch.cuda.graph(g_all, capture_error_mode="thread_local"):
                    self._mb_forward_backward()
                    dist.all_reduce(self._flat_grad, op=dist.ReduceOp.SUM)
                    self._mb_apply()
            except Exception as exc:
                raise RuntimeError("capturing the RCCL gradient all-reduce inside the optimizer hipGraph failed; run without "
                                   "graph_allreduce / MYO_GRAPH_ALLREDUCE (the eager collective between two graphs)") from exc
            self._graph_fb, self._allreduce_in_graph = g_all, True
        if not self._allreduce_in_graph:
            with torch.cuda.graph(self._graph_fb, capture_error_mode="thread_local"):
                self._mb_forward_backward()
                if self.world == 1:
                    self._mb_apply()
            if self.world > 1:
                self._graph_ap = torch.cuda.CUDAGraph()
                with torch.cuda.graph(self._graph_ap, capture_error_mode="thread_local"):
                    self._mb_apply()
        self._graph_epoch = None
        n_mb = B // bs
        if self.world == 1 and os.environ.get("MYO_EPOCH_GRAPH") != "0" and n_mb > 1:
            k = max(1, min(n_mb, int(os.environ.get("MYO_EPOCH_GRAPH_STEPS", "64"))))
            self._epoch_chunk = k
            self._gs["perm"] = torch.zeros(k * bs, dtype=torch.long, device=d)
            self._gs["perm"].copy_(torch.arange(k * bs, device=d))
            torch.cuda.synchronize(d)
            self._graph_epoch = torch.cuda.CUDAGraph()
            with torch.cuda.graph(self._graph_epoch, capture_error_mode="thread_local"):
                for s in range(0, k * bs, bs):
                    self._gs["idx"].copy_(self._gs["perm"][s:s + bs])
                    self._mb_forward_backward()
                    self._mb_apply()
        self._flat_adam.restore(snap)
        self._graph = (B, bs)

    def _train_graphed(self, adv, ret):
        cfg = self.cfg
        B = cfg.n_steps * self.env.num_envs
        bs = min(cfg.batch_size, B)
        ext = (cfg.sync_adv_moments and self.world > 1) or not cfg.normalize_advantage
        if self._fused.external_adv_stats != ext:
            self._fused.external_adv_stats = ext
            self._graph = None
        if self._graph != (B, bs):
            self._build_graphs(B, bs)
        g = self._gs
        g["adv"].copy_(adv.view(B)); g["ret"].copy_(ret.view(B))
        if not cfg.normalize_advantage:
            self._fused.stats.copy_(torch.tensor([0.0, 1.0], device=self.device))
        if getattr(self, "_graph_epoch", None) is not None and not ext:
            k, n_mb = self._epoch_chunk, B // bs
            for _ in range(cfg.n_epochs):
                perm = torch.randperm(B, generator=self.gen, device=self.device)
                done = 0
                while n_mb - done >= k:
                    g["perm"].copy_(perm[done * bs:(done + k) * bs])
                    self._graph_epoch.replay()
                    done += k
                for j in range(done, n_mb):
                    g["idx"].copy_(perm[j * bs:(j + 1) * bs])
                    self._graph_fb.replay()
                self.n_updates += n_mb
            self._fused.refresh_shadow()
            return g["pl"], g["vl"]
        for _ in range(cfg.n_epochs):
            perm = torch.randperm(B, generator=self.gen, device=self.device)
            for s in range(0, B - bs + 1, bs):
                g["idx"].copy_(perm[s:s + bs])
                if ext and cfg.normalize_advantage:
                    a = g["adv"][perm[s:s + bs]].double()
                    m = torch.stack([a.sum(), (a * a).sum(), torch.tensor(float(bs), dtype=torch.float64, device=self.device)])
                    dist.all_reduce(m)
                    mean = m[0] / m[2]
                    std = torch.sqrt(torch.clamp(m[1] / m[2] - mean * mean, min=0.0) * m[2] / (m[2] - 1))
                    self._fused.stats.copy_(torch.stack([mean, std]).float())
                self._graph_fb.replay()
                if self.world > 1 and not self._allreduce_in_graph:
                    dist.all_reduce(self._flat_grad, op=dist.ReduceOp.SUM)
                    if self._dp_check:
                        self._dp_compare("gradient after the all-reduce", self._flat_grad)
                        self._dp_compare("parameters before the optimizer step", self._flat_adam.flat["p"])
                        self._dp_compare("Adam m before the optimizer step", self._flat_adam.m)
                        self._dp_compare("Adam v before the optimizer step", self._flat_adam.v)
                        self._dp_compare("Adam step counter before the optimizer step", self._flat_adam._step)
                    self._graph_ap.replay()
                    if self._dp_check:
                        self._dp_compare("gradient after the optimizer step", self._flat_grad)
                        self._dp_compare("|g|^2 partial sums", self._flat_adam.sq[:64].contiguous())
                        self._dp_compare("parameters after the optimizer step", self._flat_adam.flat["p"])
                self.n_updates += 1
        self._fused.refresh_shadow()
        return g["pl"], g["vl"]

    _dp_check = bool(__import__("os").environ.get("MYO_DP_CHECK"))

    def _dp_compare(self, what: str, x: torch.Tensor) -> None:
        cs = x.detach().contiguous().view(torch.int32).to(torch.int64).sum().reshape(1)
        lo, hi = cs.clone(), cs.clone()
        dist.all_reduce(lo, op=dist.ReduceOp.MIN); dist.all_reduce(hi, op=dist.ReduceOp.MAX)
        if int(lo[0]) != int(hi[0]) and dist.get_rank() == 0:
            print(f"MYO_DP_CHECK: {what} differs across ranks at optimizer step {self.n_updates}", flush=True)

    def _rec_forward_backward(self):
        g = self._rg
        idx = g["idx"]
        if self._fused_rec is not None:
            pl, vl = self._fused_rec.run_sequences(self.obs_buf, self.act_buf, self.start_buf, self.logp_buf, g["adv"], g["ret"],
                                                   g["h0"], g["c0"], idx)
            g["pl"], g["vl"] = pl, vl
            return
        self._flat_grad.zero_()
        st0 = tuple(x.index_select(1, idx) for x in g["state0"])
        sel = lambda buf: buf.index_select(1, idx)
        with self._autocast():
            v, lp, ent = self.policy.evaluate_actions(sel(self.obs_buf), sel(self.act_buf), st0, sel(self.start_buf))
        loss, pl, vl = self._loss(v.reshape(-1), lp.reshape(-1), ent, sel(self.logp_buf).reshape(-1),
                                  sel(g["adv"]).reshape(-1), sel(g["ret"]).reshape(-1))
        loss.backward()
        g["pl"].copy_(pl); g["vl"].copy_(vl)

    def _build_recurrent_graphs(self, T, N, m):
        d = self.device
        self._rg = {"idx": torch.arange(m, device=d), "state0": tuple(torch.zeros_like(x) for x in self._rollout_state0),
                    "adv": torch.zeros((T, N), device=d), "ret": torch.zeros((T, N), device=d),
                    "pl": torch.zeros((), device=d), "vl": torch.zeros((), device=d)}
        if self._fused_rec is not None:
            H = self.policy.hidden
            self._rg["h0"], self._rg["c0"] = torch.zeros((2, N, H), device=d), torch.zeros((2, N, H), device=d)
        side = torch.cuda.Stream(device=d)
        snap = self._flat_adam.snapshot()
        side.wait_stream(torch.cuda.current_stream(d))
        with torch.cuda.stream(side):
            for _ in range(2):
                self._rec_forward_backward()
                if self.world > 1:
                    dist.all_reduce(self._flat_grad)
                self._mb_apply()
        torch.cuda.current_stream(d).wait_stream(side)
        torch.cuda.synchronize(d)
        self._rgraph_fb, self._rgraph_ap = torch.cuda.CUDAGraph(), None
        with torch.cuda.graph(self._rgraph_fb, capture_error_mode="thread_local"):
            self._rec_forward_backward()
            if self.world == 1:
                self._mb_apply()
        if self.world > 1:
            self._rgraph_ap = torch.cuda.CUDAGraph()
            with torch.cuda.graph(self._rgraph_ap, capture_error_mode="thread_local"):
                self._mb_apply()
        self._flat_adam.restore(snap)
        self._rgraph = (T, N, m)

    def _rec_stage(self, adv, ret, T, N, m):
        cfg = self.cfg
        if self._fused_rec is not None:
            ext = (cfg.sync_adv_moments and self.world > 1) or not cfg.normalize_advantage
            if self._fused_rec.external_adv_stats != ext:
                self._fused_rec.external_adv_stats = ext
                self._rgraph = None
        if getattr(self, "_rgraph", None) != (T, N, m):
            self._build_recurrent_graphs(T, N, m)
        g = self._rg
        g["adv"].copy_(adv); g["ret"].copy_(ret)
        for dst, src in zip(g["state0"], self._rollout_state0):
            dst.copy_(src)
        fr = self._fused_rec
        if fr is not None:
            fr.refresh_shadow()
            hp, cp, hv, cv = self._rollout_state0
            g["h0"][0].copy_(hp[0]); g["h0"][1].copy_(hv[0]); g["c0"][0].copy_(cp[0]); g["c0"][1].copy_(cv[0])
            if not cfg.normalize_advantage:
                fr.stats.copy_(torch.tensor([0.0, 1.0], device=self.device))
        return g

    def _train_recurrent_graphed(self, adv, ret):
        cfg = self.cfg
        T, N = cfg.n_steps, self.env.num_envs
        m = max(1, min(N, cfg.batch_size // T))
        g, fr = self._rec_stage(adv, ret, T, N, m), self._fused_rec
        for _ in range(cfg.n_epochs):
            perm = torch.randperm(N, generator=self.gen, device=self.device)
            for s in range(0, N - m + 1, m):
                g["idx"].copy_(perm[s:s + m])
                if fr is not None and fr.external_adv_stats and cfg.normalize_advantage:
                    a = g["adv"][:, perm[s:s + m]].double()
                    mom = torch.stack([a.sum(), (a * a).sum(), torch.tensor(float(a.numel()), dtype=torch.float64, device=self.device)])
                    dist.all_reduce(mom)
                    mean = mom[0] / mom[2]
                    std = torch.sqrt(torch.clamp(mom[1] / mom[2] - mean * mean, min=0.0) * mom[2] / (mom[2] - 1))
                    fr.stats.copy_(torch.stack([mean, std]).float())
                self._rgraph_fb.replay()
                if self.world > 1:
                    dist.all_reduce(self._flat_grad, op=dist.ReduceOp.SUM)
                    self._rgraph_ap.replay()
                self.n_updates += 1
        return g["pl"], g["vl"]

    def _optimizer_state_dict(self) -> dict:
        cfg = self.cfg
        params = list(self.policy.parameters())
        state = {}
        if self._flat_adam is not None:
            fa, flat = self._flat_adam, self.policy._flat
            slot = {id(p): sl for p, sl in zip(flat["params"], flat["slots"])}
            step = float(fa.step_count)
            if step > 0:
                for i, p in enumerate(params):
                    off, k = slot[id(p)]
                    state[i] = {"step": torch.tensor(step), "exp_avg": fa.m[off:off + k].view(p.shape).cpu().clone(),
                                "exp_avg_sq": fa.v[off:off + k].view(p.shape).cpu().clone()}
        else:
            sd = self.optimizer.state_dict()
            state = {i: {k: (v.detach().cpu().clone() if torch.is_tensor(v) else v) for k, v in st.items()}
                     for i, st in sd["state"].items()}
        return {"state": state, "param_groups": [{"lr": cfg.learning_rate, "betas": (0.9, 0.999), "eps": 1e-5, "weight_decay": 0,
                                                  "amsgrad": False, "maximize": False, "foreach": None, "capturable": False,
                                                  "params": list(range(len(params)))}]}

    def load_optimizer_state(self, opt: Optional[dict]) -> bool:
        if not opt or not opt.get("state"):
            return False
        params = list(self.policy.parameters())
        st = opt["state"]
        if sorted(st) != list(range(len(params))) or any(tuple(st[i]["exp_avg"].shape) != tuple(p.shape) for i, p in enumerate(params)):
            return False
        step = float(st[0]["step"]) if "step" in st[0] else 0.0
        if self._flat_adam is not None:
            fa, flat = self._flat_adam, self.policy._flat
            slot = {id(p): sl for p, sl in zip(flat["params"], flat["slots"])}
            for i, p in enumerate(params):
                off, k = slot[id(p)]
                fa.m[off:off + k].copy_(st[i]["exp_avg"].reshape(-1).to(fa.m))
                fa.v[off:off + k].copy_(st[i]["exp_avg_sq"].reshape(-1).to(fa.v))
            fa.set_step_count(step)
        else:
            dev = self.device
            for i, p in enumerate(params):
                self.optimizer.state[p] = {"step": torch.tensor(step, dtype=torch.float32, device=dev if self.device.type == "cuda" else "cpu"),
                                           "exp_avg": st[i]["exp_avg"].to(p).clone(), "exp_avg_sq": st[i]["exp_avg_sq"].to(p).clone()}
        return True

    def save(self, path: str) -> None:
        from .sb3_zip import save_sb3_zip
        cfg = self.cfg
        hyper = {k: getattr(cfg, k) for k in ("n_steps", "batch_size", "n_epochs", "gamma", "gae_lambda", "ent_coef", "vf_coef",
                                              "max_grad_norm", "learning_rate", "clip_range", "normalize_advantage")}
        last = self._last_obs.detach().cpu().numpy() if self._last_obs is not None else None
        orig = getattr(self.env, "old_obs", None)
        save_sb3_zip(path, self.policy, hyper, n_envs=self.env.num_envs, num_timesteps=self.num_timesteps, n_updates=self.n_updates,
                     last_obs=last, last_original_obs=orig.detach().cpu().numpy() if orig is not None else None,
                     last_episode_starts=self._last_starts.detach().cpu().numpy() > 0.5,
                     optimizer_state=self._optimizer_state_dict(), clip_obs=float(getattr(self.env, "clip_obs", 10.0)))

    def set_parameters(self, path: str) -> None:
        from .sb3_zip import read_zip
        _, sd, _ = read_zip(path)
        self.policy.load_state_dict(sd, strict=True)
        if self._fused is not None:
            self._fused.refresh_shadow()

    def learn(self, total_timesteps: int, callback: Optional[Callable[["PPO"], None]] = None, log=None):
        t_start = time.time()
        while self.num_timesteps < total_timesteps:
            self.collect_rollouts()
            if callback is not None:
                callback(self)
            stats = self.train()
            if log is not None and self.rank == 0:
                fps = self.num_timesteps / max(1e-9, time.time() - t_start)
                log({"time/fps": fps, "time/total_timesteps": self.num_timesteps, **self.episode_stats(),
                     **{"train/" + k: v for k, v in stats.items()}})
        return self

    @property
    def n_calls(self) -> int:
        return self.num_timesteps // max(1, self.env.num_envs * self.world)
```

Before: 1.750 million.

## Write bf16 weight images from Adam and batch advantage stats per epoch graph

The Adam kernel now scatters each updated parameter straight into the bf16 and bias weight images that the MLP step and the rollout policy use, through a precomputed destination map. This lets the per-minibatch prep kernel that rebuilt those images be skipped, and the rollout can share the same image buffer. Advantage moments for all minibatches in the epoch graph are computed up front in one batched launch, and the per-minibatch idx copy is dropped by passing perm slices directly. The cost is an extra map read and scattered writes inside Adam, plus some added coupling between the layout code and the kernels.

```diff
diff --git a/include/myobatch.h b/include/myobatch.h
--- a/include/myobatch.h
+++ b/include/myobatch.h
@@ -222,10 +222,13 @@
   int64_t workspace_bytes;
   float* sqnorm_part;
   int32_t* adam_step;
+  void* images;
+  int32_t images_current;
 } myo_ppo_mlp_desc;
 int myo_ppo_mlp_sqnorm_parts(int act_dim);
 long long myo_ppo_mlp_workspace_bytes(int B, int obs_dim, int act_dim, int hidden, long long G);
 int myo_ppo_mlp_step(const myo_ppo_mlp_desc* d, void* stream);
+int myo_ppo_adv_stats(const float* adv, const int64_t* idx, int B, int nmb, float* part, float* stats, void* stream);
 
 typedef struct myo_ppo_mlp_rollout_desc {
   const float* obs;
@@ -250,6 +253,9 @@
 int myo_adam_apply(float* p, const float* g, float* m, float* v, int n, float lr, float b1, float b2,
                    float eps, float max_norm, float grad_scale, const int* step, const float* scratch, int nparts,
                    uint16_t* p_bf16, void* stream);
+int myo_adam_apply_images(float* p, const float* g, float* m, float* v, int n, float lr, float b1, float b2,
+                          float eps, float max_norm, float grad_scale, const int* step, const float* scratch, int nparts,
+                          uint16_t* p_bf16, const int32_t* img_map, void* images, void* stream);
 
 const char* myo_last_error(void);
 const char* myo_version(void);
diff --git a/myochallenge_amd/csrc/myo_ppo_mlp.h b/myochallenge_amd/csrc/myo_ppo_mlp.h
--- a/myochallenge_amd/csrc/myo_ppo_mlp.h
+++ b/myochallenge_amd/csrc/myo_ppo_mlp.h
@@ -45,26 +45,30 @@
 };
 
 #define MLP_ADV_BLOCKS 64
+__device__ __forceinline__ void mlp_adv_merge(const float* adv_part, int adv_nb, int B, float* adv_stats) {
+  __shared__ float sp[3 * MLP_ADV_BLOCKS];
+  const int t = threadIdx.x;
+  if (t < 3 * adv_nb) sp[t] = adv_part[t];
+  __syncthreads();
+  if (t == 0) {
+    float cn = 0.f, cm = 0.f, c2 = 0.f;
+    for (int b = 0; b < adv_nb; ++b) {
+      const float bn = sp[3 * b], bm = sp[3 * b + 1], b2 = sp[3 * b + 2];
+      if (bn > 0.f) {
+        const float tot = cn + bn, dl = bm - cm;
+        cm += dl * (bn / tot);
+        c2 += b2 + dl * dl * (cn * bn / tot);
+        cn = tot;
+      }
+    }
+    adv_stats[0] = cm; adv_stats[1] = sqrtf(c2 / (B > 1 ? B - 1 : 1));
+  }
+}
+__global__ void __launch_bounds__(256) k_adv_merge(const float* __restrict__ part, int adv_nb, int B, float* __restrict__ stats) {
+  mlp_adv_merge(part + (size_t)blockIdx.x * 3 * adv_nb, adv_nb, B, stats + 2 * blockIdx.x);
+}
 __global__ void __launch_bounds__(256) k_mlp_prep(MlpPrepArgs P) {
-  if (P.adv_nb > 0 && blockIdx.x == gridDim.x - 1) {
-    __shared__ float sp[3 * MLP_ADV_BLOCKS];
-    const int t = threadIdx.x;
-    if (t < 3 * P.adv_nb) sp[t] = P.adv_part[t];
-    __syncthreads();
-    if (t == 0) {
-      float cn = 0.f, cm = 0.f, c2 = 0.f;
-      for (int b = 0; b < P.adv_nb; ++b) {
-        const float bn = sp[3 * b], bm = sp[3 * b + 1], b2 = sp[3 * b + 2];
-        if (bn > 0.f) {
-          const float tot = cn + bn, dl = bm - cm;
-          cm += dl * (bn / tot);
-          c2 += b2 + dl * dl * (cn * bn / tot);
-          cn = tot;
-        }
-      }
-      P.adv_stats[0] = cm; P.adv_stats[1] = sqrtf(c2 / (P.B > 1 ? P.B - 1 : 1));
-    }
-  }
+  if (P.adv_nb > 0 && blockIdx.x == gridDim.x - 1) mlp_adv_merge(P.adv_part, P.adv_nb, P.B, P.adv_stats);
   constexpr int H = MLP_H;
   const long long tid = (long long)blockIdx.x * blockDim.x + threadIdx.x, nth = (long long)gridDim.x * blockDim.x;
   for (int net = 0; net < 2; ++net) {
@@ -100,6 +104,7 @@
   __shared__ float red[4];
   __shared__ float s_mean;
   const int t = threadIdx.x, nb = gridDim.x;
+  idx += (size_t)blockIdx.y * B; part += (size_t)blockIdx.y * 3 * nb;
   const int chunk = (B + nb - 1) / nb, lo = blockIdx.x * chunk, hi = min(B, lo + chunk), n = max(hi - lo, 0);
   constexpr int PER = 4;
   float v[PER];
diff --git a/myochallenge_amd/csrc/myobatch.hip b/myochallenge_amd/csrc/myobatch.hip
--- a/myochallenge_amd/csrc/myobatch.hip
+++ b/myochallenge_amd/csrc/myobatch.hip
@@ -1584,7 +1584,8 @@
 __global__ void __launch_bounds__(256) k_adam(float* __restrict__ p, const float* __restrict__ g, float* __restrict__ m,
                                               float* __restrict__ v, int n, float lr, float b1, float b2, float eps,
                                               float max_norm, float gs, const int* __restrict__ step,
-                                              const float* __restrict__ part, unsigned short* __restrict__ p_bf16, int nparts) {
+                                              const float* __restrict__ part, unsigned short* __restrict__ p_bf16, int nparts,
+                                              const int* __restrict__ img_map, void* __restrict__ images) {
   __shared__ float sq_red[256];
   {
     float a = 0.f;
@@ -1607,6 +1608,16 @@
     const float pn = p[i] - step_size * mi / (sqrtf(vi) * inv_sqrt_bc2 + eps);
     p[i] = pn;
     if (p_bf16) p_bf16[i] = myo_f2bf(pn);
+    if (img_map) {
+      const int d0 = img_map[2 * i], d1 = img_map[2 * i + 1];
+      if (d0 >= 0) {
+        unsigned u = __float_as_uint(pn);
+        u += 0x7fffu + ((u >> 16) & 1u);
+        const unsigned short h = (unsigned short)(u >> 16);
+        reinterpret_cast<unsigned short*>(images)[d0] = h;
+        if (d1 >= 0) reinterpret_cast<unsigned short*>(images)[d1] = h;
+      } else if (d0 < -1) reinterpret_cast<float*>(images)[-2 - d0] = pn;
+    }
   }
 }
 extern "C" int myo_adam_clip_step(float* p, const float* g, float* m, float* v, int n, float lr, float b1, float b2,
@@ -1617,7 +1628,7 @@
   const int blocks = (n + 255) / 256 < 1024 ? (n + 255) / 256 : 1024;
   hipLaunchKernelGGL(k_grad_sqnorm, dim3(MYO_SQN_BLOCKS), dim3(256), 0, st, g, n, grad_scale, scratch, step);
   hipLaunchKernelGGL(k_adam, dim3(blocks), dim3(256), 0, st, p, g, m, v, n, lr, b1, b2, eps, max_norm, grad_scale, step, scratch,
-                     (unsigned short*)p_bf16, MYO_SQN_BLOCKS);
+                     (unsigned short*)p_bf16, MYO_SQN_BLOCKS, (const int*)nullptr, (void*)nullptr);
   LAUNCH_CHECK(0)
   return MYO_OK;
 }
@@ -1627,7 +1638,18 @@
   if (!p || !g || !m || !v || !step || !scratch || n <= 0 || nparts <= 0) return fail(MYO_E_ARG, "myo_adam_apply: bad arguments");
   const int blocks = (n + 255) / 256 < 1024 ? (n + 255) / 256 : 1024;
   hipLaunchKernelGGL(k_adam, dim3(blocks), dim3(256), 0, (hipStream_t)stream, p, g, m, v, n, lr, b1, b2, eps, max_norm, grad_scale, step, scratch,
-                     (unsigned short*)p_bf16, nparts);
+                     (unsigned short*)p_bf16, nparts, (const int*)nullptr, (void*)nullptr);
+  LAUNCH_CHECK(0)
+  return MYO_OK;
+}
+extern "C" int myo_adam_apply_images(float* p, const float* g, float* m, float* v, int n, float lr, float b1, float b2,
+                                     float eps, float max_norm, float grad_scale, const int* step, const float* scratch, int nparts,
+                                     uint16_t* p_bf16, const int32_t* img_map, void* images, void* stream) {
+  if (!p || !g || !m || !v || !step || !scratch || !img_map || !images || n <= 0 || nparts <= 0)
+    return fail(MYO_E_ARG, "myo_adam_apply_images: bad arguments");
+  const int blocks = (n + 255) / 256 < 1024 ? (n + 255) / 256 : 1024;
+  hipLaunchKernelGGL(k_adam, dim3(blocks), dim3(256), 0, (hipStream_t)stream, p, g, m, v, n, lr, b1, b2, eps, max_norm, grad_scale, step, scratch,
+                     (unsigned short*)p_bf16, nparts, (const int*)img_map, images);
   LAUNCH_CHECK(0)
   return MYO_OK;
 }
@@ -1652,6 +1674,18 @@
   w.bytes = o;
   return w;
 }
+struct MlpImg { unsigned short *W1p, *W2, *W2T, *Whp, *WhT; float* bias; size_t bytes; };
+static MlpImg mlp_carve_images(unsigned char* base, int OP) {
+  MlpImg w;
+  size_t o = 0;
+  auto take = [&](size_t n) { unsigned char* p = base ? base + o : nullptr; o += (n + 255) / 256 * 256; return p; };
+  const size_t H = MLP_H;
+  w.W1p = (unsigned short*)take(2 * H * OP * 2); w.W2 = (unsigned short*)take(2 * H * H * 2); w.W2T = (unsigned short*)take(2 * H * H * 2);
+  w.Whp = (unsigned short*)take(2 * MLP_APM * H * 2); w.WhT = (unsigned short*)take(2 * H * MLP_AKP * 2);
+  w.bias = (float*)take((4 * H + 2 * MLP_APM) * 4);
+  w.bytes = o;
+  return w;
+}
 static int mlp_shape_ok(int B, int O, int A, int hidden) {
   return hidden == MLP_H && O >= 1 && O <= MLP_OPMAX && A >= 1 && A <= MLP_APM && B >= 64 * MLP_SPLITK && B % (64 * MLP_SPLITK) == 0;
 }
@@ -1668,8 +1702,14 @@
     return fail(MYO_E_ARG, "myo_ppo_mlp_step: null argument");
   const int B = d->B, O = d->O, A = d->A, OP = (O + 31) / 32 * 32;
   if (!mlp_shape_ok(B, O, A, d->hidden)) return fail(MYO_E_UNSUPPORTED, "myo_ppo_mlp_step: needs hidden = %d, obs <= %d, act <= %d, batch a multiple of %d", MLP_H, MLP_OPMAX, MLP_APM, 64 * MLP_SPLITK);
-  const MlpWs w = mlp_carve((unsigned char*)d->workspace, B, OP, A, d->G);
+  MlpWs w = mlp_carve((unsigned char*)d->workspace, B, OP, A, d->G);
   if ((long long)w.bytes > d->workspace_bytes) return fail(MYO_E_ARG, "myo_ppo_mlp_step: workspace too small (%zu bytes needed)", w.bytes);
+  if (d->images_current && (!d->images || d->compute_adv_stats))
+    return fail(MYO_E_ARG, "myo_ppo_mlp_step: images_current needs an image block and compute_adv_stats = 0");
+  if (d->images) {
+    const MlpImg im = mlp_carve_images((unsigned char*)d->images, OP);
+    w.W1p = im.W1p; w.W2 = im.W2; w.W2T = im.W2T; w.Whp = im.Whp; w.WhT = im.WhT; w.bias = im.bias;
+  }
   hipStream_t st = (hipStream_t)stream;
   static bool lds_set = false;
   if (!lds_set) {
@@ -1686,7 +1726,7 @@
   }
   pp.adv_part = w.advpart; pp.adv_stats = d->adv_stats; pp.adv_nb = d->compute_adv_stats ? MLP_ADV_BLOCKS : 0; pp.B = B;
   pp.W1p = w.W1p; pp.W2 = w.W2; pp.W2T = w.W2T; pp.Whp = w.Whp; pp.WhT = w.WhT; pp.bias = w.bias;
-  hipLaunchKernelGGL(k_mlp_prep, dim3(256), dim3(256), 0, st, pp);
+  if (!d->images_current) hipLaunchKernelGGL(k_mlp_prep, dim3(256), dim3(256), 0, st, pp);
   MlpArgs a;
   a.obs = d->obs; a.act = d->act; a.oldlp = d->oldlp; a.adv = d->adv; a.ret = d->ret; a.idx = (const long long*)d->idx;
   a.log_std = d->params + d->off_log_std; a.adv_stats = d->adv_stats;
@@ -1722,18 +1762,15 @@
   return MYO_OK;
 }
 
-struct MlpImg { unsigned short *W1p, *W2, *W2T, *Whp, *WhT; float* bias; size_t bytes; };
-static MlpImg mlp_carve_images(unsigned char* base, int OP) {
-  MlpImg w;
-  size_t o = 0;
-  auto take = [&](size_t n) { unsigned char* p = base ? base + o : nullptr; o += (n + 255) / 256 * 256; return p; };
-  const size_t H = MLP_H;
-  w.W1p = (unsigned short*)take(2 * H * OP * 2); w.W2 = (unsigned short*)take(2 * H * H * 2); w.W2T = (unsigned short*)take(2 * H * H * 2);
-  w.Whp = (unsigned short*)take(2 * MLP_APM * H * 2); w.WhT = (unsigned short*)take(2 * H * MLP_AKP * 2);
-  w.bias = (float*)take((4 * H + 2 * MLP_APM) * 4);
-  w.bytes = o;
-  return w;
-}
+extern "C" int myo_ppo_adv_stats(const float* adv, const int64_t* idx, int B, int nmb, float* part, float* stats, void* stream) {
+  if (!adv || !idx || !part || !stats || B <= 0 || nmb <= 0) return fail(MYO_E_ARG, "myo_ppo_adv_stats: bad arguments");
+  hipStream_t st = (hipStream_t)stream;
+  hipLaunchKernelGGL(k_adv_moments, dim3(MLP_ADV_BLOCKS, nmb), dim3(256), 0, st, adv, (const long long*)idx, B, part);
+  hipLaunchKernelGGL(k_adv_merge, dim3(nmb), dim3(256), 0, st, (const float*)part, MLP_ADV_BLOCKS, B, stats);
+  LAUNCH_CHECK(0)
+  return MYO_OK;
+}
+
 static int mlp_rollout_ok(const myo_ppo_mlp_rollout_desc* d) {
   return d->hidden == MLP_H && d->O >= 1 && d->O <= MLP_OPMAX && d->A >= 1 && d->A <= MLP_APM && d->N >= MLP_BM && d->N % MLP_BM == 0;
 }
diff --git a/myochallenge_amd/native.py b/myochallenge_amd/native.py
--- a/myochallenge_amd/native.py
+++ b/myochallenge_amd/native.py
@@ -67,6 +67,7 @@
         ("clip", C.c_float), ("vf_coef", C.c_float), ("ent_coef", C.c_float), ("compute_adv_stats", C.c_int32),
         ("adv_stats", C.c_void_p), ("acc", C.c_void_p), ("workspace", C.c_void_p), ("workspace_bytes", C.c_int64),
         ("sqnorm_part", C.c_void_p), ("adam_step", C.c_void_p),
+        ("images", C.c_void_p), ("images_current", C.c_int32),
     ]
 
 
@@ -169,6 +170,8 @@
         L.myo_lstm_seq_bwd.argtypes = [vp, C.c_longlong, C.c_longlong] + [vp] * 5 + [i32] * 5 + [vp] * 2
         L.myo_adam_clip_step.argtypes = [vp] * 4 + [i32] + [C.c_float] * 6 + [vp, vp, vp, vp]
         L.myo_adam_apply.argtypes = [vp] * 4 + [i32] + [C.c_float] * 6 + [vp, vp, i32, vp, vp]
+        L.myo_adam_apply_images.argtypes = [vp] * 4 + [i32] + [C.c_float] * 6 + [vp, vp, i32, vp, vp, vp, vp]
+        L.myo_ppo_adv_stats.argtypes = [vp, vp, i32, i32, vp, vp, vp]
         L.myo_ppo_mlp_workspace_bytes.restype = C.c_longlong
         L.myo_ppo_mlp_workspace_bytes.argtypes = [i32, i32, i32, i32, C.c_longlong]
         L.myo_ppo_mlp_step.argtypes = [C.POINTER(PpoMlpDesc), vp]
@@ -215,7 +218,7 @@
     "myo_batch_set_state", "myo_batch_warmstart", "myo_batch_set_bad_state_buffer", "myo_batch_set_task", "myo_batch_get_task", "myo_batch_set_object_group", "myo_batch_object_friction", "myo_batch_bind_constants", "myo_batch_tune_wrap_order", "myo_batch_forward_dump",
     "myo_batch_dump_size", "myo_batch_dump_offset", "myo_batch_kernel_ms",
     "myo_batch_enable_timing", "myo_ppo_loss_grad", "myo_ppo_gather", "myo_bias_relu_bf16", "myo_rollout_policy_input", "myo_rollout_sample",
-    "myo_vecnorm_step", "myo_rollout_sample_sde", "myo_vecnorm_batch_moments", "myo_vecnorm_finish", "myo_rollout_advance", "myo_gae", "myo_lstm_cell_fwd", "myo_lstm_cell_bwd", "myo_lstm_step_supported", "myo_lstm_step_fwd", "myo_lstm_step_bwd", "myo_lstm_seq_supported", "myo_lstm_seq_fwd", "myo_lstm_seq_bwd", "myo_splitk_reduce", "myo_splitk_reduce2", "myo_relu_bwd_colsum_bf16", "myo_adam_clip_step", "myo_ppo_mlp_workspace_bytes", "myo_ppo_mlp_step", "myo_ppo_mlp_sqnorm_parts", "myo_adam_apply", "myo_ppo_mlp_rollout_workspace_bytes", "myo_ppo_mlp_rollout_refresh", "myo_ppo_mlp_rollout", "myo_last_error", "myo_version",
+    "myo_vecnorm_step", "myo_rollout_sample_sde", "myo_vecnorm_batch_moments", "myo_vecnorm_finish", "myo_rollout_advance", "myo_gae", "myo_lstm_cell_fwd", "myo_lstm_cell_bwd", "myo_lstm_step_supported", "myo_lstm_step_fwd", "myo_lstm_step_bwd", "myo_lstm_seq_supported", "myo_lstm_seq_fwd", "myo_lstm_seq_bwd", "myo_splitk_reduce", "myo_splitk_reduce2", "myo_relu_bwd_colsum_bf16", "myo_adam_clip_step", "myo_ppo_mlp_workspace_bytes", "myo_ppo_mlp_step", "myo_ppo_mlp_sqnorm_parts", "myo_adam_apply", "myo_adam_apply_images", "myo_ppo_adv_stats", "myo_ppo_mlp_rollout_workspace_bytes", "myo_ppo_mlp_rollout_refresh", "myo_ppo_mlp_rollout", "myo_last_error", "myo_version",
     "myo_model_default_camera", "myo_batch_geom_poses", "myo_batch_render",
 ]
 
diff --git a/myochallenge_amd/rl/fused_mlp.py b/myochallenge_amd/rl/fused_mlp.py
--- a/myochallenge_amd/rl/fused_mlp.py
+++ b/myochallenge_amd/rl/fused_mlp.py
@@ -115,6 +115,44 @@
     return policy._flat
 
 
+MLP_H, MLP_APM, MLP_AKP = 256, 48, 64
+
+
+def image_layout(O: int) -> dict:
+    H, OP = MLP_H, (O + 31) // 32 * 32
+    sizes = (("W1p", 2 * H * OP * 2), ("W2", 2 * H * H * 2), ("W2T", 2 * H * H * 2), ("Whp", 2 * MLP_APM * H * 2),
+             ("WhT", 2 * H * MLP_AKP * 2), ("bias", (4 * H + 2 * MLP_APM) * 4))
+    lay, o = {"OP": OP}, 0
+    for name, n in sizes:
+        lay[name] = o
+        o += (n + 255) // 256 * 256
+    lay["bytes"] = o
+    return lay
+
+
+def image_destination_map(n: int, O: int, A: int, off_W1, off_b1, off_W2, off_b2, off_Wh, off_bh):
+    import numpy as np
+    H, lay = MLP_H, image_layout(O)
+    OP = lay["OP"]
+    m = np.full((n, 2), -1, dtype=np.int32)
+    for net in range(2):
+        Ah = A if net == 0 else 1
+        o, i = np.divmod(np.arange(H * O), O)
+        m[off_W1[net] + np.arange(H * O), 0] = lay["W1p"] // 2 + net * H * OP + o * OP + i
+        o, i = np.divmod(np.arange(H * H), H)
+        m[off_W2[net] + np.arange(H * H), 0] = lay["W2"] // 2 + net * H * H + o * H + i
+        m[off_W2[net] + np.arange(H * H), 1] = lay["W2T"] // 2 + net * H * H + i * H + o
+        a, h = np.divmod(np.arange(Ah * H), H)
+        m[off_Wh[net] + np.arange(Ah * H), 0] = lay["Whp"] // 2 + net * MLP_APM * H + a * H + h
+        m[off_Wh[net] + np.arange(Ah * H), 1] = lay["WhT"] // 2 + net * H * MLP_AKP + h * MLP_AKP + a
+        e = np.arange(H)
+        m[off_b1[net] + e, 0] = -2 - (lay["bias"] // 4 + net * H + e)
+        m[off_b2[net] + e, 0] = -2 - (lay["bias"] // 4 + 2 * H + net * H + e)
+        e = np.arange(Ah)
+        m[off_bh[net] + e, 0] = -2 - (lay["bias"] // 4 + 4 * H + net * MLP_APM + e)
+    return m
+
+
 class FlatAdam:
 
     def __init__(self, flat, lib, lr, max_norm, betas=(0.9, 0.999), eps=1e-5):
@@ -126,6 +164,9 @@
         self.sq = torch.zeros(512, device=dev)
         self.presummed = 0
         self.shadow = None
+        self.img_map = None
+        self.images = None
+        self.refresh_images = None
 
     @property
     def step_count(self):
@@ -138,6 +179,12 @@
         f = self.flat
         stream = torch.cuda.current_stream(f["p"].device).cuda_stream
         p = lambda t: C.c_void_p(t.data_ptr())
+        if self.presummed > 0 and self.img_map is not None:
+            self.lib.check(self.lib.L.myo_adam_apply_images(
+                p(f["p"]), p(f["g"]), p(self.m), p(self.v), f["p"].numel(), self.lr, self.betas[0], self.betas[1],
+                self.eps, self.max_norm, float(grad_scale), p(self._step), p(self.sq), int(self.presummed),
+                p(self.shadow) if self.shadow is not None else None, p(self.img_map), p(self.images), C.c_void_p(stream)))
+            return
         if self.presummed > 0:
             self.lib.check(self.lib.L.myo_adam_apply(
                 p(f["p"]), p(f["g"]), p(self.m), p(self.v), f["p"].numel(), self.lr, self.betas[0], self.betas[1],
@@ -157,6 +204,8 @@
             t.copy_(s)
         if self.shadow is not None:
             self.shadow.copy_(self.flat["p"])
+        if self.refresh_images is not None:
+            self.refresh_images()
 
 
 class FusedPPOStep:
@@ -199,6 +248,59 @@
         self._mfma = {}
         self.use_mfma_step = True
         self.adam = None
+        self._images = None
+        self._img_desc = None
+        self._rollout = None
+
+    def _mfma_shapes_ok(self, O):
+        flat = getattr(self.policy, "_flat", None)
+        if not self.use_mfma_step or flat is None or self.merged is None or len(self.merged) != 2 or self.policy.recurrent:
+            return False
+        pi, vf = self.nets["pi"], self.nets["vf"]
+        hid = pi[0].weight.shape[0]
+        return all(tuple(l.weight.shape) == s for l, s in ((pi[0], (hid, O)), (vf[0], (hid, O)), (pi[1], (hid, hid)), (vf[1], (hid, hid)),
+                                                          (pi[2], (self.A, hid)), (vf[2], (1, hid)))) and self.policy.log_std.dim() == 1
+
+    def _offsets_into(self, d):
+        flat = self.policy._flat
+        slot = {id(p): sl[0] for p, sl in zip(flat["params"], flat["slots"])}
+        for k, (a, b) in enumerate(zip(self.nets["pi"], self.nets["vf"])):
+            for net, lin in enumerate((a, b)):
+                wname, bname = (("off_W1", "off_b1"), ("off_W2", "off_b2"), ("off_Wh", "off_bh"))[k]
+                getattr(d, wname)[net] = slot[id(lin.weight)]
+                getattr(d, bname)[net] = slot[id(lin.bias)]
+        d.off_log_std = slot[id(self.policy.log_std)]
+
+    def share_images(self, O):
+        from .. import native
+        if self._images is not None:
+            return True
+        if self.adam is None or not self._mfma_shapes_ok(O):
+            return False
+        hid = self.nets["pi"][0].weight.shape[0]
+        nbytes = self.lib.L.myo_ppo_mlp_rollout_workspace_bytes(O, self.A, hid)
+        if nbytes <= 0:
+            return False
+        assert nbytes == image_layout(O)["bytes"], "image_layout() and mlp_carve_images() disagree"
+        flat = self.policy._flat
+        dev = flat["p"].device
+        d = native.PpoMlpRolloutDesc()
+        d.N, d.O, d.A, d.hidden, d.params = 32, O, self.A, hid, flat["p"].data_ptr()
+        self._offsets_into(d)
+        images = torch.zeros(nbytes, dtype=torch.uint8, device=dev)
+        d.workspace, d.workspace_bytes = images.data_ptr(), nbytes
+        m = image_destination_map(flat["p"].numel(), O, self.A, d.off_W1, d.off_b1, d.off_W2, d.off_b2, d.off_Wh, d.off_bh)
+        self._images, self._img_desc = images, d
+        self.adam.img_map, self.adam.images = torch.from_numpy(m).to(dev).contiguous(), images
+        self.adam.refresh_images = self.refresh_rollout_images
+        self.refresh_rollout_images()
+        return True
+
+    def adv_stats_chunk(self, adv_all, idx, B, nmb, part, stats):
+        stream = torch.cuda.current_stream(self.acc.device).cuda_stream
+        assert idx.numel() >= B * nmb and part.numel() >= 192 * nmb and stats.numel() >= 2 * nmb
+        self.lib.check(self.lib.L.myo_ppo_adv_stats(C.c_void_p(adv_all.data_ptr()), C.c_void_p(idx.data_ptr()), B, nmb,
+                                                    C.c_void_p(part.data_ptr()), C.c_void_p(stats.data_ptr()), C.c_void_p(stream)))
 
     def _mfma_desc(self, B, obs_all, act_all, oldlp_all, adv_all, ret_all, idx):
         from .. import native
@@ -239,6 +341,8 @@
         d.clip, d.vf_coef, d.ent_coef = self.clip, self.vf, self.ent
         d.adv_stats, d.acc = self.stats.data_ptr(), self.acc.data_ptr()
         d.workspace, d.workspace_bytes = ws.data_ptr(), nbytes
+        if self._images is not None:
+            d.images = self._images.data_ptr()
         if self.adam is not None and self.lib.L.myo_ppo_mlp_sqnorm_parts(self.A) <= self.adam.sq.numel():
             d.sqnorm_part, d.adam_step = self.adam.sq.data_ptr(), self.adam._step.data_ptr()
         self._mfma[key] = (d, ws)
@@ -259,7 +363,7 @@
         nbytes = self.lib.L.myo_ppo_mlp_rollout_workspace_bytes(O, self.A, hid)
         if nbytes <= 0:
             return None
-        ws = torch.zeros(nbytes, dtype=torch.uint8, device=obs.device)
+        ws = self._images if self._images is not None else torch.zeros(nbytes, dtype=torch.uint8, device=obs.device)
         slot = {id(p): sl[0] for p, sl in zip(flat["params"], flat["slots"])}
         d = native.PpoMlpRolloutDesc()
         d.obs, d.N, d.O, d.A, d.hidden, d.params = obs.data_ptr(), N, O, self.A, hid, flat["p"].data_ptr()
@@ -278,16 +382,21 @@
 
     def refresh_rollout_images(self):
         r = getattr(self, "_rollout", None)
-        if r is not None:
-            stream = torch.cuda.current_stream(self.acc.device).cuda_stream
+        stream = torch.cuda.current_stream(self.acc.device).cuda_stream
+        if self._img_desc is not None:
+            self.lib.check(self.lib.L.myo_ppo_mlp_rollout_refresh(C.byref(self._img_desc), C.c_void_p(stream)))
+        if r is not None and r[1] is not self._images:
             self.lib.check(self.lib.L.myo_ppo_mlp_rollout_refresh(C.byref(r[0]), C.c_void_p(stream)))
 
     def rollout_policy(self, d):
         stream = torch.cuda.current_stream(self.acc.device).cuda_stream
         self.lib.check(self.lib.L.myo_ppo_mlp_rollout(C.byref(d), C.c_void_p(stream)))
 
-    def _mfma_step(self, d):
-        d.compute_adv_stats = 0 if self.external_adv_stats else 1
+    def _mfma_step(self, d, stats=None, images_current=False):
+        d.compute_adv_stats = 0 if (self.external_adv_stats or stats is not None) else 1
+        d.adv_stats = (self.stats if stats is None else stats).data_ptr()
+        d.images = self._images.data_ptr() if self._images is not None else None
+        d.images_current = 1 if (images_current and self._images is not None and not d.compute_adv_stats) else 0
         stream = torch.cuda.current_stream(self.acc.device).cuda_stream
         self.lib.check(self.lib.L.myo_ppo_mlp_step(C.byref(d), C.c_void_p(stream)))
         if self.adam is not None:
@@ -399,12 +508,13 @@
         return dmean.to(torch.bfloat16), dvalue.to(torch.bfloat16).unsqueeze(-1)
 
     @torch.no_grad()
-    def run_indexed(self, obs_all, act_all, oldlp_all, adv_all, ret_all, idx):
+    def run_indexed(self, obs_all, act_all, oldlp_all, adv_all, ret_all, idx, stats=None, images_current=False):
         if self.merged is None:
             return self.run(obs_all[idx], act_all[idx], oldlp_all[idx], adv_all[idx], ret_all[idx])
         d = self._mfma_desc(idx.shape[0], obs_all, act_all, oldlp_all, adv_all, ret_all, idx)
         if d is not None:
-            return self._mfma_step(d)
+            return self._mfma_step(d, stats, images_current)
+        assert stats is None and not images_current, "the lean step exists on the fused MLP path only"
         if self.adam is not None:
             self.adam.presummed = 0
         B, O, A = idx.shape[0], obs_all.shape[1], self.A
@@ -419,6 +529,12 @@
                                                  p(x2), 2, p(act), p(oldlp), p(adv), p(ret), None if self.external_adv_stats else p(self.stats), p(work),
                                                  C.c_void_p(stream)))
         return self._merged_core(x2, act, oldlp, adv, ret)
+
+    def lean_ok(self, B, obs_all, act_all, oldlp_all, adv_all, ret_all, idx):
+        if self._images is None or self.adam is None or self.adam.img_map is None or self.external_adv_stats:
+            return False
+        d = self._mfma_desc(B, obs_all, act_all, oldlp_all, adv_all, ret_all, idx)
+        return d is not None and bool(d.sqnorm_part)
 
     @torch.no_grad()
     def _run_merged(self, obs, actions, old_logp, adv, returns):
diff --git a/myochallenge_amd/rl/ppo.py b/myochallenge_amd/rl/ppo.py
--- a/myochallenge_amd/rl/ppo.py
+++ b/myochallenge_amd/rl/ppo.py
@@ -105,6 +105,8 @@
         self.world = dist.get_world_size() if dist.is_available() and dist.is_initialized() else 1
         if self._fused is not None and self._flat_adam is not None and self.world == 1 and os.environ.get("MYO_ADAM_SEPARATE") != "1":
             self._fused.adam = self._flat_adam
+            if os.environ.get("MYO_ADAM_IMAGES") != "0":
+                self._fused.share_images(env.obs_dim)
         self.rank = dist.get_rank() if self.world > 1 else 0
         N, T, O, A = env.num_envs, cfg.n_steps, env.obs_dim, env.act_dim
         d = self.device
@@ -598,10 +600,10 @@
         stats.update(policy_loss=float(pl), value_loss=float(vl), n_updates=self.n_updates)
         return stats
 
-    def _mb_forward_backward(self):
+    def _mb_forward_backward(self, idx=None, stats=None, lean=False):
         g, cfg = self._gs, self.cfg
-        idx = g["idx"]
-        pl, vl = self._fused.run_indexed(g["obs"], g["act"], g["oldlp"], g["adv"], g["ret"], idx)
+        idx = g["idx"] if idx is None else idx
+        pl, vl = self._fused.run_indexed(g["obs"], g["act"], g["oldlp"], g["adv"], g["ret"], idx, stats=stats, images_current=lean)
         g["pl"], g["vl"] = pl, vl
 
     def _mb_apply(self):
@@ -663,10 +665,21 @@
             self._gs["perm"].copy_(torch.arange(k * bs, device=d))
             torch.cuda.synchronize(d)
             self._graph_epoch = torch.cuda.CUDAGraph()
+            g = self._gs
+            lean = self._fused.lean_ok(bs, g["obs"], g["act"], g["oldlp"], g["adv"], g["ret"], g["idx"])
+            if lean:
+                g["adv_stats"] = torch.zeros((k, 2), device=d)
+                g["adv_part"] = torch.zeros(192 * k, device=d)
+            torch.cuda.synchronize(d)
             with torch.cuda.graph(self._graph_epoch, capture_error_mode="thread_local"):
-                for s in range(0, k * bs, bs):
-                    self._gs["idx"].copy_(self._gs["perm"][s:s + bs])
-                    self._mb_forward_backward()
+                if lean:
+                    self._fused.adv_stats_chunk(g["adv"], g["perm"], bs, k, g["adv_part"], g["adv_stats"])
+                for j, s in enumerate(range(0, k * bs, bs)):
+                    if lean:
+                        self._mb_forward_backward(idx=g["perm"][s:s + bs], stats=g["adv_stats"][j], lean=True)
+                    else:
+                        g["idx"].copy_(g["perm"][s:s + bs])
+                        self._mb_forward_backward()
                     self._mb_apply()
         self._flat_adam.restore(snap)
         self._graph = (B, bs)
```

New measurement: 1.766 million, median of 6. No clear change (+0.9%).
